# facebookresearch/AudioDec

Measured on NVIDIA H100. Metric: 48 kHz audio samples/s, encode+quantize+lookup+decode (% HBM roofline in `roofline`), higher is better.
Workload: dtype f32

## Files before the change

### audiodec_b200/_lib.py

```python
from __future__ import annotations

import ctypes
import os

_HERE = os.path.dirname(os.path.abspath(__file__))
LIB_PATH = os.environ.get("ADEC_LIB_PATH") or os.path.join(_HERE, "lib", "libaudiodec_b200.so")
MAX_STAGES = 8

c_int, c_float, c_void_p, c_char_p = ctypes.c_int, ctypes.c_float, ctypes.c_void_p, ctypes.c_char_p
c_int64 = ctypes.c_int64
_I8 = c_int * MAX_STAGES


class AdecConfig(ctypes.Structure):
    _fields_ = [
        ("model_type", c_int),
        ("input_channels", c_int), ("output_channels", c_int), ("encode_channels", c_int), ("decode_channels", c_int),
        ("code_dim", c_int), ("codebook_num", c_int), ("codebook_size", c_int),
        ("n_enc", c_int), ("enc_ratios", _I8), ("enc_strides", _I8),
        ("n_dec", c_int), ("dec_ratios", _I8), ("dec_strides", _I8),
        ("bias", c_int),
        ("in_channels", c_int), ("out_channels", c_int), ("channels", c_int), ("kernel_size", c_int),
        ("n_up", c_int), ("upsample_scales", _I8), ("upsample_kernel_sizes", _I8),
        ("resblock_kernel_size", c_int),
        ("n_dil", c_int), ("resblock_dilations", _I8),
        ("groups", c_int),
        ("negative_slope", c_float),
        ("use_weight_norm", c_int),
        ("has_stats", c_int),
        ("codec_activate", c_int),
        ("n_resblocks", c_int), ("resblock_kernel_sizes", _I8),
        ("compute_dtype", c_int),
    ]


MODEL_SYMAD, MODEL_HIFIGAN = 0, 1

SYMBOLS = {
    "adec_create": (c_int, [ctypes.POINTER(AdecConfig), c_int, ctypes.POINTER(c_void_p)]),
    "adec_destroy": (None, [c_void_p]),
    "adec_last_error": (c_char_p, [c_void_p]),
    "adec_set_tensor": (c_int, [c_void_p, c_char_p, c_void_p, ctypes.POINTER(c_int64), c_int]),
    "adec_finalize": (c_int, [c_void_p]),
    "adec_n_streams": (c_int, [c_void_p]),
    "adec_set_streams": (c_int, [c_void_p, c_int]),
    "adec_reset": (c_int, [c_void_p, c_void_p]),
    "adec_encode": (c_int, [c_void_p, c_void_p, c_int, c_int, c_void_p, c_void_p]),
    "adec_quantize": (c_int, [c_void_p, c_void_p, c_int, c_int, c_void_p, c_void_p]),
    "adec_quantize_ex": (c_int, [c_void_p, c_void_p, c_int, c_int, c_void_p, c_void_p, c_void_p, c_void_p]),
    "adec_lookup": (c_int, [c_void_p, c_void_p, c_int, c_int, c_void_p, c_void_p]),
    "adec_lookup_packed": (c_int, [c_void_p, c_void_p, c_int, c_int, c_void_p, c_void_p]),
    "adec_decode": (c_int, [c_void_p, c_void_p, c_int, c_int, c_void_p, c_void_p]),
    "adec_encode_offline": (c_int, [c_void_p, c_void_p, c_int, c_int, c_void_p, c_void_p]),
    "adec_decode_offline": (c_int, [c_void_p, c_void_p, c_int, c_int, c_void_p, c_void_p]),
    "adec_decode_bf16": (c_int, [c_void_p, c_void_p, c_int, c_int, c_void_p, c_void_p]),
    "adec_decode_offline_bf16": (c_int, [c_void_p, c_void_p, c_int, c_int, c_void_p, c_void_p]),
    "adec_encode_offline_varlen": (c_int, [c_void_p, c_void_p, ctypes.POINTER(c_int), c_int, c_void_p, c_void_p]),
    "adec_decode_offline_varlen": (c_int, [c_void_p, c_void_p, ctypes.POINTER(c_int), c_int, c_void_p, c_void_p]),
    "adec_decode_offline_varlen_bf16": (c_int, [c_void_p, c_void_p, ctypes.POINTER(c_int), c_int, c_void_p, c_void_p]),
    "adec_encode_streams": (c_int, [c_void_p, c_void_p, ctypes.POINTER(c_int), ctypes.POINTER(c_int), c_int, c_void_p, c_void_p]),
    "adec_decode_streams": (c_int, [c_void_p, c_void_p, ctypes.POINTER(c_int), ctypes.POINTER(c_int), c_int, c_void_p, c_void_p]),
    "adec_decode_streams_bf16": (c_int, [c_void_p, c_void_p, ctypes.POINTER(c_int), ctypes.POINTER(c_int), c_int, c_void_p, c_void_p]),
    "adec_copy_stream_state": (c_int, [c_void_p, c_int, ctypes.POINTER(c_int), c_int, c_void_p]),
    "adec_frames_for": (c_int, [c_void_p, c_int]),
    "adec_hop_length": (c_int, [c_void_p]),
    "adec_codec_host": (c_int, [c_void_p, c_void_p, c_void_p, c_int, c_int, c_void_p, c_void_p, c_void_p]),
    "adec_packed_frame_bytes": (c_int, [c_void_p]),
    "adec_pack_indices": (c_int, [c_void_p, c_void_p, c_int, c_int, c_void_p, c_void_p]),
    "adec_unpack_indices": (c_int, [c_void_p, c_void_p, c_int, c_int, c_void_p, c_void_p]),
    "adec_index_error": (c_int, [c_void_p, c_void_p]),
    "adec_range_error": (c_int, [c_void_p, c_void_p]),
    "adec_launch_count": (c_int64, [c_void_p]),
    "adec_ktrace": (c_int, [c_void_p, ctypes.POINTER(ctypes.c_ulonglong), c_int]),
    "adec_probe_mma": (c_int, [c_int, c_int, c_int, c_int, ctypes.POINTER(ctypes.c_double), ctypes.POINTER(ctypes.c_double)]),
    "adec_profile": (c_int, [c_void_p, c_int]),
    "adec_profile_report": (c_int, [c_void_p, c_char_p, c_int]),
    "adec_test_causal_conv": (c_int, [c_int, c_void_p, c_int, c_int, c_int, c_void_p, c_void_p, c_int, c_int, c_int,
                                      c_int, c_int, c_int, c_float, c_void_p, c_void_p]),
    "adec_test_residual_unit": (c_int, [c_int, c_void_p, c_int, c_int, c_int, c_void_p, c_void_p, c_int, c_int, c_void_p, c_void_p]),
    "adec_test_causal_convtr": (c_int, [c_int, c_void_p, c_int, c_int, c_int, c_void_p, c_void_p, c_int, c_int,
                                        c_void_p, c_void_p]),
    "adec_test_vocoder_layer": (c_int, [c_int, c_int, c_int, c_void_p, c_int, c_int, c_int, c_void_p, c_void_p, c_int, c_int, c_int,
                                        c_int, c_int, c_int, c_int, c_float, c_void_p, c_void_p, c_void_p, c_int, c_void_p, c_void_p]),
}

_lib = None


def load():
    global _lib
    if _lib is not None:
        return _lib
    if not os.path.exists(LIB_PATH):
        raise RuntimeError(
            f"{LIB_PATH} not found: build the CUDA extension first "
            "(python -c 'import __graft_entry__ as g; g.build()').  audiodec_b200 has no CPU fallback.")
    lib = ctypes.CDLL(LIB_PATH)
    for name, (res, args) in SYMBOLS.items():
        fn = getattr(lib, name)
        fn.restype = res
        fn.argtypes = args
    _lib = lib
    return lib


def last_error(handle=None) -> str:
    msg = load().adec_last_error(handle)
    return msg.decode() if msg else ""
```

### audiodec_b200/csrc/adec.cu

```cuda
#include <cuda_runtime.h>

#include <algorithm>
#include <cmath>
#include <cstdarg>
#include <cstdio>
#include <cstring>
#include <map>
#include <memory>
#include <set>
#include <string>
#include <vector>

#include "../../include/audiodec_b200.h"
#include "kernels.cuh"
#include "wg_conv.cuh"
#include <cuda_fp16.h>
#include <cuda_bf16.h>

using namespace adec;

namespace {
thread_local std::string g_create_error;

std::string fmt(const char* f, ...) {
    char buf[1024];
    va_list ap;
    va_start(ap, f);
    vsnprintf(buf, sizeof buf, f, ap);
    va_end(ap);
    return buf;
}

struct HostTensor {
    std::vector<int64_t> shape;
    std::vector<float> data;
    int64_t numel() const { int64_t n = 1; for (auto s : shape) n *= s; return n; }
};

int round_up(int v, int m) { return (v + m - 1) / m * m; }
bool is_pow2(int v) { return v > 0 && (v & (v - 1)) == 0; }
int ilog2(int v) { int l = 0; while ((1 << l) < v) ++l; return l; }

typedef cudaError_t (*ConvLaunchFn)(const ConvArgs&, dim3, int, cudaStream_t);

template <int CW, int CO, int TT, int KC, bool F>
cudaError_t launch_conv(const ConvArgs& a, dim3 grid, int window_rows, cudaStream_t s) {
    using Cfg = ConvCfg<CW, CO, TT, KC>;
    static bool configured[64] = {false};
    int dev = 0;
    cudaGetDevice(&dev);
    auto kern = conv_gemm_kernel<CW, CO, TT, KC, F>;
    if (dev < 64 && !configured[dev]) {
        cudaError_t e = cudaFuncSetAttribute(kern, cudaFuncAttributeMaxDynamicSharedMemorySize, 227 * 1024);
        if (e != cudaSuccess) return e;
        configured[dev] = true;
    }
    const size_t smem = Cfg::smem_bytes(window_rows);
    if (smem > 227 * 1024) return cudaErrorInvalidConfiguration;
    kern<<<grid, Cfg::NTHREADS, smem, s>>>(a);
    return cudaGetLastError();
}

struct ConvKernelCfg { int CW, CO, TT, KC; bool fuse; ConvLaunchFn fn; };

#define ADEC_PLAIN(CW) \
    {CW, 256, 64, 8, false, launch_conv<CW, 256, 64, 8, false>}, \
    {CW, 128, 64, 16, false, launch_conv<CW, 128, 64, 16, false>}, \
    {CW, 64, 128, 32, false, launch_conv<CW, 64, 128, 32, false>}, \
    {CW, 32, 256, 32, false, launch_conv<CW, 32, 256, 32, false>}

const ConvKernelCfg kConvKernels[] = {
    ADEC_PLAIN(32), ADEC_PLAIN(64), ADEC_PLAIN(96), ADEC_PLAIN(128), ADEC_PLAIN(256),
    {32, 32, 256, 32, true, launch_conv<32, 32, 256, 32, true>},
    {64, 64, 128, 32, true, launch_conv<64, 64, 128, 32, true>},
    {128, 128, 64, 16, true, launch_conv<128, 128, 64, 16, true>},
    {256, 256, 64, 8, true, launch_conv<256, 256, 64, 8, true>},
};

const ConvKernelCfg* find_conv_kernel(int CW, int CO, bool fuse) {
    for (const auto& k : kConvKernels)
        if (k.CW == CW && k.CO == CO && k.fuse == fuse) return &k;
    return nullptr;
}

typedef cudaError_t (*TcPersistFn)(const ConvArgs&, int, int, int, int, int, cudaStream_t);
template <int NT, bool F, int PRE, int PREC, bool BST, bool VL>
cudaError_t launch_wg(const ConvArgs& a, int n_xtiles, int n_ytiles, int n_tiles, int n_ctas, int smem_bytes, cudaStream_t s) {
    static bool configured[64] = {false};
    int dev = 0;
    cudaGetDevice(&dev);
    auto kern = wg_conv_kernel<NT, F, PRE, PREC, BST, VL>;
    constexpr int kMaxDyn = 227 * 1024;
    if (dev < 64 && !configured[dev]) {
        cudaError_t e = cudaFuncSetAttribute(kern, cudaFuncAttributeMaxDynamicSharedMemorySize, kMaxDyn);
        if (e != cudaSuccess) return e;
        configured[dev] = true;
    }
    if (smem_bytes > kMaxDyn) return cudaErrorInvalidConfiguration;
    static const bool pdl = [] { const char* e = getenv("ADEC_PDL"); return !e || atoi(e) != 0; }();
    cudaLaunchConfig_t cfg{};
    cfg.gridDim = dim3((unsigned)n_ctas);
    cfg.blockDim = dim3((unsigned)WgCfg<NT, PREC>::THREADS);
    cfg.dynamicSmemBytes = (size_t)smem_bytes;
    cfg.stream = s;
    cudaLaunchAttribute attr[1];
    attr[0].id = cudaLaunchAttributeProgrammaticStreamSerialization;
    attr[0].val.programmaticStreamSerializationAllowed = 1;
    cfg.attrs = attr;
    cfg.numAttrs = pdl ? 1 : 0;
    return cudaLaunchKernelEx(&cfg, kern, a, n_xtiles, n_ytiles, n_tiles);
}
typedef size_t (*TcSmemFn)(int, bool);
typedef int (*TcWbufFn)(int, bool);
struct TcKernelCfg { int NT; bool fuse; int pre, prec; bool bst; int tap_bytes; TcPersistFn pfn, pfn_vl; TcSmemFn smem; TcWbufFn n_wbuf; };
#define ADEC_TC1(NT, F, PRE, PREC, BST) \
    {NT, F, PRE, PREC, BST, WgCfg<NT, PREC>::TAP_BYTES, launch_wg<NT, F, PRE, PREC, BST, false>, launch_wg<NT, F, PRE, PREC, BST, true>, \
     WgCfg<NT, PREC>::smem_bytes, WgCfg<NT, PREC>::n_wbuf}
#define ADEC_TC_FP32(NT, PREC) \
    ADEC_TC1(NT, true, ACT_ELU, PREC, false), ADEC_TC1(NT, false, ACT_NONE, PREC, false), ADEC_TC1(NT, false, ACT_ELU, PREC, false), \
    ADEC_TC1(NT, false, ACT_LRELU, PREC, false), ADEC_TC1(NT, false, ACT_NORM, PREC, false)
#define ADEC_TC_BF16(NT, BST) \
    ADEC_TC1(NT, false, ACT_NONE, PREC_BF16, BST), ADEC_TC1(NT, false, ACT_LRELU, PREC_BF16, BST), ADEC_TC1(NT, false, ACT_NORM, PREC_BF16, BST)
#define ADEC_TC(NT) ADEC_TC_FP32(NT, PREC_F16), ADEC_TC_FP32(NT, PREC_TF32), ADEC_TC_BF16(NT, false), ADEC_TC_BF16(NT, true)
const TcKernelCfg kTcKernels[] = {ADEC_TC(128), ADEC_TC(64), ADEC_TC(32)};
int kTcMaxFuse = 128;

const TcKernelCfg* find_tc_kernel(int NT, bool fuse, int pre, int prec, bool bst) {
    for (const auto& k : kTcKernels)
        if (k.NT == NT && k.fuse == fuse && k.pre == pre && k.prec == prec && k.bst == bst) return &k;
    return nullptr;
}

uint16_t half_bits(float x) { const __half h = __float2half_rn(x); uint16_t u; memcpy(&u, &h, 2); return u; }
float half_value(uint16_t u) { __half h; memcpy(&h, &u, 2); return __half2float(h); }
uint16_t bf16_bits(float x) { const __nv_bfloat16 h = __float2bfloat16_rn(x); uint16_t u; memcpy(&u, &h, 2); return u; }

float tf32_round_host(float x) {
    uint32_t u;
    memcpy(&u, &x, 4);
    if ((u & 0x7F800000u) == 0x7F800000u) return x;
    u = (u + 0x1000u) & 0xFFFFE000u;
    float r;
    memcpy(&r, &u, 4);
    return r;
}

enum OpKind { OP_STEM, OP_CONV, OP_HEAD };
enum { BUF_EXT_IN = -10, BUF_EXT_OUT = -11, BUF_NONE = -1 };

struct Op {
    OpKind kind = OP_CONV;
    std::string name;
    int G = 1, Cin = 0, Cin_eff = 0, Cout = 0, Ktaps = 1, dil = 1, RG = 1;
    int P = 0;
    int down = 1;
    int up = 1;
    bool fuse = false, shared_in = false, out_nct = false, post_tanh = false;
    int pre_act = ACT_NONE, mid_act = ACT_NONE;
    float slope = 0.f;
    std::vector<float> weff;
    std::vector<float> weff2;
    std::vector<float> hbias;
    std::vector<float> hstate;
    const ConvKernelCfg* kc = nullptr;
    const TcKernelCfg* tc = nullptr;
    float w_scale = 1.f, w2_scale = 1.f;
    int n_pieces = 1, n_co_tiles = 1;
    float *w = nullptr, *w2 = nullptr, *bias = nullptr;
    const float *mean = nullptr, *scale = nullptr;
    float head_bias = 0.f;
    long long w_tile_floats = 0;
    int st_C = 0, st_groups = 1;
    float* st[2] = {nullptr, nullptr};
    int cur = 0;
    int in_buf = BUF_NONE, out_buf = BUF_NONE, res_buf = BUF_NONE;
    int ldx = 0, x_goff = 0, ldy = 0, y_goff = 0, ldr = 0, r_goff = 0;
};

struct DevBuf {
    float* p = nullptr;
    size_t cap = 0;
};

struct SlotBits {
    std::vector<uint8_t> bit;
    bool dirty = false;
};

}

struct adec_handle {
    adec_config cfg{};
    int device = 0;
    bool finalized = false;
    std::string err;
    std::map<std::string, HostTensor> tensors;
    std::set<std::string> consumed;
    std::vector<Op> enc_ops, dec_ops;
    int n_streams = 1;
    int st_cap = 1;
    int engine = 2;
    bool use_tc = true;
    bool bf16 = false;
    bool act_bf16 = false;
    int act_bytes() const { return act_bf16 ? 2 : 4; }
    bool stack_rows = true;
    unsigned long long* d_ktrace = nullptr;
    int ktrace_n = 0;
    int n_sms = 132;
    DevBuf ws[3];
    std::vector<void*> owned;
    float *d_embed = nullptr, *d_e2 = nullptr, *d_codebook = nullptr;
    float *d_mean = nullptr, *d_scale = nullptr;
    int* d_err = nullptr;
    int64_t launches = 0;
    bool profiling = false;
    std::vector<std::pair<cudaEvent_t, cudaEvent_t>> prof_events;
    std::vector<std::string> prof_names;
    std::vector<double> prof_bytes;
    DevBuf hx, hz, hzq, hy;
    DevBuf vl_tab;
    SlotBits enc_slots, dec_slots;
    DevBuf slot_tab;
    long long* hidx = nullptr;
    size_t hidx_cap = 0;

    int fail(const std::string& m) { err = m; return 1; }
};

namespace {

#define CK(h, call)                                                                        \
    do {                                                                                   \
        cudaError_t e_ = (call);                                                           \
        if (e_ != cudaSuccess) return (h)->fail(fmt("%s failed: %s", #call, cudaGetErrorString(e_))); \
    } while (0)

int dev_alloc(adec_handle* h, float** p, size_t n_floats) {
    CK(h, cudaMalloc((void**)p, std::max<size_t>(n_floats, 4) * sizeof(float)));
    h->owned.push_back(*p);
    return 0;
}

int dev_upload(adec_handle* h, float** p, const std::vector<float>& v) {
    if (dev_alloc(h, p, v.size())) return 1;
    if (!v.empty()) CK(h, cudaMemcpy(*p, v.data(), v.size() * sizeof(float), cudaMemcpyHostToDevice));
    return 0;
}

int ensure(adec_handle* h, DevBuf& b, size_t n_floats) {
    if (b.cap >= n_floats) return 0;
    if (b.p) CK(h, cudaFree(b.p));
    b.p = nullptr;
    b.cap = 0;
    CK(h, cudaMalloc((void**)&b.p, n_floats * sizeof(float)));
    b.cap = n_floats;
    return 0;
}

const HostTensor* find(adec_handle* h, const std::string& key) {
    auto it = h->tensors.find(key);
    if (it == h->tensors.end()) return nullptr;
    h->consumed.insert(key);
    return &it->second;
}

int get_weight(adec_handle* h, const std::string& prefix, HostTensor* out) {
    if (const HostTensor* w = find(h, prefix + ".weight")) { *out = *w; return 0; }
    const HostTensor* g = find(h, prefix + ".weight_g");
    const HostTensor* v = find(h, prefix + ".weight_v");
    if (!g || !v) return h->fail("missing key " + prefix + ".weight (or .weight_g/.weight_v)");
    const int64_t n0 = v->shape[0], inner = v->numel() / n0;
    if (g->numel() != n0) return h->fail("bad weight_g shape for " + prefix);
    *out = *v;
    for (int64_t i = 0; i < n0; ++i) {
        double ss = 0;
        for (int64_t j = 0; j < inner; ++j) ss += (double)v->data[i * inner + j] * v->data[i * inner + j];
        const float scale = g->data[i] / (float)std::sqrt(ss);
        for (int64_t j = 0; j < inner; ++j) out->data[i * inner + j] = v->data[i * inner + j] * scale;
    }
    return 0;
}

int make_conv_op(adec_handle* h, Op* op, const std::string& name, const HostTensor& W, const HostTensor* bias,
                 int stride, int dil, int groups, int pre_act, float slope, bool shared_in) {
    if (W.shape.size() != 3) return h->fail("conv weight must be 3-D: " + name);
    const int cout_t = (int)W.shape[0], cin_g = (int)W.shape[1], K = (int)W.shape[2];
    if (cout_t % groups) return h->fail("Cout not divisible by groups: " + name);
    const int cout_g = cout_t / groups;
    op->kind = OP_CONV;
    op->name = name;
    op->G = groups;
    op->pre_act = pre_act;
    op->slope = slope;
    op->shared_in = shared_in;
    op->Cout = round_up(cout_g, 32);
    if (stride == 1) {
        op->RG = 1; op->Ktaps = K; op->dil = dil; op->P = (K - 1) * dil; op->down = 1;
        op->Cin = round_up(cin_g, 32);
        op->Cin_eff = op->Cin;
    } else {
        if (K != 2 * stride || dil != 1) return h->fail(fmt("%s: strided conv needs kernel=2*stride, dilation 1", name.c_str()));
        if (!is_pow2(cin_g) || cin_g < 4) return h->fail(fmt("%s: strided conv needs power-of-two Cin>=4", name.c_str()));
        op->RG = stride; op->Ktaps = 2; op->dil = 1; op->P = K - 1; op->down = stride;
        op->Cin = cin_g;
        op->Cin_eff = round_up(stride * cin_g, 32);
    }
    op->weff.assign((size_t)groups * op->Ktaps * op->Cin_eff * op->Cout, 0.f);
    for (int g = 0; g < groups; ++g)
        for (int co = 0; co < cout_g; ++co)
            for (int ci = 0; ci < cin_g; ++ci)
                for (int k = 0; k < K; ++k) {
                    const float v = W.data[((size_t)(g * cout_g + co) * cin_g + ci) * K + k];
                    int tap, q;
                    if (stride == 1) { tap = k; q = ci; }
                    else { tap = k / stride; q = (k % stride) * cin_g + ci; }
                    op->weff[(((size_t)g * op->Ktaps + tap) * op->Cin_eff + q) * op->Cout + co] = v;
                }
    if (bias) {
        op->hbias.assign((size_t)groups * op->Cout, 0.f);
        for (int g = 0; g < groups; ++g)
            for (int co = 0; co < cout_g; ++co) op->hbias[(size_t)g * op->Cout + co] = bias->data[g * cout_g + co];
    }
    op->st_groups = shared_in ? 1 : groups;
    op->st_C = op->st_groups * op->Cin;
    return 0;
}

int make_convtr_op(adec_handle* h, Op* op, const std::string& name, const HostTensor& W, const HostTensor* bias,
                   int stride, int pre_act, float slope) {
    if (W.shape.size() != 3 || W.shape[2] != 2 * stride) return h->fail(name + ": transposed conv needs kernel = 2*stride");
    const int cin = (int)W.shape[0], cout = (int)W.shape[1], K = 2 * stride;
    op->kind = OP_CONV;
    op->name = name;
    op->G = 1; op->RG = 1; op->Ktaps = 2; op->dil = 1; op->P = 1; op->down = 1; op->up = stride;
    op->pre_act = pre_act; op->slope = slope;
    op->Cin = round_up(cin, 32);
    op->Cin_eff = op->Cin;
    op->Cout = round_up(stride * cout, 32);
    op->weff.assign((size_t)2 * op->Cin_eff * op->Cout, 0.f);
    for (int ci = 0; ci < cin; ++ci)
        for (int co = 0; co < cout; ++co)
            for (int r = 0; r < stride; ++r) {
                op->weff[((size_t)0 * op->Cin_eff + ci) * op->Cout + r * cout + co] = W.data[((size_t)ci * cout + co) * K + stride + r];
                op->weff[((size_t)1 * op->Cin_eff + ci) * op->Cout + r * cout + co] = W.data[((size_t)ci * cout + co) * K + r];
            }
    if (bias) {
        op->hbias.assign(op->Cout, 0.f);
        for (int r = 0; r < stride; ++r)
            for (int co = 0; co < cout; ++co) op->hbias[r * cout + co] = bias->data[co];
    }
    op->st_groups = 1;
    op->st_C = op->Cin;
    return 0;
}

int make_ru_op(adec_handle* h, Op* op, const std::string& name, const HostTensor& W1, const HostTensor& W2, int dil, int act) {
    if (make_conv_op(h, op, name, W1, nullptr, 1, dil, 1, act, 0.f, false)) return 1;
    const int c = (int)W1.shape[0];
    if (W1.shape[1] != c || W2.shape[0] != c || W2.shape[1] != c || W2.shape[2] != 1 || c != op->Cout)
        return h->fail(name + ": residual unit needs square weights with C % 32 == 0");
    op->fuse = true;
    op->mid_act = act;
    op->weff2.assign((size_t)c * c, 0.f);
    for (int co = 0; co < c; ++co)
        for (int ci = 0; ci < c; ++ci) op->weff2[(size_t)ci * c + co] = W2.data[(size_t)co * c + ci];
    return 0;
}

void split_ru_op(const Op& ru, Op* conv, Op* pw) {
    *conv = ru;
    conv->fuse = false;
    conv->weff2.clear();
    conv->mid_act = ACT_NONE;
    *pw = Op();
    pw->kind = OP_CONV;
    pw->name = ru.name + ".conv2";
    pw->G = 1; pw->Cin = ru.Cout; pw->Cin_eff = ru.Cout; pw->Cout = ru.Cout; pw->Ktaps = 1; pw->dil = 1; pw->RG = 1; pw->P = 0;
    pw->pre_act = ru.mid_act; pw->slope = ru.slope;
    pw->weff = ru.weff2;
    pw->st_groups = 1; pw->st_C = ru.Cout;
}

int pick_piece_width(const Op& op) {
    static const int cands[] = {256, 128, 96, 64, 32};
    for (int cw : cands) {
        if (op.Cin_eff % cw) continue;
        if (op.RG > 1 && !(cw % op.Cin == 0 || op.Cin % cw == 0)) continue;
        return cw;
    }
    return 0;
}

int finalize_op_tc(adec_handle* h, Op* op) {
    int NT = op->Cout % 128 == 0 ? 128 : op->Cout % 64 == 0 ? 64 : 32;
    const bool pad_tile = !op->fuse && NT == 32 && op->Cout > 64 && op->Cout < 128;
    if (pad_tile) NT = 128;
    op->tc = find_tc_kernel(NT, op->fuse, op->pre_act, PREC_TF32, false);
    if (!op->tc || (op->fuse && (NT != op->Cout || op->mid_act != op->pre_act))) return h->fail(op->name + ": no tensor-core kernel");
    const int KS = TC_CP, CP = TC_CP;
    op->n_pieces = op->Cin_eff / CP;
    op->n_co_tiles = pad_tile ? 1 : op->Cout / NT;
    op->w_tile_floats = (long long)op->Ktaps * op->Cin_eff * NT * 2;
    auto pack = [&](const float* weff, int G, int ntiles, int pieces, int taps, int cin_eff, int cout, std::vector<float>* out) {
        out->assign((size_t)G * ntiles * taps * cin_eff * NT * 2, 0.f);
        size_t o = 0;
        for (int g = 0; g < G; ++g)
            for (int nt = 0; nt < ntiles; ++nt)
                for (int pc = 0; pc < pieces; ++pc)
                    for (int tap = 0; tap < taps; ++tap)
                        for (int ks = 0; ks < CP / KS; ++ks) {
                            float* hi = out->data() + o;
                            float* lo = hi + (size_t)KS * NT;
                            for (int c4 = 0; c4 < KS / 4; ++c4)
                                for (int n = 0; n < NT; ++n)
                                    for (int e = 0; e < 4; ++e) {
                                        const int k = pc * CP + ks * KS + c4 * 4 + e;
                                        const float w = nt * NT + n < cout ? weff[(((size_t)g * taps + tap) * cin_eff + k) * cout + nt * NT + n] : 0.f;
                                        const float wh = tf32_round_host(w);
                                        hi[((size_t)c4 * NT + n) * 4 + e] = wh;
                                        lo[((size_t)c4 * NT + n) * 4 + e] = tf32_round_host(w - wh);
                                    }
                            o += (size_t)2 * KS * NT;
                        }
    };
    std::vector<float> packed;
    pack(op->weff.data(), op->G, op->n_co_tiles, op->n_pieces, op->Ktaps, op->Cin_eff, op->Cout, &packed);
    if (dev_upload(h, &op->w, packed)) return 1;
    if (op->fuse) {
        std::vector<float> p2;
        pack(op->weff2.data(), 1, 1, op->Cout / CP, 1, op->Cout, op->Cout, &p2);
        if (dev_upload(h, &op->w2, p2)) return 1;
    }
    if (!op->hbias.empty() && dev_upload(h, &op->bias, op->hbias)) return 1;
    std::vector<float>().swap(op->weff);
    std::vector<float>().swap(op->weff2);
    return 0;
}

int finalize_op_f16(adec_handle* h, Op* op) {
    int NT = op->Cout % 128 == 0 ? 128 : op->Cout % 64 == 0 ? 64 : 32;
    const bool pad_tile = !op->fuse && NT == 32 && op->Cout > 64 && op->Cout < 128;
    if (pad_tile) NT = 128;
    const int prec = (h->bf16 && !op->fuse) ? PREC_BF16 : PREC_F16;
    if (h->act_bf16 && op->RG > 1) return h->fail(op->name + ": bf16 activations are built for stride-1 and transposed convs only");
    op->tc = find_tc_kernel(NT, op->fuse, op->pre_act, prec, h->act_bf16);
    if (!op->tc || (op->fuse && (NT != op->Cout || op->mid_act != op->pre_act))) return h->fail(op->name + ": no tensor-core kernel");
    const int CP = TC_CP, KB = TC_CP / 8, npl = prec == PREC_F16 ? 3 : 1;
    op->n_pieces = op->Cin_eff / CP;
    op->n_co_tiles = pad_tile ? 1 : op->Cout / NT;
    const size_t tap_bytes = (size_t)op->tc->tap_bytes;
    op->w_tile_floats = (long long)((size_t)op->n_pieces * op->Ktaps * tap_bytes / 4);
    auto pow2_scale = [](const std::vector<float>& w, int* p_out) {
        float wmax = 0.f;
        for (float v : w) wmax = std::max(wmax, std::fabs(v));
        int p = 0;
        if (wmax > 0.f && std::isfinite(wmax)) {
            while (std::ldexp(wmax, p) < 4096.f) ++p;
            while (std::ldexp(wmax, p) >= 8192.f) --p;
        }
        *p_out = p;
    };
    auto pack = [&](const float* weff, int G, int ntiles, int pieces, int taps, int cin_eff, int cout, int p2, std::vector<float>* out) {
        std::vector<uint16_t> img((size_t)G * ntiles * pieces * taps * tap_bytes / 2, 0);
        size_t o = 0;
        for (int g = 0; g < G; ++g)
            for (int nt = 0; nt < ntiles; ++nt)
                for (int pc = 0; pc < pieces; ++pc)
                    for (int tap = 0; tap < taps; ++tap) {
                        for (int kb = 0; kb < KB; ++kb)
                            for (int n = 0; n < NT; ++n)
                                for (int e = 0; e < 8; ++e) {
                                    const int k = pc * CP + kb * 8 + e;
                                    const float w = nt * NT + n < cout ? weff[(((size_t)g * taps + tap) * cin_eff + k) * cout + nt * NT + n] : 0.f;
                                    const size_t at = o + ((size_t)kb * NT + n) * 8 + e, plane = (size_t)KB * NT * 8;
                                    if (prec == PREC_F16) {
                                        const float ws = std::ldexp(w, p2);
                                        const uint16_t hi = half_bits(ws);
                                        img[at] = hi;
                                        img[at + plane] = half_bits(ws - half_value(hi));
                                        img[at + 2 * plane] = half_bits(half_value(hi) * (1.0f / 2048.0f));
                                    } else {
                                        img[at] = bf16_bits(w);
                                    }
                                }
                        o += (size_t)npl * KB * NT * 8;
                    }
        out->assign((img.size() + 1) / 2, 0.f);
        memcpy(out->data(), img.data(), img.size() * 2);
    };
    int p1 = 0, p2 = 0;
    if (prec == PREC_F16) pow2_scale(op->weff, &p1);
    op->w_scale = std::ldexp(1.0f, -p1);
    std::vector<float> packed;
    pack(op->weff.data(), op->G, op->n_co_tiles, op->n_pieces, op->Ktaps, op->Cin_eff, op->Cout, p1, &packed);
    if (dev_upload(h, &op->w, packed)) return 1;
    if (op->fuse) {
        pow2_scale(op->weff2, &p2);
        op->w2_scale = std::ldexp(1.0f, -p2);
        std::vector<float> pk2;
        pack(op->weff2.data(), 1, 1, op->Cout / CP, 1, op->Cout, op->Cout, p2, &pk2);
        if (dev_upload(h, &op->w2, pk2)) return 1;
    }
    if (!op->hbias.empty() && dev_upload(h, &op->bias, op->hbias)) return 1;
    std::vector<float>().swap(op->weff);
    std::vector<float>().swap(op->weff2);
    return 0;
}

int finalize_op(adec_handle* h, Op* op) {
    if (op->kind != OP_CONV) return 0;
    if (h->engine == 2) return finalize_op_f16(h, op);
    if (h->use_tc) return finalize_op_tc(h, op);
    int CW, CO;
    if (op->fuse) {
        CW = CO = op->Cout;
    } else {
        CW = pick_piece_width(*op);
        CO = op->Cout % 256 == 0 ? 256 : op->Cout % 128 == 0 ? 128 : op->Cout % 64 == 0 ? 64 : 32;
    }
    op->kc = CW ? find_conv_kernel(CW, CO, op->fuse) : nullptr;
    if (!op->kc) return h->fail(fmt("%s: no kernel for Cin_eff=%d Cout=%d fuse=%d", op->name.c_str(), op->Cin_eff, op->Cout, (int)op->fuse));
    op->n_pieces = op->Cin_eff / CW;
    op->n_co_tiles = op->Cout / CO;
    const int KC = op->kc->KC, nkc = CW / KC;
    op->w_tile_floats = (long long)op->Ktaps * op->Cin_eff * CO;
    std::vector<float> packed((size_t)op->G * op->n_co_tiles * op->w_tile_floats);
    size_t o = 0;
    for (int g = 0; g < op->G; ++g)
        for (int ct = 0; ct < op->n_co_tiles; ++ct)
            for (int pc = 0; pc < op->n_pieces; ++pc)
                for (int tap = 0; tap < op->Ktaps; ++tap)
                    for (int kcc = 0; kcc < nkc; ++kcc)
                        for (int k = 0; k < KC; ++k) {
                            const int q = pc * CW + kcc * KC + k;
                            const float* src = &op->weff[(((size_t)g * op->Ktaps + tap) * op->Cin_eff + q) * op->Cout + ct * CO];
                            for (int co = 0; co < CO; ++co) packed[o++] = src[co];
                        }
    if (dev_upload(h, &op->w, packed)) return 1;
    if (op->fuse) {
        if (dev_upload(h, &op->w2, op->weff2)) return 1;
    }
    if (!op->hbias.empty() && dev_upload(h, &op->bias, op->hbias)) return 1;
    std::vector<float>().swap(op->weff);
    std::vector<float>().swap(op->weff2);
    return 0;
}

int alloc_state(adec_handle* h, Op* op, int n_streams) {
    const size_t per = (size_t)op->P * op->st_C, eb = h->act_bytes();
    if (per == 0) return 0;
    for (int i = 0; i < 2; ++i) {
        CK(h, cudaMalloc((void**)&op->st[i], per * n_streams * eb));
        CK(h, cudaMemset(op->st[i], 0, per * n_streams * eb));
    }
    op->cur = 0;
    if (!op->hstate.empty()) {
        std::vector<uint16_t> hb;
        if (h->act_bf16) for (float v : op->hstate) hb.push_back(bf16_bits(v));
        const void* src = h->act_bf16 ? (const void*)hb.data() : (const void*)op->hstate.data();
        for (int s = 0; s < n_streams; ++s)
            CK(h, cudaMemcpy((char*)op->st[0] + s * per * eb, src, per * eb, cudaMemcpyHostToDevice));
    }
    return 0;
}

void load_pad_buffer(adec_handle* h, Op* op, const std::string& key, int c_real) {
    const HostTensor* pb = find(h, key);
    if (!pb || pb->shape.size() != 3 || op->P == 0) return;
    const int C = (int)pb->shape[1], P = (int)pb->shape[2];
    if (P != op->P) return;
    bool any = false;
    for (float v : pb->data) any |= (v != 0.f);
    if (!any) return;
    op->hstate.assign((size_t)op->P * op->st_C, 0.f);
    const int groups = op->st_groups, cg = c_real;
    for (int g = 0; g < groups; ++g)
        for (int c = 0; c < cg && g * cg + c < C; ++c)
            for (int p = 0; p < P; ++p) op->hstate[(size_t)p * op->st_C + g * op->Cin + c] = pb->data[((size_t)(g * cg + c)) * P + p];
}

struct RunCtx {
    int B;
    const float* ext_in;
    float* ext_out;
    cudaStream_t stream;
    bool offline = false;
    const int* vl_len = nullptr;
    const char* what = "";
    const int* slots = nullptr;
};

SlotBits* slot_bits(adec_handle* h, const std::vector<Op>& ops) {
    return &ops == &h->enc_ops ? &h->enc_slots : &ops == &h->dec_ops ? &h->dec_slots : nullptr;
}

int slot_copy(adec_handle* h, std::vector<Op>& ops, const std::vector<int>& pairs, int src_sel, int dst_sel, cudaStream_t stream) {
    const int n = (int)pairs.size() / 2;
    if (n == 0) return 0;
    if (ensure(h, h->slot_tab, pairs.size())) return 1;
    CK(h, cudaMemcpyAsync(h->slot_tab.p, pairs.data(), pairs.size() * sizeof(int), cudaMemcpyHostToDevice, stream));
    for (Op& op : ops) {
        const long long per = (long long)op.P * op.st_C * h->act_bytes() / 4;
        if (!per) continue;
        const long long tot = per * n;
        slot_copy_kernel<<<(unsigned)((tot + 255) / 256), 256, 0, stream>>>(op.st[op.cur ^ dst_sel], op.st[op.cur ^ src_sel], per,
                                                                          reinterpret_cast<const int*>(h->slot_tab.p), n);
        CK(h, cudaGetLastError());
        ++h->launches;
    }
    return 0;
}

int slot_fixup(adec_handle* h, std::vector<Op>& ops, cudaStream_t stream) {
    SlotBits* sb = slot_bits(h, ops);
    if (!sb || !sb->dirty) return 0;
    std::vector<int> pairs;
    for (int s = 0; s < (int)sb->bit.size(); ++s)
        if (sb->bit[s]) { pairs.push_back(s); pairs.push_back(s); }
    if (slot_copy(h, ops, pairs, 1, 0, stream)) return 1;
    std::fill(sb->bit.begin(), sb->bit.end(), 0);
    sb->dirty = false;
    return 0;
}

constexpr long long kVlMaxRows = (1ll << 31) - 4096;

struct VlPlan {
    std::vector<int> tab;
    std::vector<long long> T, Tout;
};
int plan_varlen(adec_handle* h, const std::vector<Op>& ops, const RunCtx& rc, VlPlan* pl) {
    const int B = rc.B;
    std::vector<long long> len(rc.vl_len, rc.vl_len + B);
    pl->tab.assign(ops.size() * 2 * (B + 1), 0);
    for (size_t k = 0; k < ops.size(); ++k) {
        const Op& op = ops[k];
        const long long halo = op.kind == OP_CONV ? (long long)(op.Ktaps - 1) * op.dil : 0;
        int* in = pl->tab.data() + k * 2 * (B + 1);
        int* out = in + B + 1;
        long long si = 0, so = 0;
        for (int b = 0; b < B; ++b) {
            const long long tout = (len[b] - 1) / op.down + 1;
            si += len[b];
            so += tout;
            if (si > kVlMaxRows || so * op.up > kVlMaxRows || so + (b + 1) * halo > kVlMaxRows)
                return h->fail(fmt("%s: the batch needs more than %lld rows at %s, beyond the kernels' 32-bit row indexing; split it",
                                   rc.what, kVlMaxRows, op.name.c_str()));
            in[b + 1] = (int)si;
            out[b + 1] = (int)so;
            len[b] = tout * op.up;
        }
        pl->T.push_back(si);
        pl->Tout.push_back(so);
    }
    return 0;
}

int run_ops(adec_handle* h, std::vector<Op>& ops, const RunCtx& rc, int T_in, int* T_out_final) {
    const bool vl = rc.vl_len != nullptr;
    VlPlan pl;
    if (vl) {
        if (plan_varlen(h, ops, rc, &pl)) return 1;
        for (const Op& op : ops)
            if (op.kind == OP_CONV && !op.tc)
                return h->fail(fmt("%s: the FFMA engine (ADEC_CONV_PATH=ffma) has no varlen kernels; use the f16 or tf32 tensor-core engine",
                                   rc.what));
    }
    size_t need[3] = {0, 0, 0};
    {
        int T = T_in;
        for (size_t k = 0; k < ops.size(); ++k) {
            const Op& op = ops[k];
            const int Tout = (T - 1) / op.down + 1;
            const size_t rows = vl ? (size_t)pl.Tout[k] : (size_t)rc.B * Tout;
            if (op.out_buf >= 0) need[op.out_buf] = std::max(need[op.out_buf], rows * op.ldy);
            T = Tout * op.up;
        }
    }
    for (int i = 0; i < 3; ++i)
        if (need[i] && ensure(h, h->ws[i], (need[i] * h->act_bytes() + 3) / 4)) return 1;
    if (!vl && rc.B != h->n_streams) return h->fail(fmt("batch %d != n_streams %d (call adec_set_streams)", rc.B, h->n_streams));
    const int* vl_tab = nullptr;
    const int* vl_slot = nullptr;
    SlotBits* sb = slot_bits(h, ops);
    if (vl && rc.slots) {
        for (const Op& op : ops)
            if ((long long)h->n_streams * op.P * op.st_C >= (1ll << 31))
                return h->fail(fmt("%s: %d streams of %s state exceed 2^31 elements per buffer; use fewer streams per handle", rc.what,
                                   h->n_streams, op.name.c_str()));
        const size_t at = pl.tab.size();
        for (int b = 0; b < rc.B; ++b) pl.tab.push_back(2 * rc.slots[b] + sb->bit[rc.slots[b]]);
        if (ensure(h, h->vl_tab, pl.tab.size())) return 1;
        CK(h, cudaMemcpyAsync(h->vl_tab.p, pl.tab.data(), pl.tab.size() * sizeof(int), cudaMemcpyHostToDevice, rc.stream));
        vl_tab = reinterpret_cast<const int*>(h->vl_tab.p);
        vl_slot = vl_tab + at;
    } else if (vl) {
        if (adec_reset(h, (void*)rc.stream)) return 1;
        if (ensure(h, h->vl_tab, pl.tab.size())) return 1;
        CK(h, cudaMemcpyAsync(h->vl_tab.p, pl.tab.data(), pl.tab.size() * sizeof(int), cudaMemcpyHostToDevice, rc.stream));
        vl_tab = reinterpret_cast<const int*>(h->vl_tab.p);
    } else if (slot_fixup(h, ops, rc.stream)) {
        return 1;
    }

    int T = T_in;
    for (size_t k = 0; k < ops.size(); ++k) {
        Op& op = ops[k];
        int Tout = (T - 1) / op.down + 1;
        const int* vl_in = vl ? vl_tab + k * 2 * (rc.B + 1) : nullptr;
        const int* vl_out = vl ? vl_in + rc.B + 1 : nullptr;
        if (vl) { T = (int)pl.T[k]; Tout = (int)pl.Tout[k]; }
        const int nb = vl ? 1 : rc.B;
        const float* xin = op.in_buf == BUF_EXT_IN ? rc.ext_in : h->ws[op.in_buf].p;
        float* yout = op.out_buf == BUF_EXT_OUT ? rc.ext_out : h->ws[op.out_buf].p;
        const float* st_in = op.st[op.cur];
        float* st_out = op.st[op.cur ^ 1];
        cudaError_t e = cudaSuccess;
        cudaEvent_t ev0 = nullptr, ev1 = nullptr;
        if (h->profiling) {
            cudaEventCreate(&ev0); cudaEventCreate(&ev1);
            cudaEventRecord(ev0, rc.stream);
        }
        if (op.kind == OP_STEM) {
            StemArgs a{};
            a.x = xin; a.x_bs = T; a.st_in = st_in; a.st_out = st_out; a.T = T;
            a.w = op.w; a.bias = op.bias; a.y = yout; a.y_bs = (long long)T * op.ldy;
            a.vl_off = vl_in; a.vl_B = rc.B; a.vl_slot = vl_slot;
            dim3 grid((T + 1023) / 1024, nb);
            if (vl) stem_kernel<32, 7, true><<<grid, 256, 0, rc.stream>>>(a);
            else stem_kernel<32, 7><<<grid, 256, 0, rc.stream>>>(a);
            e = cudaGetLastError();
        } else if (op.kind == OP_HEAD) {
            HeadArgs a{};
            a.x = xin; a.x_bs = (long long)T * op.ldx; a.ldx = op.ldx; a.st_in = st_in; a.st_out = st_out; a.T = T;
            a.w = op.w; a.bias = op.head_bias; a.pre_act = op.pre_act; a.slope = op.slope; a.post_tanh = op.post_tanh;
            a.y = yout; a.y_bs = T;
            a.vl_off = vl_in; a.vl_B = rc.B; a.vl_slot = vl_slot;
            dim3 grid((T + 255) / 256, nb);
            if (vl && h->act_bf16) head_kernel<32, 7, true, true><<<grid, 256, 0, rc.stream>>>(a);
            else if (vl) head_kernel<32, 7, false, true><<<grid, 256, 0, rc.stream>>>(a);
            else if (h->act_bf16) head_kernel<32, 7, true><<<grid, 256, 0, rc.stream>>>(a);
            else head_kernel<32, 7, false><<<grid, 256, 0, rc.stream>>>(a);
            e = cudaGetLastError();
        } else {
            ConvArgs a{};
            a.x = xin; a.x_bs = (long long)T * op.ldx; a.ldx = op.ldx; a.x_goff = op.x_goff;
            a.st_in = st_in; a.st_out = st_out; a.st_ld = op.st_C; a.st_goff = op.shared_in ? 0 : op.Cin; a.st_groups = op.st_groups;
            a.P = op.P; a.T = T; a.Tout = Tout;
            a.Ktaps = op.Ktaps; a.dil = op.dil; a.RG = op.RG; a.lgCin = ilog2(op.Cin); a.Cin = op.Cin;
            a.n_pieces = op.n_pieces; a.pre_act = op.pre_act; a.slope = op.slope; a.mean = op.mean; a.scale = op.scale;
            a.w = op.w; a.w2 = op.w2; a.bias = op.bias; a.n_co_tiles = op.n_co_tiles; a.Cout_g = op.Cout;
            a.w_tile_floats = op.w_tile_floats;
            if (op.fuse) { a.res = xin; a.res_bs = a.x_bs; a.ldr = op.ldx; a.r_goff = 0; }
            else if (op.res_buf >= 0) { a.res = h->ws[op.res_buf].p; a.res_bs = (long long)Tout * op.ldr; a.ldr = op.ldr; a.r_goff = op.r_goff; }
            a.y = yout; a.ldy = op.ldy; a.y_goff = op.y_goff; a.out_nct = op.out_nct;
            a.y_bs = op.out_nct ? (long long)op.G * op.Cout * Tout : (long long)Tout * op.ldy;
            a.mid_act = op.mid_act;
            a.hist_rep = (rc.offline && op.up > 1) ? 1 : 0;
            a.w_scale = op.w_scale; a.w2_scale = op.w2_scale; a.err = h->d_err;
            if (h->d_ktrace && h->ktrace_n < 4096) a.dbg = h->d_ktrace + 3 * (size_t)(h->ktrace_n++);
            if (op.tc) {
                const int wrows = TC_TT + (op.Ktaps - 1) * op.dil;
                dim3 grid((Tout + TC_TT - 1) / TC_TT, op.G * op.n_co_tiles, rc.B);
                a.n_streams = rc.B;
                if (vl) {
                    const long long rows = (long long)Tout + (long long)rc.B * (op.Ktaps - 1) * op.dil;
                    grid = dim3((unsigned)((rows + TC_TT - 1) / TC_TT), grid.y, 1);
                    a.n_streams = 1;
                    a.vl_in = vl_in; a.vl_out = vl_out; a.vl_B = rc.B; a.vl_slot = vl_slot;
                } else if (h->stack_rows) {
                    const long long L = (long long)Tout + (long long)(op.Ktaps - 1) * op.dil;
                    const long long stacked = (rc.B * L + TC_TT - 1) / TC_TT;
                    if (stacked * 4 <= (long long)grid.x * rc.B * 3 && rc.B * L < (1ll << 30)) {
                        a.stack_L = (int)L;
                        grid = dim3((unsigned)stacked, grid.y, 1);
                    }
                }
                const long long n_tiles = (long long)grid.x * grid.y * grid.z;
                const int n_ctas = (int)std::min<long long>(n_tiles, h->n_sms);
                const size_t psmem = op.tc->smem(wrows, op.fuse);
                a.n_wbuf = op.tc->n_wbuf(wrows, op.fuse);
                if (a.n_wbuf < 1) return h->fail(fmt("%s: window of %d rows does not fit in shared memory", op.name.c_str(), wrows));
                e = (vl ? op.tc->pfn_vl : op.tc->pfn)(a, (int)grid.x, (int)grid.y, (int)n_tiles, n_ctas, (int)psmem, rc.stream);
            } else {
                const int TT = op.kc->TT;
                dim3 grid((Tout + TT - 1) / TT, op.G * op.n_co_tiles, rc.B);
                e = op.kc->fn(a, grid, TT + (op.Ktaps - 1) * op.dil, rc.stream);
            }
        }
        if (e != cudaSuccess) return h->fail(fmt("launch of %s failed: %s", op.name.c_str(), cudaGetErrorString(e)));
        ++h->launches;
        if (h->profiling) {
            cudaEventRecord(ev1, rc.stream);
            h->prof_events.emplace_back(ev0, ev1);
            h->prof_names.push_back(op.name);
            const double cin = op.kind == OP_STEM ? 1 : (double)op.G * op.Cin_eff / std::max(1, op.RG) * (op.shared_in ? 1.0 / op.G : 1.0);
            const double cout = op.kind == OP_HEAD ? 1 : (double)op.G * op.Cout;
            const double eb = h->act_bytes();
            double bytes = eb * nb * (cin * T + cout * Tout);
            if (op.fuse) bytes += eb * nb * (3.0 * cout * Tout);
            else if (op.res_buf >= 0) bytes += eb * nb * cout * Tout;
            h->prof_bytes.push_back(bytes);
        }
        if (op.P > 0 && !vl) op.cur ^= 1;
        T = Tout * op.up;
    }
    if (vl_slot) {
        for (int b = 0; b < rc.B; ++b) sb->bit[rc.slots[b]] ^= 1;
        sb->dirty = true;
    }
    if (T_out_final) *T_out_final = T;
    return 0;
}

int need_tensor(adec_handle* h, const std::string& key, const HostTensor** out) {
    *out = find(h, key);
    if (!*out) return h->fail("missing key " + key);
    return 0;
}

int build_stem(adec_handle* h, Op* op, const std::string& prefix, int cout) {
    HostTensor Wt;
    if (get_weight(h, prefix + ".conv", &Wt)) return 1;
    const HostTensor* W = &Wt;
    if (W->shape[0] != 32 || W->shape[1] != 1 || W->shape[2] != 7 || cout != 32)
        return h->fail("stem conv: only input_channels=1, encode_channels=32, kernel 7 is built");
    op->kind = OP_STEM; op->name = prefix; op->P = 6; op->st_C = 1; op->Cin = 1; op->Cout = 32;
    std::vector<float> w(7 * 32);
    for (int co = 0; co < 32; ++co)
        for (int k = 0; k < 7; ++k) w[k * 32 + co] = W->data[co * 7 + k];
    if (dev_upload(h, &op->w, w)) return 1;
    if (const HostTensor* b = find(h, prefix + ".conv.bias")) { if (dev_upload(h, &op->bias, b->data)) return 1; }
    if (const HostTensor* pb = find(h, prefix + ".pad_buffer")) {
        bool any = false; for (float v : pb->data) any |= v != 0.f;
        if (any && pb->numel() == 6) op->hstate = pb->data;
    }
    return 0;
}

int build_head(adec_handle* h, Op* op, const std::string& prefix, int pre_act, float slope, bool tanh_out) {
    HostTensor W;
    if (get_weight(h, prefix + ".conv", &W)) return 1;
    if (W.shape[0] != 1 || W.shape[1] != 32 || W.shape[2] != 7)
        return h->fail("head conv: only 32 -> 1 channels, kernel 7 is built");
    op->kind = OP_HEAD; op->name = prefix; op->P = 6; op->st_C = 32; op->Cin = 32; op->Cout = 1;
    op->pre_act = pre_act; op->slope = slope; op->post_tanh = tanh_out;
    std::vector<float> w(7 * 32);
    for (int ci = 0; ci < 32; ++ci)
        for (int k = 0; k < 7; ++k) w[k * 32 + ci] = W.data[ci * 7 + k];
    if (dev_upload(h, &op->w, w)) return 1;
    if (const HostTensor* b = find(h, prefix + ".conv.bias")) op->head_bias = b->data[0];
    op->st_groups = 1;
    load_pad_buffer(h, op, prefix + ".pad_buffer", 32);
    return 0;
}

struct Wire {
    int cur = BUF_EXT_IN;
    int cur_ld = 0;
    int pick(int avoid1 = -99, int avoid2 = -99) const {
        for (int i = 0; i < 3; ++i)
            if (i != cur && i != avoid1 && i != avoid2) return i;
        return 0;
    }
};

void chain(Op* op, Wire* w, int out_ld) {
    op->in_buf = w->cur; op->ldx = w->cur_ld; op->x_goff = op->shared_in ? 0 : op->Cin;
    op->out_buf = w->pick(); op->ldy = out_ld; op->y_goff = op->Cout;
    w->cur = op->out_buf; w->cur_ld = out_ld;
}

int push_ru(adec_handle* h, std::vector<Op>* ops, Wire* w, const std::string& ru, int dil, int ch) {
    HostTensor W1, W2;
    if (get_weight(h, ru + ".conv1.conv", &W1) || get_weight(h, ru + ".conv2", &W2)) return 1;
    Op op;
    if (make_ru_op(h, &op, ru, W1, W2, dil, ACT_ELU)) return 1;
    load_pad_buffer(h, &op, ru + ".conv1.pad_buffer", ch);
    if (h->use_tc && op.Cout > kTcMaxFuse) {
        Op conv, pw;
        split_ru_op(op, &conv, &pw);
        const int x_buf = w->cur;
        chain(&conv, w, ch);
        pw.in_buf = w->cur; pw.ldx = ch; pw.x_goff = pw.Cin;
        pw.res_buf = x_buf; pw.ldr = ch; pw.r_goff = 0;
        pw.out_buf = w->pick(x_buf); pw.ldy = ch; pw.y_goff = pw.Cout;
        w->cur = pw.out_buf; w->cur_ld = ch;
        ops->push_back(std::move(conv));
        ops->push_back(std::move(pw));
    } else {
        chain(&op, w, ch);
        ops->push_back(std::move(op));
    }
    return 0;
}

int build_symad(adec_handle* h) {
    const adec_config& c = h->cfg;
    if (c.input_channels != 1 || c.output_channels != 1) return h->fail("symAD: only mono (input/output_channels=1) is built");
    if (c.code_dim != 64) return h->fail("symAD: only code_dim=64 is built");
    Wire w; w.cur = BUF_EXT_IN; w.cur_ld = 1;
    {
        Op op;
        if (build_stem(h, &op, "encoder.conv", c.encode_channels)) return 1;
        op.in_buf = BUF_EXT_IN; op.ldx = 1; op.out_buf = 0; op.ldy = 32;
        w.cur = 0; w.cur_ld = 32;
        h->enc_ops.push_back(std::move(op));
    }
    int ch = c.encode_channels;
    static const int dils[3] = {1, 3, 9};
    for (int i = 0; i < c.n_enc; ++i) {
        const std::string pre = fmt("encoder.conv_blocks.%d", i);
        for (int j = 0; j < 3; ++j)
            if (push_ru(h, &h->enc_ops, &w, pre + fmt(".res_units.%d", j), dils[j], ch)) return 1;
        HostTensor W;
        if (get_weight(h, pre + ".conv.conv", &W)) return 1;
        const HostTensor* b = find(h, pre + ".conv.conv.bias");
        Op op;
        if (make_conv_op(h, &op, pre + ".conv", W, b, c.enc_strides[i], 1, 1, ACT_NONE, 0.f, false)) return 1;
        load_pad_buffer(h, &op, pre + ".conv.pad_buffer", ch);
        ch = c.encode_channels * c.enc_ratios[i];
        chain(&op, &w, ch);
        h->enc_ops.push_back(std::move(op));
    }
    {
        HostTensor W;
        if (get_weight(h, "projector.project.conv", &W)) return 1;
        Op op;
        if (make_conv_op(h, &op, "projector.project", W, find(h, "projector.project.conv.bias"), 1, 1, 1,
                         c.codec_activate ? ACT_ELU : ACT_NONE, 0.f, false)) return 1;
        load_pad_buffer(h, &op, "projector.project.pad_buffer", ch);
        op.in_buf = w.cur; op.ldx = w.cur_ld; op.x_goff = op.Cin;
        op.out_buf = BUF_EXT_OUT; op.out_nct = true; op.ldy = op.Cout; op.y_goff = op.Cout;
        if (op.Cout != c.code_dim) return h->fail("projector: code_dim must be a multiple of 32");
        h->enc_ops.push_back(std::move(op));
    }
    Wire d; d.cur = BUF_EXT_IN; d.cur_ld = c.code_dim;
    {
        HostTensor W;
        if (get_weight(h, "decoder.conv1.conv", &W)) return 1;
        Op op;
        if (make_conv_op(h, &op, "decoder.conv1", W, find(h, "decoder.conv1.conv.bias"), 1, 1, 1, ACT_NONE, 0.f, false)) return 1;
        load_pad_buffer(h, &op, "decoder.conv1.pad_buffer", c.code_dim);
        chain(&op, &d, op.Cout);
        h->dec_ops.push_back(std::move(op));
    }
    for (int i = 0; i < c.n_dec; ++i) {
        const std::string pre = fmt(c.codec_activate ? "decoder.conv_blocks.%d.1" : "decoder.conv_blocks.%d", i);
        const int cin = c.decode_channels * c.dec_ratios[i];
        const int cout = i < c.n_dec - 1 ? c.decode_channels * c.dec_ratios[i + 1] : c.decode_channels;
        HostTensor W;
        if (get_weight(h, pre + ".conv.deconv", &W)) return 1;
        Op op;
        if (make_convtr_op(h, &op, pre + ".conv", W, find(h, pre + ".conv.deconv.bias"), c.dec_strides[i],
                           c.codec_activate ? ACT_ELU : ACT_NONE, 0.f)) return 1;
        if (op.Cout != c.dec_strides[i] * cout) return h->fail(pre + ": stride*Cout must be a multiple of 32");
        load_pad_buffer(h, &op, pre + ".conv.pad_buffer", cin);
        chain(&op, &d, op.Cout);
        d.cur_ld = cout;
        h->dec_ops.push_back(std::move(op));
        for (int j = 0; j < 3; ++j)
            if (push_ru(h, &h->dec_ops, &d, pre + fmt(".res_units.%d", j), dils[j], cout)) return 1;
    }
    {
        Op op;
        if (build_head(h, &op, "decoder.conv2", c.codec_activate ? ACT_ELU : ACT_NONE, 0.f, c.codec_activate != 0)) return 1;
        op.in_buf = d.cur; op.ldx = d.cur_ld; op.out_buf = BUF_EXT_OUT; op.ldy = 1;
        h->dec_ops.push_back(std::move(op));
    }
    const int nq = c.codebook_num, D = c.code_dim, N = c.codebook_size;
    if (N != 1024) return h->fail("RVQ: only codebook_size=1024 is built");
    std::vector<float> embed((size_t)nq * D * N), e2((size_t)nq * N), cb((size_t)nq * N * D);
    for (int i = 0; i < nq; ++i) {
        const HostTensor* E;
        if (need_tensor(h, fmt("quantizer.codebook.layers.%d.embed", i), &E)) return 1;
        if (E->shape.size() != 2 || E->shape[0] != D || E->shape[1] != N) return h->fail("bad embed shape");
        std::copy(E->data.begin(), E->data.end(), embed.begin() + (size_t)i * D * N);
        for (int cdx = 0; cdx < N; ++cdx) {
            float total = 0.f;
            for (int bk = 0; bk < D; bk += 16) {
                float part = 0.f;
                for (int k = bk; k < bk + 16 && k < D; ++k) {
                    volatile float sq = E->data[(size_t)k * N + cdx] * E->data[(size_t)k * N + cdx];
                    part = part + sq;
                }
                total = bk == 0 ? part : total + part;
            }
            e2[(size_t)i * N + cdx] = total;
            for (int k = 0; k < D; ++k) cb[((size_t)i * N + cdx) * D + k] = E->data[(size_t)k * N + cdx];
        }
        find(h, fmt("quantizer.codebook.layers.%d.cluster_size", i));
        find(h, fmt("quantizer.codebook.layers.%d.embed_avg", i));
    }
    if (dev_upload(h, &h->d_embed, embed) || dev_upload(h, &h->d_e2, e2) || dev_upload(h, &h->d_codebook, cb)) return 1;
    return 0;
}

int synthesize_mrf_as_groups(adec_handle* h, int stage, int C, HostTensor W1[], HostTensor B1[], HostTensor W2[], HostTensor B2[],
                             HostTensor* Wout) {
    const adec_config& c = h->cfg;
    const int nb = c.n_resblocks;
    int K = 0;
    for (int b = 0; b < nb; ++b) K = std::max(K, c.resblock_kernel_sizes[b]);
    for (int j = 0; j < c.n_dil; ++j)
        for (int which = 0; which < 2; ++which) {
            HostTensor& W = which ? W2[j] : W1[j];
            HostTensor& Bt = which ? B2[j] : B1[j];
            W.shape = {nb * C, C, K};
            W.data.assign((size_t)nb * C * C * K, 0.f);
            Bt.shape = {nb * C};
            Bt.data.assign((size_t)nb * C, 0.f);
            for (int b = 0; b < nb; ++b) {
                const int kb = c.resblock_kernel_sizes[b];
                const std::string pre = fmt("blocks.%d.blocks.%d.convs%d.%d", stage, b, which + 1, j);
                HostTensor w;
                if (get_weight(h, pre + ".conv", &w)) return 1;
                if (w.shape.size() != 3 || w.shape[0] != C || w.shape[1] != C || w.shape[2] != kb) return h->fail("bad shape: " + pre);
                for (int co = 0; co < C; ++co)
                    for (int ci = 0; ci < C; ++ci)
                        for (int k = 0; k < kb; ++k)
                            W.data[((size_t)(b * C + co) * C + ci) * K + (K - kb) + k] = w.data[((size_t)co * C + ci) * kb + k];
                if (const HostTensor* bb = find(h, pre + ".conv.bias"))
                    for (int co = 0; co < C; ++co) Bt.data[b * C + co] = bb->data[co];
                find(h, pre + ".pad_buffer");
            }
        }
    Wout->shape = {C, nb * C, 1};
    Wout->data.assign((size_t)C * nb * C, 0.f);
    for (int co = 0; co < C; ++co)
        for (int b = 0; b < nb; ++b) Wout->data[(size_t)co * nb * C + b * C + co] = 1.0f / nb;
    return 0;
}

int build_hifigan(adec_handle* h) {
    const adec_config& c = h->cfg;
    if (c.out_channels != 1) return h->fail("HiFi-GAN: only out_channels=1 is built");
    const bool mrf = c.n_resblocks > 0;
    if (!mrf && c.groups < 2) return h->fail("HiFi-GAN: groups must be > 1 for the MultiGroupConv1d variant");
    if (mrf && c.groups != 1) return h->fail("HiFi-GAN: MultiReceptiveField needs groups = 1");
    const float slope = c.negative_slope;
    if (c.has_stats) {
        const HostTensor *m, *s;
        if (need_tensor(h, "mean", &m) || need_tensor(h, "scale", &s)) return 1;
        std::vector<float> mp(round_up(c.in_channels, 32), 0.f), sp(round_up(c.in_channels, 32), 1.f);
        std::copy(m->data.begin(), m->data.end(), mp.begin());
        std::copy(s->data.begin(), s->data.end(), sp.begin());
        if (dev_upload(h, &h->d_mean, mp) || dev_upload(h, &h->d_scale, sp)) return 1;
    }
    Wire w; w.cur = BUF_EXT_IN; w.cur_ld = c.in_channels;
    {
        HostTensor W;
        if (get_weight(h, "input_conv.conv", &W)) return 1;
        Op op;
        if (make_conv_op(h, &op, "input_conv", W, find(h, "input_conv.conv.bias"), 1, 1, 1, c.has_stats ? ACT_NORM : ACT_NONE, 0.f, false)) return 1;
        op.mean = h->d_mean; op.scale = h->d_scale;
        load_pad_buffer(h, &op, "input_conv.pad_buffer", c.in_channels);
        chain(&op, &w, op.Cout);
        h->dec_ops.push_back(std::move(op));
    }
    for (int i = 0; i < c.n_up; ++i) {
        const int cin = c.channels >> i, cout = c.channels >> (i + 1), s = c.upsample_scales[i];
        if (c.upsample_kernel_sizes[i] != 2 * s) return h->fail("HiFi-GAN: upsample kernel must be 2*scale (HiFiGAN.py:95)");
        {
            HostTensor W;
            const std::string pre = fmt("upsamples.%d", i);
            if (get_weight(h, pre + ".deconv", &W)) return 1;
            Op op;
            if (make_convtr_op(h, &op, pre, W, find(h, pre + ".deconv.bias"), s, ACT_LRELU, slope)) return 1;
            if (op.Cout != s * cout) return h->fail(pre + ": scale*Cout must be a multiple of 32");
            load_pad_buffer(h, &op, pre + ".pad_buffer", cin);
            chain(&op, &w, op.Cout);
            w.cur_ld = cout;
            h->dec_ops.push_back(std::move(op));
        }
        const int G = mrf ? c.n_resblocks : c.groups, C3 = G * cout;
        HostTensor mW1[ADEC_MAX_STAGES], mB1[ADEC_MAX_STAGES], mW2[ADEC_MAX_STAGES], mB2[ADEC_MAX_STAGES], mWout;
        if (mrf && synthesize_mrf_as_groups(h, i, cout, mW1, mB1, mW2, mB2, &mWout)) return 1;
        const int A = w.cur;
        const int Bb = w.pick();
        const int Cc = w.pick(Bb);
        for (int j = 0; j < c.n_dil; ++j) {
            const std::string p1 = fmt("blocks.%d.convs1.%d", i, j), p2 = fmt("blocks.%d.convs2.%d", i, j);
            HostTensor W1, W2;
            const HostTensor *b1 = nullptr, *b2 = nullptr;
            if (mrf) {
                W1 = mW1[j]; W2 = mW2[j]; b1 = &mB1[j]; b2 = &mB2[j];
            } else {
                if (get_weight(h, p1 + ".conv", &W1) || get_weight(h, p2 + ".conv", &W2)) return 1;
                b1 = find(h, p1 + ".conv.bias"); b2 = find(h, p2 + ".conv.bias");
            }
            Op o1, o2;
            if (make_conv_op(h, &o1, p1, W1, b1, 1, c.resblock_dilations[j], G, ACT_LRELU, slope, j == 0)) return 1;
            if (make_conv_op(h, &o2, p2, W2, b2, 1, 1, G, ACT_LRELU, slope, false)) return 1;
            if (o1.Cout != cout || o1.Cin != cout) return h->fail(p1 + ": channels must be a multiple of 32");
            if (!mrf) {
                load_pad_buffer(h, &o1, p1 + ".pad_buffer", cout);
                load_pad_buffer(h, &o2, p2 + ".pad_buffer", cout);
            }
            o1.in_buf = j == 0 ? A : Cc; o1.ldx = j == 0 ? cout : C3; o1.x_goff = j == 0 ? 0 : cout;
            o1.out_buf = Bb; o1.ldy = C3; o1.y_goff = cout;
            o2.in_buf = Bb; o2.ldx = C3; o2.x_goff = cout;
            o2.res_buf = j == 0 ? A : Cc; o2.ldr = j == 0 ? cout : C3; o2.r_goff = j == 0 ? 0 : cout;
            o2.out_buf = Cc; o2.ldy = C3; o2.y_goff = cout;
            h->dec_ops.push_back(std::move(o1));
            h->dec_ops.push_back(std::move(o2));
        }
        {
            HostTensor W;
            const std::string po = fmt("blocks.%d.conv_out", i);
            if (mrf) W = mWout;
            else if (get_weight(h, po, &W)) return 1;
            Op op;
            if (make_conv_op(h, &op, po, W, find(h, po + ".bias"), 1, 1, 1, ACT_NONE, 0.f, false)) return 1;
            op.in_buf = Cc; op.ldx = C3; op.x_goff = op.Cin;
            op.out_buf = A; op.ldy = cout; op.y_goff = op.Cout;
            w.cur = A; w.cur_ld = cout;
            h->dec_ops.push_back(std::move(op));
        }
    }
    {
        Op op;
        if (build_head(h, &op, "output_conv", ACT_LRELU, 0.01f, true)) return 1;
        op.in_buf = w.cur; op.ldx = w.cur_ld; op.out_buf = BUF_EXT_OUT; op.ldy = 1;
        h->dec_ops.push_back(std::move(op));
    }
    return 0;
}

int hop_of(const adec_handle* h) {
    int hop = 1;
    if (h->cfg.model_type == ADEC_MODEL_SYMAD) for (int i = 0; i < h->cfg.n_enc; ++i) hop *= h->cfg.enc_strides[i];
    else for (int i = 0; i < h->cfg.n_up; ++i) hop *= h->cfg.upsample_scales[i];
    return hop;
}

struct DeviceGuard {
    int prev = -1;
    explicit DeviceGuard(int dev) { cudaGetDevice(&prev); if (prev != dev) cudaSetDevice(dev); else prev = -1; }
    ~DeviceGuard() { if (prev >= 0) cudaSetDevice(prev); }
};

}

extern "C" {

int adec_create(const adec_config* cfg, int device, adec_handle** out) {
    if (!cfg || !out) { g_create_error = "null argument"; return 1; }
    int ndev = 0;
    cudaError_t e = cudaGetDeviceCount(&ndev);
    if (e != cudaSuccess || device < 0 || device >= ndev) {
        g_create_error = fmt("no usable CUDA device %d (%s); audiodec_b200 has no CPU fallback", device,
                             e == cudaSuccess ? "out of range" : cudaGetErrorString(e));
        return 1;
    }
    if (cfg->n_enc > ADEC_MAX_STAGES || cfg->n_dec > ADEC_MAX_STAGES || cfg->n_up > ADEC_MAX_STAGES || cfg->n_dil > ADEC_MAX_STAGES) {
        g_create_error = "too many stages";
        return 1;
    }
    auto* h = new adec_handle();
    h->cfg = *cfg;
    h->device = device;
    if (const char* pth = getenv("ADEC_CONV_PATH")) {
        if (!strcmp(pth, "ffma")) h->engine = 0;
        else if (!strcmp(pth, "tf32")) h->engine = 1;
        else if (!strcmp(pth, "f16") || !strcmp(pth, "tc") || !*pth) h->engine = 2;
        else { g_create_error = std::string("ADEC_CONV_PATH must be f16, tf32 or ffma, not ") + pth; delete h; return 1; }
    }
    h->use_tc = h->engine != 0;
    if (const char* sr = getenv("ADEC_STACK_ROWS")) h->stack_rows = atoi(sr) != 0;
    if (const char* kt = getenv("ADEC_KTRACE")) {
        if (atoi(kt)) { DeviceGuard dgk(device); cudaMalloc((void**)&h->d_ktrace, 4096 * 3 * sizeof(unsigned long long)); }
    }
    h->bf16 = cfg->compute_dtype == 1 || cfg->compute_dtype == 2;
    h->act_bf16 = cfg->compute_dtype == 2;
    if (cfg->compute_dtype < 0 || cfg->compute_dtype > 2) {
        g_create_error = "compute_dtype must be 0 (fp32), 1 (bf16 operands) or 2 (bf16 operands and activations)";
        delete h;
        return 1;
    }
    if (h->bf16 && (cfg->model_type != ADEC_MODEL_HIFIGAN || h->engine != 2)) {
        g_create_error = "compute_dtype = bf16 is built for the HiFi-GAN vocoder on the f16 tensor-core engine only (the encoder, projector and RVQ "
                         "must stay fp32-grade for bit-identical indices)";
        delete h;
        return 1;
    }
    if (h->act_bf16 && cfg->in_channels % 8) {
        g_create_error = "compute_dtype = 2 needs in_channels to be a multiple of 8";
        delete h;
        return 1;
    }
    if (const char* mf = getenv("ADEC_TC_MAXFUSE")) kTcMaxFuse = atoi(mf);
    cudaDeviceGetAttribute(&h->n_sms, cudaDevAttrMultiProcessorCount, device);
    DeviceGuard dg(device);
    if (cudaMalloc((void**)&h->d_err, sizeof(int)) != cudaSuccess || cudaMemset(h->d_err, 0, sizeof(int)) != cudaSuccess) {
        g_create_error = "cudaMalloc failed";
        delete h;
        return 1;
    }
    *out = h;
    return 0;
}

void adec_destroy(adec_handle* h) {
    if (!h) return;
    DeviceGuard dg(h->device);
    for (void* p : h->owned) cudaFree(p);
    for (auto* ops : {&h->enc_ops, &h->dec_ops})
        for (Op& op : *ops)
            for (int i = 0; i < 2; ++i) if (op.st[i]) cudaFree(op.st[i]);
    for (auto& b : h->ws) if (b.p) cudaFree(b.p);
    for (DevBuf* b : {&h->hx, &h->hz, &h->hzq, &h->hy, &h->vl_tab, &h->slot_tab}) if (b->p) cudaFree(b->p);
    if (h->hidx) cudaFree(h->hidx);
    if (h->d_err) cudaFree(h->d_err);
    if (h->d_ktrace) cudaFree(h->d_ktrace);
    delete h;
}

const char* adec_last_error(const adec_handle* h) { return h ? h->err.c_str() : g_create_error.c_str(); }

int adec_set_tensor(adec_handle* h, const char* key, const float* data, const int64_t* shape, int ndim) {
    if (!h || !key || !data || ndim < 0 || ndim > 4) return h ? h->fail("bad argument to adec_set_tensor") : 1;
    if (h->finalized) return h->fail("adec_set_tensor after adec_finalize");
    HostTensor t;
    t.shape.assign(shape, shape + ndim);
    t.data.assign(data, data + t.numel());
    h->tensors[key] = std::move(t);
    return 0;
}

int adec_finalize(adec_handle* h) {
    if (!h) return 1;
    if (h->finalized) return h->fail("already finalized");
    DeviceGuard dg(h->device);
    int rc = h->cfg.model_type == ADEC_MODEL_SYMAD ? build_symad(h)
           : h->cfg.model_type == ADEC_MODEL_HIFIGAN ? build_hifigan(h)
           : h->fail("unknown model_type");
    if (rc) return rc;
    for (const auto& kv : h->tensors)
        if (!h->consumed.count(kv.first)) return h->fail("unexpected key in state dict: " + kv.first);
    for (auto* ops : {&h->enc_ops, &h->dec_ops})
        for (Op& op : *ops) {
            if (finalize_op(h, &op)) return 1;
            if (alloc_state(h, &op, 1)) return 1;
        }
    h->n_streams = 1;
    h->enc_slots.bit.assign(1, 0);
    h->dec_slots.bit.assign(1, 0);
    h->tensors.clear();
    h->finalized = true;
    return 0;
}

int adec_n_streams(const adec_handle* h) { return h ? h->n_streams : 0; }

static int resize_state(adec_handle* h, int n, bool replicate) {
    const int keep = std::min(n, h->n_streams);
    CK(h, cudaDeviceSynchronize());
    if (slot_fixup(h, h->enc_ops, 0) || slot_fixup(h, h->dec_ops, 0)) return 1;
    CK(h, cudaDeviceSynchronize());
    for (auto* ops : {&h->enc_ops, &h->dec_ops})
        for (Op& op : *ops) {
            const size_t per = (size_t)op.P * op.st_C * h->act_bytes() / 4;
            if (!per) continue;
            if (n > h->st_cap) {
                float* nb[2] = {nullptr, nullptr};
                for (int i = 0; i < 2; ++i) CK(h, cudaMalloc((void**)&nb[i], per * n * sizeof(float)));
                CK(h, cudaMemcpy(nb[0], op.st[op.cur], per * keep * sizeof(float), cudaMemcpyDeviceToDevice));
                for (int i = 0; i < 2; ++i) cudaFree(op.st[i]);
                op.st[0] = nb[0]; op.st[1] = nb[1]; op.cur = 0;
            }
            if (n > keep) {
                float* tail = op.st[op.cur] + per * keep;
                const long long tot = (long long)per * (n - keep);
                if (replicate) {
                    replicate_kernel<<<(unsigned)((tot + 255) / 256), 256>>>(tail, op.st[op.cur], (long long)per, n - keep);
                    CK(h, cudaGetLastError());
                } else {
                    CK(h, cudaMemset(tail, 0, tot * sizeof(float)));
                }
            }
        }
    CK(h, cudaDeviceSynchronize());
    h->st_cap = std::max(h->st_cap, n);
    h->n_streams = n;
    h->enc_slots.bit.assign(n, 0);
    h->dec_slots.bit.assign(n, 0);
    return 0;
}

int adec_set_streams(adec_handle* h, int n) {
    if (!h || !h->finalized) return h ? h->fail("not finalized") : 1;
    if (n == h->n_streams) return 0;
    if (n < 1) return h->fail("n_streams must be >= 1");
    DeviceGuard dg(h->device);
    return resize_state(h, n, h->n_streams == 1);
}

static int offline_state(adec_handle* h, int B, cudaStream_t s) {
    if (B != h->n_streams && resize_state(h, B, false)) return 1;
    return adec_reset(h, (void*)s);
}

int adec_reset(adec_handle* h, void* stream) {
    if (!h || !h->finalized) return h ? h->fail("not finalized") : 1;
    DeviceGuard dg(h->device);
    for (auto* ops : {&h->enc_ops, &h->dec_ops})
        for (Op& op : *ops) {
            const size_t per = (size_t)op.P * op.st_C;
            if (!per) continue;
            for (int i = 0; i < 2; ++i) CK(h, cudaMemsetAsync(op.st[i], 0, per * h->n_streams * h->act_bytes(), (cudaStream_t)stream));
        }
    for (SlotBits* sb : {&h->enc_slots, &h->dec_slots}) {
        std::fill(sb->bit.begin(), sb->bit.end(), 0);
        sb->dirty = false;
    }
    return 0;
}

int adec_frames_for(const adec_handle* h, int T) {
    if (!h || h->cfg.model_type != ADEC_MODEL_SYMAD) return -1;
    int t = T;
    for (int i = 0; i < h->cfg.n_enc; ++i) t = (t - 1) / h->cfg.enc_strides[i] + 1;
    return t;
}

int adec_hop_length(const adec_handle* h) { return h ? hop_of(h) : -1; }

int adec_encode(adec_handle* h, const float* x, int B, int T, float* z, void* stream) {
    if (!h || !h->finalized) return h ? h->fail("not finalized") : 1;
    if (h->cfg.model_type != ADEC_MODEL_SYMAD) return h->fail("encode: not a symAD handle");
    if (B < 1 || T < 1) return h->fail("encode: empty input");
    DeviceGuard dg(h->device);
    RunCtx rc{B, x, z, (cudaStream_t)stream};
    return run_ops(h, h->enc_ops, rc, T, nullptr);
}

static int varlen_args(adec_handle* h, const char* name, const int* lengths, int B) {
    if (B < 1) return h->fail(fmt("%s: B must be >= 1, got %d", name, B));
    if (!lengths) return h->fail(fmt("%s: lengths is NULL", name));
    for (int b = 0; b < B; ++b)
        if (lengths[b] < 1) return h->fail(fmt("%s: utterance %d has length %d; every length must be >= 1", name, b, lengths[b]));
    return 0;
}

static int stream_args(adec_handle* h, const char* name, const int* streams, int B) {
    if (!streams) return h->fail(fmt("%s: streams is NULL", name));
    std::vector<char> seen(h->n_streams, 0);
    for (int b = 0; b < B; ++b) {
        const int s = streams[b];
        if (s < 0 || s >= h->n_streams)
            return h->fail(fmt("%s: stream %d (entry %d) is out of range [0, %d) (call adec_set_streams)", name, s, b, h->n_streams));
        if (seen[s]) return h->fail(fmt("%s: stream %d is listed twice; each stream advances by one chunk per call", name, s));
        seen[s] = 1;
    }
    return 0;
}

static int decode_common(adec_handle* h, const void* zq, int B, int F, void* y, void* stream, bool offline, bool bf16_io,
                         bool vl = false, const int* vl_frames = nullptr, const int* slots = nullptr, bool slot_call = false) {
    if (!h || !h->finalized) return h ? h->fail("not finalized") : 1;
    const char* base = slot_call ? "decode_streams" : vl ? "decode_offline_varlen" : offline ? "decode_offline" : "decode";
    const std::string name = std::string(base) + (bf16_io ? "_bf16" : "");
    if (h->act_bf16 && !bf16_io)
        return h->fail(fmt("%s: this handle has bf16 activations (compute_dtype 2); call adec_%s_bf16 with bf16 zq / y", name.c_str(), base));
    if (!h->act_bf16 && bf16_io)
        return h->fail(fmt("%s: this handle has fp32 activations (compute_dtype %d); call adec_%s with fp32 zq / y", name.c_str(),
                           h->cfg.compute_dtype, base));
    if (bf16_io && (((uintptr_t)zq | (uintptr_t)y) & 15)) return h->fail(fmt("%s: zq and y must be 16-byte aligned", name.c_str()));
    if (vl) {
        if (varlen_args(h, name.c_str(), vl_frames, B)) return 1;
        if (slot_call && stream_args(h, name.c_str(), slots, B)) return 1;
    } else if (B < 1 || F < 1) {
        return h->fail(fmt("%s: empty input", name.c_str()));
    }
    DeviceGuard dg(h->device);
    if (offline && !vl && offline_state(h, B, (cudaStream_t)stream)) return 1;
    RunCtx rc{B, (const float*)zq, (float*)y, (cudaStream_t)stream, offline, vl ? vl_frames : nullptr, name.c_str(), slots};
    return run_ops(h, h->dec_ops, rc, vl ? 1 : F, nullptr);
}

int adec_decode(adec_handle* h, const float* zq, int B, int F, float* y, void* stream) {
    return decode_common(h, zq, B, F, y, stream, false, false);
}

int adec_decode_bf16(adec_handle* h, const uint16_t* zq, int B, int F, uint16_t* y, void* stream) {
    return decode_common(h, zq, B, F, y, stream, false, true);
}

int adec_encode_offline(adec_handle* h, const float* x, int B, int T, float* z, void* stream) {
    if (!h || !h->finalized) return h ? h->fail("not finalized") : 1;
    if (h->cfg.model_type != ADEC_MODEL_SYMAD) return h->fail("encode_offline: not a symAD handle");
    if (B < 1 || T < 1) return h->fail("encode_offline: empty input");
    DeviceGuard dg(h->device);
    if (offline_state(h, B, (cudaStream_t)stream)) return 1;
    RunCtx rc{B, x, z, (cudaStream_t)stream, true};
    return run_ops(h, h->enc_ops, rc, T, nullptr);
}

int adec_decode_offline(adec_handle* h, const float* zq, int B, int F, float* y, void* stream) {
    return decode_common(h, zq, B, F, y, stream, true, false);
}

int adec_decode_offline_bf16(adec_handle* h, const uint16_t* zq, int B, int F, uint16_t* y, void* stream) {
    return decode_common(h, zq, B, F, y, stream, true, true);
}

int adec_encode_offline_varlen(adec_handle* h, const float* x, const int* lengths, int B, float* z, void* stream) {
    if (!h || !h->finalized) return h ? h->fail("not finalized") : 1;
    if (h->cfg.model_type != ADEC_MODEL_SYMAD) return h->fail("encode_offline_varlen: not a symAD handle");
    if (varlen_args(h, "encode_offline_varlen", lengths, B)) return 1;
    DeviceGuard dg(h->device);
    RunCtx rc{B, x, z, (cudaStream_t)stream, true, lengths, "encode_offline_varlen"};
    return run_ops(h, h->enc_ops, rc, 1, nullptr);
}

int adec_decode_offline_varlen(adec_handle* h, const float* zq, const int* frames, int B, float* y, void* stream) {
    return decode_common(h, zq, B, 0, y, stream, true, false, true, frames);
}

int adec_decode_offline_varlen_bf16(adec_handle* h, const uint16_t* zq, const int* frames, int B, uint16_t* y, void* stream) {
    return decode_common(h, zq, B, 0, y, stream, true, true, true, frames);
}

int adec_encode_streams(adec_handle* h, const float* x, const int* lengths, const int* streams, int B, float* z, void* stream) {
    if (!h || !h->finalized) return h ? h->fail("not finalized") : 1;
    if (h->cfg.model_type != ADEC_MODEL_SYMAD) return h->fail("encode_streams: not a symAD handle");
    if (varlen_args(h, "encode_streams", lengths, B) || stream_args(h, "encode_streams", streams, B)) return 1;
    DeviceGuard dg(h->device);
    RunCtx rc{B, x, z, (cudaStream_t)stream, false, lengths, "encode_streams", streams};
    return run_ops(h, h->enc_ops, rc, 1, nullptr);
}

int adec_decode_streams(adec_handle* h, const float* zq, const int* frames, const int* streams, int B, float* y, void* stream) {
    return decode_common(h, zq, B, 0, y, stream, false, false, true, frames, streams, true);
}

int adec_decode_streams_bf16(adec_handle* h, const uint16_t* zq, const int* frames, const int* streams, int B, uint16_t* y, void* stream) {
    return decode_common(h, zq, B, 0, y, stream, false, true, true, frames, streams, true);
}

int adec_copy_stream_state(adec_handle* h, int src, const int* dst, int n, void* stream) {
    if (!h || !h->finalized) return h ? h->fail("not finalized") : 1;
    if (src < 0 || src >= h->n_streams) return h->fail(fmt("copy_stream_state: src %d is out of range [0, %d)", src, h->n_streams));
    if (n < 0 || (n > 0 && !dst)) return h->fail("copy_stream_state: bad dst list");
    for (int i = 0; i < n; ++i)
        if (dst[i] < 0 || dst[i] >= h->n_streams)
            return h->fail(fmt("copy_stream_state: dst %d (entry %d) is out of range [0, %d)", dst[i], i, h->n_streams));
    DeviceGuard dg(h->device);
    for (auto* ops : {&h->enc_ops, &h->dec_ops}) {
        SlotBits* sb = slot_bits(h, *ops);
        const int sel = sb->bit[src];
        std::vector<int> pairs;
        for (int i = 0; i < n; ++i)
            if (dst[i] != src) { pairs.push_back(src); pairs.push_back(dst[i]); }
        if (slot_copy(h, *ops, pairs, sel, sel, (cudaStream_t)stream)) return 1;
        for (int i = 0; i < n; ++i) sb->bit[dst[i]] = (uint8_t)sel;
        if (sel) sb->dirty = true;
    }
    return 0;
}

static int index_bits(int n) { int b = 1; while ((1 << b) < n) ++b; return b; }

int adec_packed_frame_bytes(const adec_handle* h) {
    if (!h || h->cfg.model_type != ADEC_MODEL_SYMAD) return -1;
    return (h->cfg.codebook_num * index_bits(h->cfg.codebook_size) + 7) / 8;
}

extern "C++" template <int FP>
cudaError_t launch_rvq(const adec_handle* h, RvqArgs a, cudaStream_t s, int* cost) {
    static int per_sm[64] = {0};
    auto kern = rvq_kernel<64, 4, FP>;
    const int dev = h->device;
    const auto smem_of = [&](int n_pass) { const int FR = n_pass * FP; return (size_t)FR * (3 * 64 + 1 + 2 * (RVQ_THREADS / 32) + a.nq) * 4; };
    if (dev < 64 && !per_sm[dev]) {
        cudaFuncSetAttribute(kern, cudaFuncAttributeMaxDynamicSharedMemorySize, 100 * 1024);
        int nb = 0;
        cudaOccupancyMaxActiveBlocksPerMultiprocessor(&nb, kern, RVQ_THREADS, smem_of(2));
        per_sm[dev] = std::max(1, nb);
    }
    const long long nfr = (long long)a.B * a.F, slots = (long long)h->n_sms * per_sm[dev < 64 ? dev : 0];
    int n_pass = (int)((nfr + slots * FP - 1) / (slots * FP));
    n_pass = std::max(1, std::min(n_pass, 96 / FP));
    if (cost) { *cost = n_pass * (FP + 2) * (int)((nfr + slots * n_pass * FP - 1) / (slots * n_pass * FP)); return cudaSuccess; }
    a.n_pass = n_pass;
    const long long FR = (long long)n_pass * FP;
    kern<<<(unsigned)((nfr + FR - 1) / FR), RVQ_THREADS, smem_of(n_pass), s>>>(a);
    return cudaGetLastError();
}

int adec_quantize_ex(adec_handle* h, const float* z, int B, int F, int64_t* idx, uint8_t* packed, float* zq, void* stream) {
    if (!h || !h->finalized) return h ? h->fail("not finalized") : 1;
    if (h->cfg.model_type != ADEC_MODEL_SYMAD) return h->fail("quantize: not a symAD handle");
    if (B < 1 || F < 1) return h->fail("quantize: empty input");
    if (!idx && !packed && !zq) return h->fail("quantize: no output requested");
    DeviceGuard dg(h->device);
    RvqArgs a{};
    a.z = z; a.B = B; a.F = F; a.nq = h->cfg.codebook_num; a.embed = h->d_embed; a.e2 = h->d_e2; a.idx = (long long*)idx;
    a.packed = packed; a.zq = zq; a.bits = index_bits(h->cfg.codebook_size); a.bpf = adec_packed_frame_bytes(h);
    int c16 = 0, c12 = 0, c8 = 0;
    launch_rvq<16>(h, a, nullptr, &c16); launch_rvq<12>(h, a, nullptr, &c12); launch_rvq<8>(h, a, nullptr, &c8);
    cudaError_t e = (c12 <= c16 && c12 <= c8) ? launch_rvq<12>(h, a, (cudaStream_t)stream, nullptr)
                  : (c16 <= c8)               ? launch_rvq<16>(h, a, (cudaStream_t)stream, nullptr)
                                              : launch_rvq<8>(h, a, (cudaStream_t)stream, nullptr);
    if (e != cudaSuccess) return h->fail(fmt("launch of rvq_kernel failed: %s", cudaGetErrorString(e)));
    ++h->launches;
    return 0;
}

int adec_quantize(adec_handle* h, const float* z, int B, int F, int64_t* idx, void* stream) {
    return adec_quantize_ex(h, z, B, F, idx, nullptr, nullptr, stream);
}

static int lookup_common(adec_handle* h, const int64_t* idx, const uint8_t* packed, int B, int F, float* zq, void* stream) {
    if (!h || !h->finalized) return h ? h->fail("not finalized") : 1;
    if (h->cfg.model_type != ADEC_MODEL_SYMAD) return h->fail("lookup: not a symAD handle");
    if (B < 1 || F < 1) return h->fail("lookup: empty input");
    DeviceGuard dg(h->device);
    LookupArgs a{};
    a.idx = (const long long*)idx; a.packed = packed; a.nfr = (long long)B * F; a.nq = h->cfg.codebook_num; a.D = h->cfg.code_dim;
    a.N = h->cfg.codebook_size; a.bits = index_bits(a.N); a.bpf = adec_packed_frame_bytes(h);
    a.codebook = h->d_codebook; a.n_rows = (long long)h->cfg.codebook_num * h->cfg.codebook_size; a.zq = zq; a.err = h->d_err;
    const long long nth = a.nfr * (a.D / 4);
    lookup_kernel<<<(unsigned)((nth + 255) / 256), 256, 0, (cudaStream_t)stream>>>(a);
    CK(h, cudaGetLastError());
    ++h->launches;
    return 0;
}

int adec_lookup(adec_handle* h, const int64_t* idx, int B, int F, float* zq, void* stream) {
    return lookup_common(h, idx, nullptr, B, F, zq, stream);
}

int adec_lookup_packed(adec_handle* h, const uint8_t* packed, int B, int F, float* zq, void* stream) {
    return lookup_common(h, nullptr, packed, B, F, zq, stream);
}

int adec_codec_host(adec_handle* enc, adec_handle* dec, const float* x_host, int B, int T, int64_t* idx_host,
                    float* y_host, void* stream) {
    if (!enc || !dec) return 1;
    if (enc->device != dec->device) return enc->fail("codec_host: handles on different devices");
    if (dec->act_bf16) return enc->fail("codec_host: the decoder has bf16 activations (compute_dtype 2), which the host path does not carry; "
                                        "use compute_dtype 0 or 1, or adec_decode_bf16 on device buffers");
    DeviceGuard dg(enc->device);
    cudaStream_t s = (cudaStream_t)stream;
    const int F = adec_frames_for(enc, T);
    if (F < 1) return enc->fail("codec_host: bad T or not a symAD encoder");
    const int D = enc->cfg.code_dim, nq = enc->cfg.codebook_num, hop = hop_of(dec);
    if (ensure(enc, enc->hx, (size_t)B * T) || ensure(enc, enc->hz, (size_t)B * D * F) || ensure(enc, enc->hzq, (size_t)B * F * D) ||
        ensure(enc, enc->hy, (size_t)B * F * hop))
        return 1;
    const size_t nidx = (size_t)nq * B * F;
    if (enc->hidx_cap < nidx) {
        if (enc->hidx) CK(enc, cudaFree(enc->hidx));
        CK(enc, cudaMalloc((void**)&enc->hidx, nidx * sizeof(long long)));
        enc->hidx_cap = nidx;
    }
    CK(enc, cudaMemcpyAsync(enc->hx.p, x_host, (size_t)B * T * sizeof(float), cudaMemcpyHostToDevice, s));
    if (adec_encode(enc, enc->hx.p, B, T, enc->hz.p, stream)) return 1;
    if (adec_quantize_ex(enc, enc->hz.p, B, F, (int64_t*)enc->hidx, nullptr, enc->hzq.p, stream)) return 1;
    if (adec_decode(dec, enc->hzq.p, B, F, enc->hy.p, stream)) { enc->err = dec->err; return 1; }
    if (idx_host) CK(enc, cudaMemcpyAsync(idx_host, enc->hidx, nidx * sizeof(long long), cudaMemcpyDeviceToHost, s));
    CK(enc, cudaMemcpyAsync(y_host, enc->hy.p, (size_t)B * F * hop * sizeof(float), cudaMemcpyDeviceToHost, s));
    CK(enc, cudaStreamSynchronize(s));
    for (adec_handle* hh : {enc, dec}) {
        int herr = 0;
        CK(enc, cudaMemcpy(&herr, hh->d_err, sizeof(int), cudaMemcpyDeviceToHost));
        if (herr) CK(enc, cudaMemset(hh->d_err, 0, sizeof(int)));
        if (herr & 1) return enc->fail("lookup: index out of range");
        if (herr & 2) return enc->fail("an activation left the range of the fp16-split tensor-core engine (|a| >= 6e4); use ADEC_CONV_PATH=tf32");
        if (hh == dec) break;
    }
    return 0;
}

static int pack_common(adec_handle* h, const char* what, int64_t* idx, int B, int F, uint8_t* packed, void* stream, bool pack) {
    if (!h || !h->finalized) return h ? h->fail("not finalized") : 1;
    if (h->cfg.model_type != ADEC_MODEL_SYMAD) return h->fail(std::string(what) + ": not a symAD handle");
    if (B < 1 || F < 1) return h->fail(std::string(what) + ": empty input");
    if (h->cfg.codebook_size < 2 || h->cfg.codebook_size > 65536) return h->fail(std::string(what) + ": codebook_size must be in [2, 65536]");
    DeviceGuard dg(h->device);
    PackArgs a{};
    a.idx = (long long*)idx; a.packed = packed; a.nfr = (long long)B * F; a.nq = h->cfg.codebook_num; a.N = h->cfg.codebook_size;
    a.bits = index_bits(a.N); a.bpf = adec_packed_frame_bytes(h); a.err = h->d_err;
    const unsigned grid = (unsigned)((a.nfr + 255) / 256);
    if (pack) pack_kernel<<<grid, 256, 0, (cudaStream_t)stream>>>(a);
    else unpack_kernel<<<grid, 256, 0, (cudaStream_t)stream>>>(a);
    CK(h, cudaGetLastError());
    ++h->launches;
    return 0;
}

int adec_pack_indices(adec_handle* h, const int64_t* idx, int B, int F, uint8_t* packed, void* stream) {
    return pack_common(h, "pack_indices", const_cast<int64_t*>(idx), B, F, packed, stream, true);
}

int adec_unpack_indices(adec_handle* h, const uint8_t* packed, int B, int F, int64_t* idx, void* stream) {
    return pack_common(h, "unpack_indices", idx, B, F, const_cast<uint8_t*>(packed), stream, false);
}

static int read_flag(adec_handle* h, void* stream, int bit) {
    if (!h || !h->d_err) return -1;
    DeviceGuard dg(h->device);
    int herr = 0;
    if (cudaStreamSynchronize((cudaStream_t)stream) != cudaSuccess ||
        cudaMemcpy(&herr, h->d_err, sizeof(int), cudaMemcpyDeviceToHost) != cudaSuccess) {
        h->fail("CUDA error while reading the device flag word");
        return -1;
    }
    if (herr & bit) {
        const int rest = herr & ~bit;
        if (cudaMemcpy(h->d_err, &rest, sizeof(int), cudaMemcpyHostToDevice) != cudaSuccess) { h->fail("CUDA error while clearing the device flag word"); return -1; }
    }
    return (herr & bit) ? 1 : 0;
}

int adec_index_error(adec_handle* h, void* stream) { return read_flag(h, stream, 1); }
int adec_range_error(adec_handle* h, void* stream) { return read_flag(h, stream, 2); }

int64_t adec_launch_count(const adec_handle* h) { return h ? h->launches : 0; }

int adec_ktrace(adec_handle* h, unsigned long long* out, int max_records) {
    if (!h || !h->d_ktrace || !out) return -1;
    DeviceGuard dg(h->device);
    const int n = std::min(h->ktrace_n, max_records);
    if (cudaDeviceSynchronize() != cudaSuccess || cudaMemcpy(out, h->d_ktrace, (size_t)n * 3 * sizeof(unsigned long long), cudaMemcpyDeviceToHost) != cudaSuccess) return -1;
    h->ktrace_n = 0;
    return n;
}

int adec_probe_mma(int device, int kind, int NT, int n_groups, double* tflops, double* ms) {
    if (!tflops || (kind != 0 && kind != 1) || (NT != 32 && NT != 64 && NT != 128 && NT != 256) || n_groups < 1) { g_create_error = "probe_mma: bad argument"; return 1; }
    int ndev = 0;
    if (cudaGetDeviceCount(&ndev) != cudaSuccess || device < 0 || device >= ndev) { g_create_error = "probe_mma: no usable CUDA device"; return 1; }
    DeviceGuard dg(device);
    int n_sms = 0;
    cudaDeviceGetAttribute(&n_sms, cudaDevAttrMultiProcessorCount, device);
    constexpr int a_pitch_rows = 136;
    const int smem = 8 * 2 * a_pitch_rows * 16 + 8 * 2 * NT * 16;
    auto launch = [&](cudaStream_t s) {
        auto go = [&](auto kern) {
            cudaFuncSetAttribute(kern, cudaFuncAttributeMaxDynamicSharedMemorySize, smem);
            kern<<<n_sms, 256, smem, s>>>(n_groups, a_pitch_rows);
        };
        if (kind == 0) {
            if (NT == 32) go(mma_probe_kernel<32, PREC_TF32>); else if (NT == 64) go(mma_probe_kernel<64, PREC_TF32>);
            else if (NT == 128) go(mma_probe_kernel<128, PREC_TF32>); else go(mma_probe_kernel<256, PREC_TF32>);
        } else {
            if (NT == 32) go(mma_probe_kernel<32, PREC_F16>); else if (NT == 64) go(mma_probe_kernel<64, PREC_F16>);
            else if (NT == 128) go(mma_probe_kernel<128, PREC_F16>); else go(mma_probe_kernel<256, PREC_F16>);
        }
    };
    cudaEvent_t e0, e1;
    cudaEventCreate(&e0); cudaEventCreate(&e1);
    launch(0);
    cudaEventRecord(e0, 0);
    launch(0);
    cudaEventRecord(e1, 0);
    cudaError_t e = cudaEventSynchronize(e1);
    float t = 0.f;
    if (e == cudaSuccess) e = cudaEventElapsedTime(&t, e0, e1);
    cudaEventDestroy(e0); cudaEventDestroy(e1);
    if (e != cudaSuccess || cudaGetLastError() != cudaSuccess) { g_create_error = fmt("probe_mma: %s", cudaGetErrorString(e)); return 1; }
    const double flops = (double)n_sms * n_groups * 12.0 * 2.0 * 128.0 * NT * (kind == 0 ? 8.0 : 16.0);
    *tflops = flops / (t * 1e-3) / 1e12;
    if (ms) *ms = t;
    return 0;
}

int adec_profile(adec_handle* h, int enable) {
    if (!h) return 1;
    for (auto& ev : h->prof_events) { cudaEventDestroy(ev.first); cudaEventDestroy(ev.second); }
    h->prof_events.clear(); h->prof_names.clear(); h->prof_bytes.clear();
    h->profiling = enable != 0;
    return 0;
}

int adec_profile_report(adec_handle* h, char* buf, int buf_len) {
    if (!h || !buf || buf_len < 2) return 1;
    DeviceGuard dg(h->device);
    std::string out;
    for (size_t i = 0; i < h->prof_events.size(); ++i) {
        if (cudaEventSynchronize(h->prof_events[i].second) != cudaSuccess) return h->fail("profile: event sync failed");
        float ms = 0.f;
        cudaEventElapsedTime(&ms, h->prof_events[i].first, h->prof_events[i].second);
        out += fmt("%s\t%.6f\t%.0f\n", h->prof_names[i].c_str(), ms, h->prof_bytes[i]);
    }
    if ((int)out.size() + 1 > buf_len) return h->fail("profile: buffer too small");
    memcpy(buf, out.c_str(), out.size() + 1);
    return 0;
}

static int run_single(adec_handle* h, Op& op, const void* x, int B, int Cin_real, int T, int Cout_real_total, void* state, int P_real,
                      void* y, bool convtr, int stride, const void* res = nullptr, bool offline = false) {
    const size_t eb = h->act_bytes();
    auto put = [eb](void* dst, size_t i, const void* src, size_t j) { memcpy((char*)dst + i * eb, (const char*)src + j * eb, eb); };
    const int G = op.shared_in ? 1 : op.G;
    const int cin_g = Cin_real / G, ldx = G * op.Cin;
    std::vector<char> xl((size_t)B * T * ldx * eb, 0);
    for (int b = 0; b < B; ++b)
        for (int g = 0; g < G; ++g)
            for (int c = 0; c < cin_g; ++c)
                for (int t = 0; t < T; ++t) put(xl.data(), ((size_t)b * T + t) * ldx + g * op.Cin + c, x, ((size_t)b * Cin_real + g * cin_g + c) * T + t);
    const size_t per = (size_t)op.P * op.st_C;
    std::vector<char> hs(per * B * eb, 0);
    if (!offline)
        for (int b = 0; b < B; ++b)
            for (int g = 0; g < G; ++g)
                for (int c = 0; c < cin_g; ++c)
                    for (int p = 0; p < P_real; ++p)
                        put(hs.data(), ((size_t)b * op.P + p) * op.st_C + g * op.Cin + c, state, ((size_t)b * Cin_real + g * cin_g + c) * P_real + p);
    op.in_buf = BUF_EXT_IN; op.ldx = ldx; op.x_goff = op.shared_in ? 0 : op.Cin;
    op.out_buf = BUF_EXT_OUT; op.ldy = op.G * op.Cout; op.y_goff = op.Cout;
    if (finalize_op(h, &op)) return 1;
    for (int i = 0; i < 2; ++i) if (dev_alloc(h, &op.st[i], (per * B * eb + 3) / 4)) return 1;
    CK(h, cudaMemcpy(op.st[0], hs.data(), hs.size(), cudaMemcpyHostToDevice));
    h->n_streams = B;
    const int Tout = (T - 1) / op.down + 1;
    const int cout_g = Cout_real_total / op.G;
    if (res) {
        std::vector<char> rl((size_t)B * Tout * op.ldy * eb, 0);
        for (int b = 0; b < B; ++b)
            for (int g = 0; g < op.G; ++g)
                for (int c = 0; c < cout_g; ++c)
                    for (int t = 0; t < Tout; ++t)
                        put(rl.data(), ((size_t)b * Tout + t) * op.ldy + g * op.Cout + c, res, ((size_t)b * Cout_real_total + g * cout_g + c) * Tout + t);
        if (ensure(h, h->ws[0], (rl.size() + 3) / 4)) return 1;
        CK(h, cudaMemcpy(h->ws[0].p, rl.data(), rl.size(), cudaMemcpyHostToDevice));
        op.res_buf = 0; op.ldr = op.ldy; op.r_goff = op.Cout;
    }
    float *dx, *dy;
    const size_t ybytes = (size_t)B * Tout * op.ldy * eb;
    if (dev_alloc(h, &dx, (xl.size() + 3) / 4) || dev_alloc(h, &dy, (ybytes + 3) / 4)) return 1;
    CK(h, cudaMemcpy(dx, xl.data(), xl.size(), cudaMemcpyHostToDevice));
    std::vector<Op> ops;
    ops.push_back(op);
    RunCtx rc{B, dx, dy, 0, offline};
    if (run_ops(h, ops, rc, T, nullptr)) return 1;
    CK(h, cudaDeviceSynchronize());
    std::vector<char> yl(ybytes), sl(per * B * eb);
    CK(h, cudaMemcpy(yl.data(), dy, yl.size(), cudaMemcpyDeviceToHost));
    CK(h, cudaMemcpy(sl.data(), ops[0].st[ops[0].cur], sl.size(), cudaMemcpyDeviceToHost));
    if (!convtr) {
        for (int b = 0; b < B; ++b)
            for (int g = 0; g < op.G; ++g)
                for (int c = 0; c < cout_g; ++c)
                    for (int t = 0; t < Tout; ++t)
                        put(y, ((size_t)b * Cout_real_total + g * cout_g + c) * Tout + t, yl.data(), ((size_t)b * Tout + t) * op.ldy + g * op.Cout + c);
    } else {
        for (int b = 0; b < B; ++b)
            for (int c = 0; c < Cout_real_total; ++c)
                for (int j = 0; j < Tout; ++j)
                    for (int r = 0; r < stride; ++r)
                        put(y, ((size_t)b * Cout_real_total + c) * Tout * stride + j * stride + r, yl.data(), ((size_t)b * Tout + j) * op.ldy + r * Cout_real_total + c);
    }
    if (!offline)
        for (int b = 0; b < B; ++b)
            for (int g = 0; g < G; ++g)
                for (int c = 0; c < cin_g; ++c)
                    for (int p = 0; p < P_real; ++p)
                        put(state, ((size_t)b * Cin_real + g * cin_g + c) * P_real + p, sl.data(), ((size_t)b * op.P + p) * op.st_C + g * op.Cin + c);
    return 0;
}

int adec_test_causal_conv(int device, const float* x, int B, int Cin, int T, const float* w, const float* bias, int Cout,
                          int K, int stride, int dil, int groups, int pre_act, float slope, float* state, float* y) {
    adec_config cfg{};
    adec_handle* h = nullptr;
    if (adec_create(&cfg, device, &h)) return 1;
    DeviceGuard dg(device);
    HostTensor W, Bt;
    W.shape = {Cout, Cin / groups, K};
    W.data.assign(w, w + (size_t)Cout * (Cin / groups) * K);
    if (bias) { Bt.shape = {Cout}; Bt.data.assign(bias, bias + Cout); }
    Op op;
    int rc = make_conv_op(h, &op, "test_conv", W, bias ? &Bt : nullptr, stride, dil, groups, pre_act, slope, false);
    if (!rc) rc = run_single(h, op, x, B, Cin, T, Cout, state, (K - 1) * dil, y, false, 1);
    if (rc) g_create_error = h->err;
    adec_destroy(h);
    return rc;
}

int adec_test_residual_unit(int device, const float* x, int B, int C, int T, const float* w1, const float* w2, int K, int dil,
                            float* state, float* y) {
    adec_config cfg{};
    adec_handle* h = nullptr;
    if (adec_create(&cfg, device, &h)) return 1;
    DeviceGuard dg(device);
    HostTensor W1, W2;
    W1.shape = {C, C, K};
    W1.data.assign(w1, w1 + (size_t)C * C * K);
    W2.shape = {C, C, 1};
    W2.data.assign(w2, w2 + (size_t)C * C);
    Op op;
    int rc = make_ru_op(h, &op, "test_ru", W1, W2, dil, ACT_ELU);
    if (!rc && h->use_tc && op.Cout > kTcMaxFuse) rc = h->fail("test_ru: C > 128 runs as two ops on the tensor-core path; test those separately");
    if (!rc) rc = run_single(h, op, x, B, C, T, C, state, (K - 1) * dil, y, false, 1);
    if (rc) g_create_error = h->err;
    adec_destroy(h);
    return rc;
}

int adec_test_causal_convtr(int device, const float* x, int B, int Cin, int T, const float* w, const float* bias, int Cout,
                            int stride, float* state, float* y) {
    adec_config cfg{};
    adec_handle* h = nullptr;
    if (adec_create(&cfg, device, &h)) return 1;
    DeviceGuard dg(device);
    HostTensor W, Bt;
    W.shape = {Cin, Cout, 2 * stride};
    W.data.assign(w, w + (size_t)Cin * Cout * 2 * stride);
    if (bias) { Bt.shape = {Cout}; Bt.data.assign(bias, bias + Cout); }
    Op op;
    int rc = make_convtr_op(h, &op, "test_convtr", W, bias ? &Bt : nullptr, stride, ACT_NONE, 0.f);
    if (!rc) rc = run_single(h, op, x, B, Cin, T, Cout, state, 1, y, true, stride);
    if (rc) g_create_error = h->err;
    adec_destroy(h);
    return rc;
}

int adec_test_vocoder_layer(int device, int compute_dtype, int kind, const void* x, int B, int Cin, int T, const float* w,
                            const float* bias, int Cout, int K, int dil, int up, int groups, int shared_in, int pre_act, float slope,
                            const float* mean, const float* scale, const void* res, int offline, void* state, void* y) {
    if (compute_dtype != 1 && compute_dtype != 2) {
        g_create_error = "adec_test_vocoder_layer: compute_dtype must be 1 or 2 (the fp32-grade engines: adec_test_causal_conv / _convtr)";
        return 1;
    }
    adec_config cfg{};
    cfg.model_type = ADEC_MODEL_HIFIGAN;
    cfg.compute_dtype = compute_dtype;
    cfg.in_channels = Cin;
    adec_handle* h = nullptr;
    if (adec_create(&cfg, device, &h)) return 1;
    DeviceGuard dg(device);
    int rc = 0;
    Op op;
    if (!x || !w || !y || B < 1 || T < 1 || (!offline && !state)) {
        rc = h->fail("adec_test_vocoder_layer: NULL x, w, y or (streaming) state, or B / T < 1");
    } else if (kind == 0 && (groups < 1 || Cin % groups || Cout % groups)) {
        rc = h->fail("adec_test_vocoder_layer: Cin and Cout must divide into groups");
    } else if (kind == 0 && pre_act == ACT_NORM && (groups != 1 || !mean || !scale)) {
        rc = h->fail("adec_test_vocoder_layer: norm needs groups = 1, mean and scale");
    } else if (kind == 0) {
        HostTensor W, Bt;
        W.shape = {Cout, Cin / groups, K};
        W.data.assign(w, w + (size_t)Cout * (Cin / groups) * K);
        if (bias) { Bt.shape = {Cout}; Bt.data.assign(bias, bias + Cout); }
        rc = make_conv_op(h, &op, "test_conv", W, bias ? &Bt : nullptr, 1, dil, groups, pre_act, slope, shared_in != 0);
        if (!rc && pre_act == ACT_NORM) {
            std::vector<float> mp(op.Cin, 0.f), sp(op.Cin, 1.f);
            std::copy(mean, mean + Cin, mp.begin());
            std::copy(scale, scale + Cin, sp.begin());
            if (dev_upload(h, &h->d_mean, mp) || dev_upload(h, &h->d_scale, sp)) rc = 1;
            op.mean = h->d_mean; op.scale = h->d_scale;
        }
        if (!rc) rc = run_single(h, op, x, B, shared_in ? Cin / groups : Cin, T, Cout, state, (K - 1) * dil, y, false, 1, res, offline != 0);
    } else if (res) {
        rc = h->fail("adec_test_vocoder_layer: a residual is built for kind 0 only");
    } else if (kind == 1) {
        HostTensor W, Bt;
        W.shape = {Cin, Cout, 2 * up};
        W.data.assign(w, w + (size_t)Cin * Cout * 2 * up);
        if (bias) { Bt.shape = {Cout}; Bt.data.assign(bias, bias + Cout); }
        rc = make_convtr_op(h, &op, "test_convtr", W, bias ? &Bt : nullptr, up, ACT_LRELU, slope);
        if (!rc) rc = run_single(h, op, x, B, Cin, T, Cout, state, 1, y, true, up, nullptr, offline != 0);
    } else if (kind == 2) {
        HostTensor W, Bt;
        W.shape = {Cout, Cin, K};
        W.data.assign(w, w + (size_t)Cout * Cin * K);
        h->tensors["test_head.conv.weight"] = W;
        if (bias) { Bt.shape = {1}; Bt.data.assign(bias, bias + 1); h->tensors["test_head.conv.bias"] = Bt; }
        rc = build_head(h, &op, "test_head", ACT_LRELU, slope, true);
        if (!rc) rc = run_single(h, op, x, B, Cin, T, 1, state, op.P, y, false, 1, nullptr, offline != 0);
    } else {
        rc = h->fail("adec_test_vocoder_layer: kind must be 0 (conv), 1 (transposed conv) or 2 (head)");
    }
    if (rc) g_create_error = h->err;
    adec_destroy(h);
    return rc;
}

}
```

### audiodec_b200/csrc/wg_conv.cuh

```cuda
#pragma once
#include <cuda_bf16.h>
#include <cuda_fp16.h>

#include "kernels.cuh"

namespace adec {

constexpr int TC_TT = 128;
constexpr int TC_CP = 32;
constexpr int TC_MIDP = 128;
constexpr float F16_LO_SCALE = 2048.f;
enum { PREC_BF16 = 1, PREC_TF32 = 2, PREC_F16 = 3 };

__device__ __forceinline__ void fence_async_smem() { asm volatile("fence.proxy.async.shared::cta;" ::: "memory"); }
__device__ __forceinline__ float tf32_rna(float x) {
    uint32_t r;
    asm("cvt.rna.tf32.f32 %0, %1;" : "=r"(r) : "f"(x));
    return __uint_as_float(r);
}

__device__ __forceinline__ uint64_t wg_desc(uint32_t saddr, uint32_t lbo_bytes) {
    return (uint64_t)((saddr & 0x3FFFF) >> 4) | ((uint64_t)((lbo_bytes >> 4) & 0x3FFF) << 16) | ((uint64_t)(128 >> 4) << 32);
}
__device__ __forceinline__ void wg_fence() { asm volatile("wgmma.fence.sync.aligned;" ::: "memory"); }
__device__ __forceinline__ void wg_commit() { asm volatile("wgmma.commit_group.sync.aligned;" ::: "memory"); }
__device__ __forceinline__ void wg_wait0() { asm volatile("wgmma.wait_group.sync.aligned 0;" ::: "memory"); }
template <int N>
__device__ __forceinline__ void wg_fence_regs(float (&d)[N]) {
#pragma unroll
    for (int i = 0; i < N; ++i) asm volatile("" : "+f"(d[i])::"memory");
}

template <int N, int PREC> struct Wgmma;
#define ADEC_WG_N32(PREC, TYPE, TAIL)                                                                                              \
    template <> struct Wgmma<32, PREC> {                                                                                           \
        __device__ __forceinline__ static void mma(float (&d)[16], uint64_t da, uint64_t db, uint32_t acc) {                     \
            asm volatile("{\n .reg .pred p;\n setp.ne.b32 p, %18, 0;\n wgmma.mma_async.sync.aligned.m64n32" TYPE                \
                         " {%0,%1,%2,%3,%4,%5,%6,%7,%8,%9,%10,%11,%12,%13,%14,%15}, %16, %17, p, 1, 1" TAIL ";\n}"                  \
                         : "+f"(d[0]), "+f"(d[1]), "+f"(d[2]), "+f"(d[3]), "+f"(d[4]), "+f"(d[5]), "+f"(d[6]), "+f"(d[7]),          \
                           "+f"(d[8]), "+f"(d[9]), "+f"(d[10]), "+f"(d[11]), "+f"(d[12]), "+f"(d[13]), "+f"(d[14]), "+f"(d[15])     \
                         : "l"(da), "l"(db), "r"(acc));                                                                            \
        }                                                                                                                          \
    };
#define ADEC_WG_N64(PREC, TYPE, TAIL)                                                                                              \
    template <> struct Wgmma<64, PREC> {                                                                                           \
        __device__ __forceinline__ static void mma(float (&d)[32], uint64_t da, uint64_t db, uint32_t acc) {                     \
            asm volatile("{\n .reg .pred p;\n setp.ne.b32 p, %34, 0;\n wgmma.mma_async.sync.aligned.m64n64" TYPE                \
                         " {%0,%1,%2,%3,%4,%5,%6,%7,%8,%9,%10,%11,%12,%13,%14,%15,%16,%17,%18,%19,%20,%21,%22,%23,%24,%25,%26,%27," \
                         "%28,%29,%30,%31}, %32, %33, p, 1, 1" TAIL ";\n}"                                                          \
                         : "+f"(d[0]), "+f"(d[1]), "+f"(d[2]), "+f"(d[3]), "+f"(d[4]), "+f"(d[5]), "+f"(d[6]), "+f"(d[7]),          \
                           "+f"(d[8]), "+f"(d[9]), "+f"(d[10]), "+f"(d[11]), "+f"(d[12]), "+f"(d[13]), "+f"(d[14]), "+f"(d[15]),    \
                           "+f"(d[16]), "+f"(d[17]), "+f"(d[18]), "+f"(d[19]), "+f"(d[20]), "+f"(d[21]), "+f"(d[22]), "+f"(d[23]),  \
                           "+f"(d[24]), "+f"(d[25]), "+f"(d[26]), "+f"(d[27]), "+f"(d[28]), "+f"(d[29]), "+f"(d[30]), "+f"(d[31])   \
                         : "l"(da), "l"(db), "r"(acc));                                                                            \
        }                                                                                                                          \
    };
ADEC_WG_N32(PREC_F16, "k16.f32.f16.f16", ", 0, 0")
ADEC_WG_N32(PREC_BF16, "k16.f32.bf16.bf16", ", 0, 0")
ADEC_WG_N32(PREC_TF32, "k8.f32.tf32.tf32", "")
ADEC_WG_N64(PREC_F16, "k16.f32.f16.f16", ", 0, 0")
ADEC_WG_N64(PREC_BF16, "k16.f32.bf16.bf16", ", 0, 0")
ADEC_WG_N64(PREC_TF32, "k8.f32.tf32.tf32", "")
#undef ADEC_WG_N32
#undef ADEC_WG_N64

template <int NT, int PREC> struct WgCfg {
    static constexpr int EB = PREC == PREC_TF32 ? 4 : 2;
    static constexpr int KBB = TC_CP * EB / 16;
    static constexpr int NPR = PREC == PREC_F16 ? 3 : PREC == PREC_TF32 ? 2 : 1;
    static constexpr int NPL = PREC == PREC_BF16 ? 1 : 2;
    static constexpr int TPG = PREC == PREC_TF32 ? 1 : 2;
    static constexpr int TAP_BYTES = NPR * KBB * NT * 16;
    static constexpr int STAGE_BYTES = TPG * TAP_BYTES;
    static constexpr int MID_BYTES = NPL * (NT * EB / 16) * TC_MIDP * 16;
    __host__ __device__ static constexpr int stages(bool fuse) { return PREC == PREC_TF32 && NT == 128 && fuse ? 1 : NT == 128 ? 2 : 3; }
    static constexpr int PW = NT < 64 ? NT : 64;
    static constexpr int NPROD = 96;
    static constexpr int THREADS = 256 + NPROD + 32;
    __host__ __device__ static constexpr int win_pitch(int wrows) { return ((wrows + 1) & ~3) + 2; }
    __host__ __device__ static constexpr int win_bytes(int wrows) { return NPL * KBB * win_pitch(wrows) * 16; }
    static int n_wbuf(int wrows, bool fuse) {
        const long long avail = 227 * 1024 - 512 - (long long)stages(fuse) * STAGE_BYTES - (fuse ? (long long)MID_BYTES : 0);
        const long long n = avail / win_bytes(wrows);
        return (int)(n > 4 ? 4 : n);
    }
    static size_t smem_bytes(int wrows, bool fuse) {
        return 512 + (size_t)stages(fuse) * STAGE_BYTES + (size_t)n_wbuf(wrows, fuse) * win_bytes(wrows) + (fuse ? (size_t)MID_BYTES : 0);
    }
};

template <int ACT>
__device__ __forceinline__ float4 apply_act_t(float4 v, float slope) {
    if (ACT == ACT_ELU) { v.x = act_elu(v.x); v.y = act_elu(v.y); v.z = act_elu(v.z); v.w = act_elu(v.w); }
    if (ACT == ACT_LRELU) { v.x = act_lrelu(v.x, slope); v.y = act_lrelu(v.y, slope); v.z = act_lrelu(v.z, slope); v.w = act_lrelu(v.w, slope); }
    return v;
}

__device__ __forceinline__ uint32_t h2_bits(__half2 h) { return *reinterpret_cast<const uint32_t*>(&h); }
__device__ __forceinline__ uint32_t b2_bits(__nv_bfloat162 h) { return *reinterpret_cast<const uint32_t*>(&h); }
template <int PREC>
__device__ __forceinline__ void split2(float x, float y, uint2& hi, uint2& lo) {
    if (PREC == PREC_F16) {
        const __half2 h = __floats2half2_rn(x, y);
        const float2 f = __half22float2(h);
        hi.x = h2_bits(h);
        lo.x = h2_bits(__floats2half2_rn((x - f.x) * F16_LO_SCALE, (y - f.y) * F16_LO_SCALE));
    } else if (PREC == PREC_TF32) {
        const float hx = tf32_rna(x), hy = tf32_rna(y);
        hi = make_uint2(__float_as_uint(hx), __float_as_uint(hy));
        lo = make_uint2(__float_as_uint(x - hx), __float_as_uint(y - hy));
    } else {
        hi.x = b2_bits(__floats2bfloat162_rn(x, y));
    }
}
template <int PREC>
__device__ __forceinline__ void split_store(unsigned char* hi, unsigned char* lo, size_t bstride, const float4 u, const float4 v) {
    uint2 h0, l0, h1, l1, h2, l2, h3, l3;
    split2<PREC>(u.x, u.y, h0, l0); split2<PREC>(u.z, u.w, h1, l1);
    split2<PREC>(v.x, v.y, h2, l2); split2<PREC>(v.z, v.w, h3, l3);
    if (PREC == PREC_TF32) {
        *reinterpret_cast<uint4*>(hi) = make_uint4(h0.x, h0.y, h1.x, h1.y);
        *reinterpret_cast<uint4*>(hi + bstride) = make_uint4(h2.x, h2.y, h3.x, h3.y);
        *reinterpret_cast<uint4*>(lo) = make_uint4(l0.x, l0.y, l1.x, l1.y);
        *reinterpret_cast<uint4*>(lo + bstride) = make_uint4(l2.x, l2.y, l3.x, l3.y);
    } else {
        *reinterpret_cast<uint4*>(hi) = make_uint4(h0.x, h1.x, h2.x, h3.x);
        if (PREC == PREC_F16) *reinterpret_cast<uint4*>(lo) = make_uint4(l0.x, l1.x, l2.x, l3.x);
    }
}

struct TileIter {
    int tile, xt, y, b, sx, sy, sb, nx, ny;
    __device__ __forceinline__ TileIter(int first, int step, int n_x, int n_y) {
        nx = n_x; ny = n_y; tile = first;
        xt = first % n_x;
        const int q = first / n_x;
        y = q % n_y; b = q / n_y;
        sx = step % n_x;
        const int sq = step / n_x;
        sy = sq % n_y; sb = sq / n_y;
    }
    __device__ __forceinline__ void next(int step) {
        tile += step;
        xt += sx;
        const int cx = xt >= nx ? 1 : 0;
        xt -= cx ? nx : 0;
        y += sy + cx;
        const int cy = y >= ny ? 1 : 0;
        y -= cy ? ny : 0;
        b += sb + cy;
    }
};

__device__ __forceinline__ float4 norm4(float4 x, const float* mean, const float* scale) {
    const float4 mu = *reinterpret_cast<const float4*>(mean);
    const float4 sc = *reinterpret_cast<const float4*>(scale);
    x.x = __fdiv_rn(x.x - mu.x, sc.x); x.y = __fdiv_rn(x.y - mu.y, sc.y);
    x.z = __fdiv_rn(x.z - mu.z, sc.z); x.w = __fdiv_rn(x.w - mu.w, sc.w);
    return x;
}

template <int NT, int PREC>
__device__ __forceinline__ void wg_group(float (&d)[WgCfg<NT, PREC>::PW / 2], uint32_t a_hi, uint32_t a_lo, uint32_t lbo, uint32_t tap_step,
                                         int ntaps, uint32_t bw) {
    using Cfg = WgCfg<NT, PREC>;
    constexpr int NKS = Cfg::KBB / 2, TPG = Cfg::TPG;
    constexpr uint32_t B_LBO = NT * 16u, B_KS = 2u * NT * 16u, B_T = Cfg::TAP_BYTES, B_PL = Cfg::KBB * NT * 16u;
    constexpr uint32_t PL_SMALL = PREC == PREC_F16 ? 2u : 0u;
    uint32_t acc = 0u;
    wg_fence_regs(d);
    wg_fence();
    if (PREC != PREC_BF16) {
#pragma unroll
        for (int t = 0; t < TPG; ++t)
#pragma unroll
            for (int ks = 0; ks < NKS; ++ks)
                if (t < ntaps) {
                    Wgmma<Cfg::PW, PREC>::mma(d, wg_desc(a_lo + t * tap_step + ks * 2u * lbo, lbo), wg_desc(bw + t * B_T + PL_SMALL * B_PL + ks * B_KS, B_LBO), acc);
                    acc = 1u;
                }
#pragma unroll
        for (int t = 0; t < TPG; ++t)
#pragma unroll
            for (int ks = 0; ks < NKS; ++ks)
                if (t < ntaps) Wgmma<Cfg::PW, PREC>::mma(d, wg_desc(a_hi + t * tap_step + ks * 2u * lbo, lbo), wg_desc(bw + t * B_T + B_PL + ks * B_KS, B_LBO), 1u);
    }
#pragma unroll
    for (int t = 0; t < TPG; ++t)
#pragma unroll
        for (int ks = 0; ks < NKS; ++ks)
            if (t < ntaps) {
                Wgmma<Cfg::PW, PREC>::mma(d, wg_desc(a_hi + t * tap_step + ks * 2u * lbo, lbo), wg_desc(bw + t * B_T + ks * B_KS, B_LBO), acc);
                acc = 1u;
            }
    wg_commit();
    wg_wait0();
    wg_fence_regs(d);
}

template <typename XT>
__device__ __forceinline__ const XT* slot_hist(const ConvArgs& a, int u, int i, int c) {
    const int e = __ldg(a.vl_slot + u);
    const XT* base = reinterpret_cast<const XT*>((e & 1) ? (const void*)a.st_out : (const void*)a.st_in);
    return base + (((e >> 1) * a.P + i) * a.st_ld + c);
}

template <int NT, bool FUSE, int PRE, int PREC, bool BST, bool VL = false>
__global__ void __launch_bounds__(WgCfg<NT, PREC>::THREADS, 1) wg_conv_kernel(const ConvArgs a, int n_xtiles, int n_ytiles, int n_tiles) {
    static_assert(!BST || (PREC == PREC_BF16 && !FUSE), "bf16 storage is built for the non-fused bf16-operand kernels");
    using Cfg = WgCfg<NT, PREC>;
    using XT = typename std::conditional<BST, __nv_bfloat16, float>::type;
    constexpr int S = Cfg::stages(FUSE), CP = TC_CP, TT = TC_TT, KBB = Cfg::KBB, EB = Cfg::EB, TPG = Cfg::TPG, PW = Cfg::PW;
    constexpr int NPROD = Cfg::NPROD, WWARP = (256 + NPROD) / 32;
    constexpr int STAGE_BYTES = Cfg::STAGE_BYTES, TAP_BYTES = Cfg::TAP_BYTES;
    constexpr int NH = NT / PW;
    constexpr int NACC = NT / 2;
    constexpr int MBLK = NT * EB / 16;

    extern __shared__ __align__(128) unsigned char smem_raw[];
    uint64_t* b_full = reinterpret_cast<uint64_t*>(smem_raw);
    uint64_t* b_empty = b_full + S;
    uint64_t* w_full = b_empty + S;
    uint64_t* w_empty = w_full + 4;
    unsigned char* bst = smem_raw + 512;
    const int wrows = TT + (a.Ktaps - 1) * a.dil;
    const int wrp = Cfg::win_pitch(wrows);
    const int win_b = Cfg::win_bytes(wrows);
    unsigned char* wbuf0 = bst + S * STAGE_BYTES;
    unsigned char* mbuf = wbuf0 + (size_t)a.n_wbuf * win_b;

    const int tid = threadIdx.x, lane = tid & 31;
    const int warp = __shfl_sync(0xffffffffu, tid >> 5, 0);
    unsigned long long kt0 = 0;
    long long kc0 = 0;
    if (a.dbg && blockIdx.x == 0 && tid == 0) { asm volatile("mov.u64 %0, %%globaltimer;" : "=l"(kt0)); kc0 = clock64(); }
    if (tid == 0) {
        for (int s = 0; s < S; ++s) { mbar_init(&b_full[s], 1); mbar_init(&b_empty[s], 2); }
        for (int i = 0; i < 4; ++i) { mbar_init(&w_full[i], NPROD); mbar_init(&w_empty[i], 2); }
        mbar_fence_init();
    }
    __syncthreads();
    asm volatile("griddepcontrol.launch_dependents;" ::: "memory");
    if (warp != WWARP) asm volatile("griddepcontrol.wait;" ::: "memory");

    if (warp == WWARP) {
        if (lane == 0) {
            int c = 0;
            auto stream = [&](const unsigned char* base, int pieces, int taps) {
                for (int p = 0; p < pieces; ++p)
                    for (int t0 = 0; t0 < taps; t0 += TPG, ++c) {
                        const int s = c % S, it = c / S;
                        const uint32_t bytes = (uint32_t)(taps - t0 >= TPG ? TPG : taps - t0) * TAP_BYTES;
                        if (it > 0) mbar_wait(&b_empty[s], (it - 1) & 1, 100);
                        mbar_arrive_expect_tx(&b_full[s], bytes);
                        bulk_g2s(bst + s * STAGE_BYTES, base + ((long long)p * taps + t0) * TAP_BYTES, bytes, &b_full[s]);
                    }
            };
            const unsigned char* w1 = reinterpret_cast<const unsigned char*>(a.w);
            const unsigned char* w2 = reinterpret_cast<const unsigned char*>(a.w2);
            for (TileIter it(blockIdx.x, gridDim.x, n_xtiles, n_ytiles); it.tile < n_tiles; it.next(gridDim.x)) {
                stream(w1 + (long long)it.y * a.w_tile_floats * 4, a.n_pieces, a.Ktaps);
                if (FUSE) stream(w2, NT / CP, 1);
            }
        }
    } else if (warp >= 8) {
        const int pt = tid - 256;
        int wb = 0, wround = 0;
        constexpr int RPP = NPROD / 4;
        constexpr int UNR = 6;
        constexpr int UNR_E = VL ? 5 : 6;
        const int c8 = pt & 3, m0 = pt >> 2;
        const size_t bstride = (size_t)wrp * 16;
        const bool halves = a.RG > 1 && a.Cin < 8;
        for (TileIter it(blockIdx.x, gridDim.x, n_xtiles, n_ytiles); it.tile < n_tiles; it.next(gridDim.x)) {
            const int xt = it.xt, y = it.y, b = it.b;
            int g = 0, co_tile = y;
            if (a.n_co_tiles != n_ytiles) { g = y / a.n_co_tiles; co_tile = y - g * a.n_co_tiles; }
            const int j0 = xt * TT;
            const XT* xg = reinterpret_cast<const XT*>(a.x) + (long long)b * a.x_bs + g * a.x_goff;
            const XT* sg = reinterpret_cast<const XT*>(a.st_in) + (long long)b * a.P * a.st_ld + g * a.st_goff;
            const int halo = (a.Ktaps - 1) * a.dil;
            int u0 = 0, u0_start = 0, u0_next = 0, u0_T = 0;
            const XT* xu0 = xg;
            if constexpr (VL) {
                u0 = vl_find(a.vl_out, halo, a.vl_B, j0);
                u0_start = vl_row(a.vl_out, halo, u0);
                u0_next = vl_row(a.vl_out, halo, u0 + 1);
                const int i0 = __ldg(a.vl_in + u0);
                u0_T = __ldg(a.vl_in + u0 + 1) - i0;
                xu0 = xg + (long long)i0 * a.ldx;
            }
            for (int p = 0; p < a.n_pieces; ++p) {
                const int buf = wb;
                const uint32_t wpar = (uint32_t)(wround - 1) & 1u;
                bool waited = wround == 0;
                if (++wb == a.n_wbuf) { wb = 0; ++wround; }
                unsigned char* hi = wbuf0 + (size_t)buf * win_b + (size_t)c8 * (KBB / 4) * bstride;
                unsigned char* lo = hi + (size_t)KBB * bstride;
                const int q = p * CP + c8 * 8;
                int r = 0, ci = q;
                if (a.RG > 1) { r = q >> a.lgCin; ci = q & (a.Cin - 1); }
                long long i_first = (long long)j0 * a.RG + r;
                long long i_last = (long long)(j0 + wrows - 1) * a.RG + r;
                const XT* xb = xg;
                int Tb = a.T;
                bool one_utt = true;
                if constexpr (VL) {
                    i_first = (long long)(j0 - u0_start) * a.RG + r;
                    i_last = (long long)(j0 - u0_start + wrows - 1) * a.RG + r;
                    xb = xu0;
                    Tb = u0_T;
                    one_utt = j0 + wrows <= u0_next;
                }
                if (i_first >= a.P && i_last - a.P < Tb && one_utt && PRE != ACT_NORM && !halves && !a.stack_L) {
                    const XT* xp = xb + ci + (i_first - a.P + (long long)m0 * a.RG) * a.ldx;
                    const long long xstep = (long long)RPP * a.RG * a.ldx;
                    for (int mb = m0; mb < wrows; mb += RPP * UNR, xp += xstep * UNR) {
                        float4 u[UNR], v[UNR];
#pragma unroll
                        for (int k = 0; k < UNR; ++k)
                            if (mb + k * RPP < wrows) ldg8(xp + k * xstep, u[k], v[k]);
                        if (!waited) { mbar_wait(&w_empty[buf], wpar, 500); waited = true; }
#pragma unroll
                        for (int k = 0; k < UNR; ++k) {
                            const int m = mb + k * RPP;
                            if (m < wrows) split_store<PREC>(hi + m * 16, lo + m * 16, bstride, apply_act_t<PRE>(u[k], a.slope), apply_act_t<PRE>(v[k], a.slope));
                        }
                    }
                } else {
                    int ci2 = ci + 4;
                    int vu = u0, vu_start = u0_start, vu_next = u0_next, vu_T = u0_T;
                    const XT* xvu = xu0;
                    for (int mb = m0; mb < wrows; mb += RPP * UNR_E) {
                        float4 u[UNR_E], v[UNR_E];
                        unsigned act = 0u;
#pragma unroll
                        for (int k = 0; k < UNR_E; ++k) {
                            const int m = mb + k * RPP;
                            u[k] = v[k] = make_float4(0.f, 0.f, 0.f, 0.f);
                            if (m < wrows) {
                                int ml = j0 + m;
                                const XT* xs = xg;
                                const XT* ss = sg;
                                bool live = true;
                                if constexpr (VL) {
                                    while (vu + 1 < a.vl_B && ml >= vu_next) {
                                        ++vu;
                                        vu_start = vu_next;
                                        vu_next = vl_row(a.vl_out, halo, vu + 1);
                                        const int i0 = __ldg(a.vl_in + vu);
                                        vu_T = __ldg(a.vl_in + vu + 1) - i0;
                                        xvu = xg + (long long)i0 * a.ldx;
                                    }
                                    ml -= vu_start;
                                    xs = xvu;
                                } else if (a.stack_L) {
                                    const int sm = ml / a.stack_L;
                                    ml -= sm * a.stack_L;
                                    live = sm < a.n_streams;
                                    xs = xg + (long long)sm * a.x_bs;
                                    ss = sg + (long long)sm * a.P * a.st_ld;
                                }
                                if constexpr (BST) {
                                    const long long i = (long long)ml * a.RG + r;
                                    long long ti = i - a.P;
                                    if (a.hist_rep && ti < 0) ti = 0;
                                    if (live) {
                                        if (ti < 0) {
                                            if (!VL) ldg8(ss + i * a.st_ld + ci, u[k], v[k]);
                                            else if (a.vl_slot) ldg8(slot_hist<XT>(a, vu, (int)i, g * a.st_goff + ci), u[k], v[k]);
                                        }
                                        else if (ti < (VL ? vu_T : a.T)) { ldg8(xs + ti * a.ldx + ci, u[k], v[k]); act |= 3u << (2 * k); }
                                    }
                                } else {
#pragma unroll
                                    for (int hf = 0; hf < 2; ++hf) {
                                        int rr = r, cc = ci + 4 * hf;
                                        if (halves) { rr = (q + 4 * hf) >> a.lgCin; cc = (q + 4 * hf) & (a.Cin - 1); if (hf) ci2 = cc; }
                                        const long long i = (long long)ml * a.RG + rr;
                                        long long ti = i - a.P;
                                        if (a.hist_rep && ti < 0) ti = 0;
                                        float4 w4 = make_float4(0.f, 0.f, 0.f, 0.f);
                                        if (live) {
                                            if (ti < 0) {
                                                if (!VL) w4 = __ldg(reinterpret_cast<const float4*>(ss + i * a.st_ld + cc));
                                                else if (a.vl_slot) w4 = ldg4(slot_hist<XT>(a, vu, (int)i, g * a.st_goff + cc));
                                            }
                                            else if (ti < (VL ? vu_T : a.T)) { w4 = __ldg(reinterpret_cast<const float4*>(xs + ti * a.ldx + cc)); act |= 1u << (2 * k + hf); }
                                        }
                                        if (hf) v[k] = w4; else u[k] = w4;
                                    }
                                }
                            }
                        }
                        if (!waited) { mbar_wait(&w_empty[buf], wpar, 500); waited = true; }
#pragma unroll
                        for (int k = 0; k < UNR_E; ++k) {
                            const int m = mb + k * RPP;
                            if (m < wrows) {
                                float4 x0 = u[k], x1 = v[k];
                                if ((act >> (2 * k)) & 1u) x0 = PRE == ACT_NORM ? norm4(x0, a.mean + ci, a.scale + ci) : apply_act_t<PRE>(x0, a.slope);
                                if ((act >> (2 * k)) & 2u) x1 = PRE == ACT_NORM ? norm4(x1, a.mean + ci2, a.scale + ci2) : apply_act_t<PRE>(x1, a.slope);
                                split_store<PREC>(hi + m * 16, lo + m * 16, bstride, x0, x1);
                            }
                        }
                    }
                }
                fence_async_smem();
                mbar_arrive(&w_full[buf]);
            }
            if (!VL && co_tile == 0 && g < a.st_groups && a.P > 0) {
                int s_lo = b, s_hi = b - 1;
                if (a.stack_L) {
                    s_lo = (j0 - (a.Tout - 1) + a.stack_L - 1) / a.stack_L;
                    if (j0 < a.Tout - 1) s_lo = 0;
                    s_hi = (j0 + TT - 1 - (a.Tout - 1)) / a.stack_L;
                    if (j0 + TT - 1 < a.Tout - 1) s_hi = -1;
                    if (s_hi > a.n_streams - 1) s_hi = a.n_streams - 1;
                } else if (xt == (a.Tout - 1) / TT) {
                    s_hi = b;
                }
                for (int sm = s_lo; sm <= s_hi; ++sm) {
                    const XT* xs = reinterpret_cast<const XT*>(a.x) + (long long)sm * a.x_bs + g * a.x_goff;
                    const XT* ss = reinterpret_cast<const XT*>(a.st_in) + (long long)sm * a.P * a.st_ld + g * a.st_goff;
                    XT* so = reinterpret_cast<XT*>(a.st_out) + (long long)sm * a.P * a.st_ld + g * a.st_goff;
                    const int nvec = a.P * (a.Cin / 4);
                    for (int idx = pt; idx < nvec; idx += NPROD) {
                        const int r = idx / (a.Cin / 4);
                        const int cc = (idx - r * (a.Cin / 4)) * 4;
                        const long long i = (long long)a.T + r;
                        float4 w4;
                        if (i < a.P) {
                            w4 = ld4(ss + i * a.st_ld + cc);
                        } else {
                            w4 = ldg4(xs + (i - a.P) * a.ldx + cc);
                            if (PRE == ACT_NORM) w4 = norm4(w4, a.mean + cc, a.scale + cc);
                            else w4 = apply_act_t<PRE>(w4, a.slope);
                        }
                        st4(so + (long long)r * a.st_ld + cc, w4);
                    }
                }
            }
        }
        if (VL && a.vl_slot && a.P > 0) {
            const long long per = (long long)a.P * a.st_ld;
            const int nvec = a.P * (a.Cin / 4);
            for (int w = blockIdx.x; w < a.vl_B * a.st_groups; w += gridDim.x) {
                const int g = w / a.vl_B, u = w - g * a.vl_B;
                const int i0 = __ldg(a.vl_in + u), Tu = __ldg(a.vl_in + u + 1) - i0;
                const XT* xs = reinterpret_cast<const XT*>(a.x) + (long long)i0 * a.ldx + g * a.x_goff;
                const XT* ss = slot_rows(a.vl_slot, u, reinterpret_cast<const XT*>(a.st_in) + g * a.st_goff,
                                         reinterpret_cast<XT*>(a.st_out) + g * a.st_goff, per, true);
                XT* so = slot_rows(a.vl_slot, u, reinterpret_cast<const XT*>(a.st_in) + g * a.st_goff,
                                   reinterpret_cast<XT*>(a.st_out) + g * a.st_goff, per, false);
                for (int idx = pt; idx < nvec; idx += NPROD) {
                    const int r = idx / (a.Cin / 4);
                    const int cc = (idx - r * (a.Cin / 4)) * 4;
                    const long long i = (long long)Tu + r;
                    float4 w4;
                    if (i < a.P) {
                        w4 = ldg4(ss + i * a.st_ld + cc);
                    } else {
                        w4 = ldg4(xs + (i - a.P) * a.ldx + cc);
                        if (PRE == ACT_NORM) w4 = norm4(w4, a.mean + cc, a.scale + cc);
                        else w4 = apply_act_t<PRE>(w4, a.slope);
                    }
                    st4(so + (long long)r * a.st_ld + cc, w4);
                }
            }
        }
    } else {
        const int wg = warp >> 2;
        const int wrow = 64 * wg + 16 * (warp & 3) + (lane >> 2), col2 = 2 * (lane & 3);
        const uint32_t row0_off = (uint32_t)(64 * wg) * 16u;
        const uint32_t wbuf0_u = smem_u32(wbuf0), mbuf_u = smem_u32(mbuf), bst_u = smem_u32(bst);
        const uint32_t lbo1 = (uint32_t)wrp * 16u, lbo2 = (uint32_t)TC_MIDP * 16u;
        const uint32_t tap_step = (uint32_t)a.dil * 16u;
        float racc[NACC];
        float part[PW / 2];
#pragma unroll
        for (int i = 0; i < PW / 2; ++i) part[i] = 0.f;
        int c = 0, wb = 0, wround = 0;
        float vmax = 0.f;
        auto group = [&](uint32_t a_hi, uint32_t a_lo, uint32_t lbo, uint32_t row_off, int ntaps) {
            const int s = c % S;
            mbar_wait(&b_full[s], (c / S) & 1, 300);
            const uint32_t bw = bst_u + (uint32_t)s * STAGE_BYTES;
#pragma unroll
            for (int h = 0; h < NH; ++h) {
                wg_group<NT, PREC>(part, a_hi + row_off, a_lo + row_off, lbo, tap_step, ntaps, bw + (uint32_t)h * PW * 16u);
#pragma unroll
                for (int i = 0; i < PW / 2; ++i) racc[h * (PW / 2) + i] = __fadd_rn(racc[h * (PW / 2) + i], part[i]);
            }
            if (threadIdx.x % 128 == 0) mbar_arrive(&b_empty[s]);
            ++c;
        };
        for (TileIter it(blockIdx.x, gridDim.x, n_xtiles, n_ytiles); it.tile < n_tiles; it.next(gridDim.x)) {
            const int xt = it.xt, y = it.y, b = it.b;
            int g = 0, co_tile = y;
            if (a.n_co_tiles != n_ytiles) { g = y / a.n_co_tiles; co_tile = y - g * a.n_co_tiles; }
            const int j0 = xt * TT;
#pragma unroll
            for (int i = 0; i < NACC; ++i) racc[i] = 0.f;
            for (int p = 0; p < a.n_pieces; ++p) {
                const int buf = wb;
                mbar_wait(&w_full[buf], wround & 1, 200);
                if (++wb == a.n_wbuf) { wb = 0; ++wround; }
                const uint32_t a_hi = wbuf0_u + (uint32_t)buf * (uint32_t)win_b;
                for (int t0 = 0; t0 < a.Ktaps; t0 += TPG)
                    group(a_hi, a_hi + (uint32_t)KBB * lbo1, lbo1, row0_off + (uint32_t)t0 * tap_step, a.Ktaps - t0 >= TPG ? TPG : a.Ktaps - t0);
                if (threadIdx.x % 128 == 0) mbar_arrive(&w_empty[buf]);
            }
            if (FUSE) {
#pragma unroll
                for (int i = 0; i < NACC; i += 4) {
                    const float4 m4 = apply_act_t<PRE>(make_float4(racc[i] * a.w_scale, racc[i + 1] * a.w_scale, racc[i + 2] * a.w_scale, racc[i + 3] * a.w_scale), a.slope);
                    racc[i] = m4.x; racc[i + 1] = m4.y; racc[i + 2] = m4.z; racc[i + 3] = m4.w;
                    vmax = fmaxf(vmax, fmaxf(fmaxf(fabsf(m4.x), fabsf(m4.y)), fmaxf(fabsf(m4.z), fabsf(m4.w))));
                }
#pragma unroll
                for (int i = 0; i < NACC; i += 2) {
                    const int h = i / (PW / 2), fi = i % (PW / 2);
                    const int co = h * PW + 8 * (fi >> 2) + col2, row = wrow + 8 * ((fi >> 1) & 1);
                    const int blk = co * EB / 16, off = (co * EB) & 15;
                    unsigned char* hp = mbuf + ((size_t)blk * TC_MIDP + row) * 16 + off;
                    uint2 hi, lo;
                    split2<PREC>(racc[i], racc[i + 1], hi, lo);
                    if (PREC == PREC_TF32) {
                        *reinterpret_cast<uint2*>(hp) = hi;
                        *reinterpret_cast<uint2*>(hp + (size_t)MBLK * TC_MIDP * 16) = lo;
                    } else {
                        *reinterpret_cast<uint32_t*>(hp) = hi.x;
                        if (PREC == PREC_F16) *reinterpret_cast<uint32_t*>(hp + (size_t)MBLK * TC_MIDP * 16) = lo.x;
                    }
                }
                fence_async_smem();
                named_bar_sync(1 + wg, 128);
#pragma unroll
                for (int i = 0; i < NACC; ++i) racc[i] = 0.f;
                for (int p = 0; p < NT / CP; ++p) {
                    const uint32_t m_hi = mbuf_u + (uint32_t)(p * KBB) * lbo2;
                    group(m_hi, m_hi + (uint32_t)MBLK * lbo2, lbo2, row0_off, 1);
                }
            }
            const float oscale = FUSE ? a.w2_scale : a.w_scale;
            int vu = 0, vu_start = 0, vu_next = 0;
            const int halo = (a.Ktaps - 1) * a.dil;
            if constexpr (VL) {
                vu = vl_find(a.vl_out, halo, a.vl_B, j0 + wrow);
                vu_start = vl_row(a.vl_out, halo, vu);
                vu_next = vl_row(a.vl_out, halo, vu + 1);
            }
#pragma unroll
            for (int hr = 0; hr < 2; ++hr) {
                int bo = b, t = j0 + wrow + 8 * hr;
                if constexpr (VL) {
                    while (vu + 1 < a.vl_B && t >= vu_next) { ++vu; vu_start = vu_next; vu_next = vl_row(a.vl_out, halo, vu + 1); }
                    const int o0 = __ldg(a.vl_out + vu), ml = t - vu_start;
                    if (ml >= __ldg(a.vl_out + vu + 1) - o0) continue;
                    t = o0 + ml;
                } else {
                    if (a.stack_L) { bo = t / a.stack_L; t -= bo * a.stack_L; }
                    if (!(t < a.Tout && bo < a.n_streams)) continue;
                }
#pragma unroll
                for (int i = 2 * hr; i < NACC; i += 4) {
                    const int h = i / (PW / 2), fi = i % (PW / 2);
                    const int co_l = co_tile * NT + h * PW + 8 * (fi >> 2) + col2;
                    if (co_l >= a.Cout_g) continue;
                    float v0 = racc[i] * oscale, v1 = racc[i + 1] * oscale;
                    if (a.bias) {
                        const float2 b2 = __ldg(reinterpret_cast<const float2*>(a.bias + g * a.Cout_g + co_l));
                        v0 += b2.x; v1 += b2.y;
                    }
                    if (a.res) {
                        const float2 r2 = ldg2(reinterpret_cast<const XT*>(a.res) + (long long)bo * a.res_bs + (long long)t * a.ldr + g * a.r_goff + co_l);
                        v0 = r2.x + v0; v1 = r2.y + v1;
                    }
                    vmax = fmaxf(vmax, fmaxf(fabsf(v0), fabsf(v1)));
                    if (a.out_nct) {
                        XT* yp = reinterpret_cast<XT*>(a.y) + (long long)bo * a.y_bs + (long long)(g * a.y_goff + co_l) * a.Tout + t;
                        st1(yp, v0);
                        st1(yp + a.Tout, v1);
                    } else {
                        st2(reinterpret_cast<XT*>(a.y) + (long long)bo * a.y_bs + (long long)t * a.ldy + g * a.y_goff + co_l, v0, v1);
                    }
                }
            }
        }
        if (PREC == PREC_F16 && a.err && !(vmax < 60000.f)) atomicOr(a.err, 2);
    }
    if (a.dbg && blockIdx.x == 0 && tid == 0) {
        unsigned long long kt1;
        asm volatile("mov.u64 %0, %%globaltimer;" : "=l"(kt1));
        a.dbg[0] = kt0; a.dbg[1] = kt1; a.dbg[2] = (unsigned long long)(clock64() - kc0);
    }
}

__device__ float g_probe_sink;
template <int NT, int PREC>
__global__ void __launch_bounds__(256) mma_probe_kernel(int n_groups, int a_pitch_rows) {
    using Cfg = WgCfg<NT, PREC>;
    constexpr int PW = Cfg::PW, KSTEPS = 8;
    extern __shared__ __align__(128) unsigned char smem[];
    const int a_bytes = KSTEPS * 2 * a_pitch_rows * 16;
    for (int i = threadIdx.x; i < a_bytes / 16 + KSTEPS * 2 * NT; i += 256) reinterpret_cast<uint4*>(smem)[i] = make_uint4(0u, 0u, 0u, 0u);
    fence_async_smem();
    __syncthreads();
    const int wg = threadIdx.x >> 7;
    const uint32_t a_u = smem_u32(smem) + (uint32_t)(64 * wg) * 16u, b_u = smem_u32(smem + a_bytes);
    const uint32_t a_lbo = (uint32_t)a_pitch_rows * 16u, b_lbo = (uint32_t)NT * 16u;
    float d[PW / 2];
#pragma unroll
    for (int i = 0; i < PW / 2; ++i) d[i] = 0.f;
    float sink = 0.f;
    for (int g = 0; g < n_groups; ++g) {
#pragma unroll 1
        for (int h = 0; h < NT / PW; ++h) {
            wg_fence_regs(d);
            wg_fence();
#pragma unroll
            for (int k = 0; k < 12; ++k) {
                const uint32_t ks = (uint32_t)((g * 12 + k) % KSTEPS);
                Wgmma<PW, PREC>::mma(d, wg_desc(a_u + ks * 2u * a_lbo, a_lbo), wg_desc(b_u + ks * 2u * b_lbo + (uint32_t)h * PW * 16u, b_lbo), k ? 1u : 0u);
            }
            wg_commit();
            wg_wait0();
            wg_fence_regs(d);
            sink += d[0];
        }
    }
    if (sink != 0.f) g_probe_sink = sink;
}

}
```

### include/audiodec_b200.h

```cpp
#ifndef AUDIODEC_B200_H
#define AUDIODEC_B200_H

#include <stdint.h>

#ifdef __cplusplus
extern "C" {
#endif

#define ADEC_MAX_STAGES 8

typedef struct adec_handle adec_handle;

enum adec_model_type {
    ADEC_MODEL_SYMAD = 0,
    ADEC_MODEL_HIFIGAN = 1
};

typedef struct adec_config {
    int model_type;
    int input_channels, output_channels, encode_channels, decode_channels;
    int code_dim, codebook_num, codebook_size;
    int n_enc;  int enc_ratios[ADEC_MAX_STAGES];  int enc_strides[ADEC_MAX_STAGES];
    int n_dec;  int dec_ratios[ADEC_MAX_STAGES];  int dec_strides[ADEC_MAX_STAGES];
    int bias;
    int in_channels, out_channels, channels, kernel_size;
    int n_up;   int upsample_scales[ADEC_MAX_STAGES];  int upsample_kernel_sizes[ADEC_MAX_STAGES];
    int resblock_kernel_size;
    int n_dil;  int resblock_dilations[ADEC_MAX_STAGES];
    int groups;
    float negative_slope;
    int use_weight_norm;
    int has_stats;
    int codec_activate;
    int n_resblocks;  int resblock_kernel_sizes[ADEC_MAX_STAGES];
    int compute_dtype;
} adec_config;

int adec_create(const adec_config *cfg, int device, adec_handle **out);
void adec_destroy(adec_handle *h);
const char *adec_last_error(const adec_handle *h);

int adec_set_tensor(adec_handle *h, const char *key, const float *data, const int64_t *shape, int ndim);
int adec_finalize(adec_handle *h);

int adec_n_streams(const adec_handle *h);
int adec_set_streams(adec_handle *h, int n_streams);
int adec_reset(adec_handle *h, void *stream);

int adec_encode(adec_handle *h, const float *x, int B, int T, float *z, void *stream);
int adec_quantize(adec_handle *h, const float *z, int B, int F, int64_t *idx, void *stream);
int adec_quantize_ex(adec_handle *h, const float *z, int B, int F, int64_t *idx, uint8_t *packed, float *zq, void *stream);
int adec_lookup(adec_handle *h, const int64_t *idx, int B, int F, float *zq, void *stream);
int adec_decode(adec_handle *h, const float *zq, int B, int F, float *y, void *stream);

int adec_decode_bf16(adec_handle *h, const uint16_t *zq, int B, int F, uint16_t *y, void *stream);

int adec_encode_offline(adec_handle *h, const float *x, int B, int T, float *z, void *stream);
int adec_decode_offline(adec_handle *h, const float *zq, int B, int F, float *y, void *stream);
int adec_decode_offline_bf16(adec_handle *h, const uint16_t *zq, int B, int F, uint16_t *y, void *stream);

int adec_encode_offline_varlen(adec_handle *h, const float *x, const int *lengths, int B, float *z, void *stream);
int adec_decode_offline_varlen(adec_handle *h, const float *zq, const int *frames, int B, float *y, void *stream);
int adec_decode_offline_varlen_bf16(adec_handle *h, const uint16_t *zq, const int *frames, int B, uint16_t *y, void *stream);

int adec_encode_streams(adec_handle *h, const float *x, const int *lengths, const int *streams, int B, float *z, void *stream);
int adec_decode_streams(adec_handle *h, const float *zq, const int *frames, const int *streams, int B, float *y, void *stream);
int adec_decode_streams_bf16(adec_handle *h, const uint16_t *zq, const int *frames, const int *streams, int B, uint16_t *y, void *stream);
int adec_copy_stream_state(adec_handle *h, int src, const int *dst, int n, void *stream);

int adec_frames_for(const adec_handle *h, int T);
int adec_hop_length(const adec_handle *h);

int adec_codec_host(adec_handle *enc, adec_handle *dec, const float *x_host, int B, int T,
                    int64_t *idx_host, float *y_host, void *stream);

int adec_packed_frame_bytes(const adec_handle *h);
int adec_pack_indices(adec_handle *h, const int64_t *idx, int B, int F, uint8_t *packed, void *stream);
int adec_unpack_indices(adec_handle *h, const uint8_t *packed, int B, int F, int64_t *idx, void *stream);
int adec_lookup_packed(adec_handle *h, const uint8_t *packed, int B, int F, float *zq, void *stream);
int adec_index_error(adec_handle *h, void *stream);
int adec_range_error(adec_handle *h, void *stream);

int64_t adec_launch_count(const adec_handle *h);

int adec_ktrace(adec_handle *h, unsigned long long *out, int max_records);

int adec_probe_mma(int device, int kind, int NT, int n_groups, double *tflops, double *ms);

int adec_profile(adec_handle *h, int enable);
int adec_profile_report(adec_handle *h, char *buf, int buf_len);

int adec_test_causal_conv(int device, const float *x, int B, int Cin, int T, const float *w, const float *bias,
                          int Cout, int K, int stride, int dil, int groups, int pre_act, float slope,
                          float *state, float *y);
int adec_test_causal_convtr(int device, const float *x, int B, int Cin, int T, const float *w, const float *bias,
                            int Cout, int stride, float *state, float *y);

int adec_test_residual_unit(int device, const float *x, int B, int C, int T, const float *w1, const float *w2,
                            int K, int dil, float *state, float *y);

int adec_test_vocoder_layer(int device, int compute_dtype, int kind, const void *x, int B, int Cin, int T,
                            const float *w, const float *bias, int Cout, int K, int dil, int up, int groups, int shared_in,
                            int pre_act, float slope, const float *mean, const float *scale, const void *res, int offline,
                            void *state, void *y);

#ifdef __cplusplus
}
#endif
#endif
```

Before: 147.7 million.

## Add paired-tap wgmma kernel for fused fp16 RU(32) residual units

Adds a PAIR variant of the fused NT=32 fp16-split residual-unit kernel. Weights for adjacent taps are repacked into a doubled output width (2*Cout), so one wgmma of N=64 computes two time-shifted outputs at once, and the time window is reorganised into dilation blocks. The aim is to use wider MMA instructions and fewer tap iterations for small-channel convs, which are poorly served by N=32 wgmma. The cost is extra weight memory, a more complex window indexing, more pipeline stages and a new epilogue path. A wgmma column test helper is also added.

```diff
diff --git a/audiodec_b200/_lib.py b/audiodec_b200/_lib.py
--- a/audiodec_b200/_lib.py
+++ b/audiodec_b200/_lib.py
@@ -78,6 +78,7 @@
     "adec_test_causal_conv": (c_int, [c_int, c_void_p, c_int, c_int, c_int, c_void_p, c_void_p, c_int, c_int, c_int,
                                       c_int, c_int, c_int, c_float, c_void_p, c_void_p]),
     "adec_test_residual_unit": (c_int, [c_int, c_void_p, c_int, c_int, c_int, c_void_p, c_void_p, c_int, c_int, c_void_p, c_void_p]),
+    "adec_test_wgmma_columns": (c_int, [c_int, c_void_p, c_void_p, c_void_p, c_void_p]),
     "adec_test_causal_convtr": (c_int, [c_int, c_void_p, c_int, c_int, c_int, c_void_p, c_void_p, c_int, c_int,
                                         c_void_p, c_void_p]),
     "adec_test_vocoder_layer": (c_int, [c_int, c_int, c_int, c_void_p, c_int, c_int, c_int, c_void_p, c_void_p, c_int, c_int, c_int,
diff --git a/audiodec_b200/csrc/adec.cu b/audiodec_b200/csrc/adec.cu
--- a/audiodec_b200/csrc/adec.cu
+++ b/audiodec_b200/csrc/adec.cu
@@ -84,12 +84,12 @@
 }
 
 typedef cudaError_t (*TcPersistFn)(const ConvArgs&, int, int, int, int, int, cudaStream_t);
-template <int NT, bool F, int PRE, int PREC, bool BST, bool VL>
+template <int NT, bool F, int PRE, int PREC, bool BST, bool VL, bool PAIR = false>
 cudaError_t launch_wg(const ConvArgs& a, int n_xtiles, int n_ytiles, int n_tiles, int n_ctas, int smem_bytes, cudaStream_t s) {
     static bool configured[64] = {false};
     int dev = 0;
     cudaGetDevice(&dev);
-    auto kern = wg_conv_kernel<NT, F, PRE, PREC, BST, VL>;
+    auto kern = wg_conv_kernel<NT, F, PRE, PREC, BST, VL, PAIR>;
     constexpr int kMaxDyn = 227 * 1024;
     if (dev < 64 && !configured[dev]) {
         cudaError_t e = cudaFuncSetAttribute(kern, cudaFuncAttributeMaxDynamicSharedMemorySize, kMaxDyn);
@@ -110,12 +110,17 @@
     cfg.numAttrs = pdl ? 1 : 0;
     return cudaLaunchKernelEx(&cfg, kern, a, n_xtiles, n_ytiles, n_tiles);
 }
-typedef size_t (*TcSmemFn)(int, bool);
-typedef int (*TcWbufFn)(int, bool);
-struct TcKernelCfg { int NT; bool fuse; int pre, prec; bool bst; int tap_bytes; TcPersistFn pfn, pfn_vl; TcSmemFn smem; TcWbufFn n_wbuf; };
+typedef size_t (*TcSmemFn)(int, bool, bool);
+typedef int (*TcWbufFn)(int, bool, bool);
+template <int NT, bool F, int PRE, int PREC, bool BST>
+constexpr TcPersistFn pair_fn() {
+    if constexpr (NT == 32 && F && PREC == PREC_F16 && !BST) return launch_wg<NT, F, PRE, PREC, BST, false, true>;
+    else return nullptr;
+}
+struct TcKernelCfg { int NT; bool fuse; int pre, prec; bool bst; int tap_bytes; TcPersistFn pfn, pfn_vl, pfn_pair; TcSmemFn smem; TcWbufFn n_wbuf; };
 #define ADEC_TC1(NT, F, PRE, PREC, BST) \
     {NT, F, PRE, PREC, BST, WgCfg<NT, PREC>::TAP_BYTES, launch_wg<NT, F, PRE, PREC, BST, false>, launch_wg<NT, F, PRE, PREC, BST, true>, \
-     WgCfg<NT, PREC>::smem_bytes, WgCfg<NT, PREC>::n_wbuf}
+     pair_fn<NT, F, PRE, PREC, BST>(), WgCfg<NT, PREC>::smem_bytes, WgCfg<NT, PREC>::n_wbuf}
 #define ADEC_TC_FP32(NT, PREC) \
     ADEC_TC1(NT, true, ACT_ELU, PREC, false), ADEC_TC1(NT, false, ACT_NONE, PREC, false), ADEC_TC1(NT, false, ACT_ELU, PREC, false), \
     ADEC_TC1(NT, false, ACT_LRELU, PREC, false), ADEC_TC1(NT, false, ACT_NORM, PREC, false)
@@ -167,6 +172,7 @@
     float w_scale = 1.f, w2_scale = 1.f;
     int n_pieces = 1, n_co_tiles = 1;
     float *w = nullptr, *w2 = nullptr, *bias = nullptr;
+    float* w_pair = nullptr;
     const float *mean = nullptr, *scale = nullptr;
     float head_bias = 0.f;
     long long w_tile_floats = 0;
@@ -461,19 +467,19 @@
         }
         *p_out = p;
     };
-    auto pack = [&](const float* weff, int G, int ntiles, int pieces, int taps, int cin_eff, int cout, int p2, std::vector<float>* out) {
-        std::vector<uint16_t> img((size_t)G * ntiles * pieces * taps * tap_bytes / 2, 0);
+    auto pack = [&](const float* weff, int G, int ntiles, int pieces, int taps, int cin_eff, int cout, int p2, int ntw, std::vector<float>* out) {
+        std::vector<uint16_t> img((size_t)G * ntiles * pieces * taps * npl * KB * ntw * 8, 0);
         size_t o = 0;
         for (int g = 0; g < G; ++g)
             for (int nt = 0; nt < ntiles; ++nt)
                 for (int pc = 0; pc < pieces; ++pc)
                     for (int tap = 0; tap < taps; ++tap) {
                         for (int kb = 0; kb < KB; ++kb)
-                            for (int n = 0; n < NT; ++n)
+                            for (int n = 0; n < ntw; ++n)
                                 for (int e = 0; e < 8; ++e) {
                                     const int k = pc * CP + kb * 8 + e;
-                                    const float w = nt * NT + n < cout ? weff[(((size_t)g * taps + tap) * cin_eff + k) * cout + nt * NT + n] : 0.f;
-                                    const size_t at = o + ((size_t)kb * NT + n) * 8 + e, plane = (size_t)KB * NT * 8;
+                                    const float w = nt * ntw + n < cout ? weff[(((size_t)g * taps + tap) * cin_eff + k) * cout + nt * ntw + n] : 0.f;
+                                    const size_t at = o + ((size_t)kb * ntw + n) * 8 + e, plane = (size_t)KB * ntw * 8;
                                     if (prec == PREC_F16) {
                                         const float ws = std::ldexp(w, p2);
                                         const uint16_t hi = half_bits(ws);
@@ -484,7 +490,7 @@
                                         img[at] = bf16_bits(w);
                                     }
                                 }
-                        o += (size_t)npl * KB * NT * 8;
+                        o += (size_t)npl * KB * ntw * 8;
                     }
         out->assign((img.size() + 1) / 2, 0.f);
         memcpy(out->data(), img.data(), img.size() * 2);
@@ -493,13 +499,27 @@
     if (prec == PREC_F16) pow2_scale(op->weff, &p1);
     op->w_scale = std::ldexp(1.0f, -p1);
     std::vector<float> packed;
-    pack(op->weff.data(), op->G, op->n_co_tiles, op->n_pieces, op->Ktaps, op->Cin_eff, op->Cout, p1, &packed);
+    pack(op->weff.data(), op->G, op->n_co_tiles, op->n_pieces, op->Ktaps, op->Cin_eff, op->Cout, p1, NT, &packed);
     if (dev_upload(h, &op->w, packed)) return 1;
+    if (op->tc->pfn_pair && op->Ktaps % 2 == 1) {
+        const int C = op->Cout, Ci = op->Cin_eff, K = op->Ktaps;
+        std::vector<float> wp((size_t)(K + 1) * Ci * 2 * C, 0.f);
+        for (int j = 0; j <= K; ++j)
+            for (int ci = 0; ci < Ci; ++ci)
+                for (int co = 0; co < C; ++co) {
+                    float* row = wp.data() + ((size_t)j * Ci + ci) * 2 * C;
+                    if (j < K) row[co] = op->weff[((size_t)j * Ci + ci) * C + co];
+                    if (j > 0) row[C + co] = op->weff[((size_t)(j - 1) * Ci + ci) * C + co];
+                }
+        std::vector<float> pkp;
+        pack(wp.data(), 1, 1, op->n_pieces, K + 1, Ci, 2 * C, p1, 2 * NT, &pkp);
+        if (dev_upload(h, &op->w_pair, pkp)) return 1;
+    }
     if (op->fuse) {
         pow2_scale(op->weff2, &p2);
         op->w2_scale = std::ldexp(1.0f, -p2);
         std::vector<float> pk2;
-        pack(op->weff2.data(), 1, 1, op->Cout / CP, 1, op->Cout, op->Cout, p2, &pk2);
+        pack(op->weff2.data(), 1, 1, op->Cout / CP, 1, op->Cout, op->Cout, p2, NT, &pk2);
         if (dev_upload(h, &op->w2, pk2)) return 1;
     }
     if (!op->hbias.empty() && dev_upload(h, &op->bias, op->hbias)) return 1;
@@ -761,7 +781,7 @@
             a.w_scale = op.w_scale; a.w2_scale = op.w2_scale; a.err = h->d_err;
             if (h->d_ktrace && h->ktrace_n < 4096) a.dbg = h->d_ktrace + 3 * (size_t)(h->ktrace_n++);
             if (op.tc) {
-                const int wrows = TC_TT + (op.Ktaps - 1) * op.dil;
+                int wrows = TC_TT + (op.Ktaps - 1) * op.dil;
                 dim3 grid((Tout + TC_TT - 1) / TC_TT, op.G * op.n_co_tiles, rc.B);
                 a.n_streams = rc.B;
                 if (vl) {
@@ -777,12 +797,18 @@
                         grid = dim3((unsigned)stacked, grid.y, 1);
                     }
                 }
+                const bool pair = op.w_pair && !vl && !a.stack_L;
+                if (pair) {
+                    a.w = op.w_pair;
+                    wrows = 2 * pair_rows(op.Ktaps, op.dil);
+                    grid.x = (unsigned)((Tout + pair_tt(op.dil) - 1) / pair_tt(op.dil));
+                }
                 const long long n_tiles = (long long)grid.x * grid.y * grid.z;
                 const int n_ctas = (int)std::min<long long>(n_tiles, h->n_sms);
-                const size_t psmem = op.tc->smem(wrows, op.fuse);
-                a.n_wbuf = op.tc->n_wbuf(wrows, op.fuse);
+                const size_t psmem = op.tc->smem(wrows, op.fuse, pair);
+                a.n_wbuf = op.tc->n_wbuf(wrows, op.fuse, pair);
                 if (a.n_wbuf < 1) return h->fail(fmt("%s: window of %d rows does not fit in shared memory", op.name.c_str(), wrows));
-                e = (vl ? op.tc->pfn_vl : op.tc->pfn)(a, (int)grid.x, (int)grid.y, (int)n_tiles, n_ctas, (int)psmem, rc.stream);
+                e = (vl ? op.tc->pfn_vl : pair ? op.tc->pfn_pair : op.tc->pfn)(a, (int)grid.x, (int)grid.y, (int)n_tiles, n_ctas, (int)psmem, rc.stream);
             } else {
                 const int TT = op.kc->TT;
                 dim3 grid((Tout + TT - 1) / TT, op.G * op.n_co_tiles, rc.B);
@@ -1669,6 +1695,31 @@
     return 0;
 }
 
+int adec_test_wgmma_columns(int device, const void* a, const void* b, float* d64, float* d32) {
+    if (!a || !b || !d64 || !d32) { g_create_error = "test_wgmma_columns: NULL argument"; return 1; }
+    int ndev = 0;
+    if (cudaGetDeviceCount(&ndev) != cudaSuccess || device < 0 || device >= ndev) { g_create_error = "test_wgmma_columns: no usable CUDA device"; return 1; }
+    DeviceGuard dg(device);
+    const size_t na = 2 * 4 * 64 * 16, nb = 3 * 4 * 64 * 16, nd = 64 * 64 * sizeof(float);
+    void* buf = nullptr;
+    cudaError_t e = cudaMalloc(&buf, na + nb + 2 * nd);
+    if (e == cudaSuccess) {
+        char* p = static_cast<char*>(buf);
+        e = cudaMemcpy(p, a, na, cudaMemcpyHostToDevice);
+        if (e == cudaSuccess) e = cudaMemcpy(p + na, b, nb, cudaMemcpyHostToDevice);
+        if (e == cudaSuccess) {
+            wgmma_cols_kernel<<<1, 128>>>(reinterpret_cast<const uint4*>(p), reinterpret_cast<const uint4*>(p + na),
+                                          reinterpret_cast<float*>(p + na + nb), reinterpret_cast<float*>(p + na + nb + nd));
+            e = cudaGetLastError();
+        }
+        if (e == cudaSuccess) e = cudaMemcpy(d64, p + na + nb, nd, cudaMemcpyDeviceToHost);
+        if (e == cudaSuccess) e = cudaMemcpy(d32, p + na + nb + nd, nd, cudaMemcpyDeviceToHost);
+        cudaFree(buf);
+    }
+    if (e != cudaSuccess) { g_create_error = fmt("test_wgmma_columns: %s", cudaGetErrorString(e)); return 1; }
+    return 0;
+}
+
 int adec_profile(adec_handle* h, int enable) {
     if (!h) return 1;
     for (auto& ev : h->prof_events) { cudaEventDestroy(ev.first); cudaEventDestroy(ev.second); }
diff --git a/audiodec_b200/csrc/wg_conv.cuh b/audiodec_b200/csrc/wg_conv.cuh
--- a/audiodec_b200/csrc/wg_conv.cuh
+++ b/audiodec_b200/csrc/wg_conv.cuh
@@ -69,25 +69,30 @@
     static constexpr int KBB = TC_CP * EB / 16;
     static constexpr int NPR = PREC == PREC_F16 ? 3 : PREC == PREC_TF32 ? 2 : 1;
     static constexpr int NPL = PREC == PREC_BF16 ? 1 : 2;
-    static constexpr int TPG = PREC == PREC_TF32 ? 1 : 2;
+    __host__ __device__ static constexpr int tpg(bool fuse) { return PREC == PREC_TF32 || (PREC == PREC_F16 && NT == 32 && fuse) ? 1 : 2; }
     static constexpr int TAP_BYTES = NPR * KBB * NT * 16;
-    static constexpr int STAGE_BYTES = TPG * TAP_BYTES;
-    static constexpr int MID_BYTES = NPL * (NT * EB / 16) * TC_MIDP * 16;
-    __host__ __device__ static constexpr int stages(bool fuse) { return PREC == PREC_TF32 && NT == 128 && fuse ? 1 : NT == 128 ? 2 : 3; }
+    __host__ __device__ static constexpr int stage_bytes(bool fuse) { return tpg(fuse) * TAP_BYTES; }
+    __host__ __device__ static constexpr int mid_bytes(bool pair) { return NPL * (NT * EB / 16) * TC_MIDP * (pair ? 2 : 1) * 16; }
+    __host__ __device__ static constexpr int stages(bool fuse, bool pair) { return pair ? 9 : PREC == PREC_TF32 && NT == 128 && fuse ? 1 : NT == 128 ? 2 : 3; }
+    __host__ __device__ static constexpr int stage_alloc(bool fuse, bool pair) { return pair ? 2 * TAP_BYTES : stage_bytes(fuse); }
     static constexpr int PW = NT < 64 ? NT : 64;
     static constexpr int NPROD = 96;
     static constexpr int THREADS = 256 + NPROD + 32;
     __host__ __device__ static constexpr int win_pitch(int wrows) { return ((wrows + 1) & ~3) + 2; }
     __host__ __device__ static constexpr int win_bytes(int wrows) { return NPL * KBB * win_pitch(wrows) * 16; }
-    static int n_wbuf(int wrows, bool fuse) {
-        const long long avail = 227 * 1024 - 512 - (long long)stages(fuse) * STAGE_BYTES - (fuse ? (long long)MID_BYTES : 0);
+    static int n_wbuf(int wrows, bool fuse, bool pair) {
+        const long long avail = 227 * 1024 - 512 - (long long)stages(fuse, pair) * stage_alloc(fuse, pair) - (fuse ? (long long)mid_bytes(pair) : 0);
         const long long n = avail / win_bytes(wrows);
         return (int)(n > 4 ? 4 : n);
     }
-    static size_t smem_bytes(int wrows, bool fuse) {
-        return 512 + (size_t)stages(fuse) * STAGE_BYTES + (size_t)n_wbuf(wrows, fuse) * win_bytes(wrows) + (fuse ? (size_t)MID_BYTES : 0);
+    static size_t smem_bytes(int wrows, bool fuse, bool pair) {
+        return 512 + (size_t)stages(fuse, pair) * stage_alloc(fuse, pair) + (size_t)n_wbuf(wrows, fuse, pair) * win_bytes(wrows) +
+               (fuse ? (size_t)mid_bytes(pair) : 0);
     }
 };
+
+__host__ __device__ constexpr int pair_tt(int dil) { return 2 * dil * (TC_TT / dil); }
+__host__ __device__ constexpr int pair_rows(int K, int dil) { return TC_TT + (K - 1) / 2 * dil; }
 
 template <int ACT>
 __device__ __forceinline__ float4 apply_act_t(float4 v, float slope) {
@@ -160,11 +165,11 @@
     return x;
 }
 
-template <int NT, int PREC>
+template <int NT, int PREC, int TPG>
 __device__ __forceinline__ void wg_group(float (&d)[WgCfg<NT, PREC>::PW / 2], uint32_t a_hi, uint32_t a_lo, uint32_t lbo, uint32_t tap_step,
                                          int ntaps, uint32_t bw) {
     using Cfg = WgCfg<NT, PREC>;
-    constexpr int NKS = Cfg::KBB / 2, TPG = Cfg::TPG;
+    constexpr int NKS = Cfg::KBB / 2;
     constexpr uint32_t B_LBO = NT * 16u, B_KS = 2u * NT * 16u, B_T = Cfg::TAP_BYTES, B_PL = Cfg::KBB * NT * 16u;
     constexpr uint32_t PL_SMALL = PREC == PREC_F16 ? 2u : 0u;
     uint32_t acc = 0u;
@@ -205,17 +210,19 @@
     return base + (((e >> 1) * a.P + i) * a.st_ld + c);
 }
 
-template <int NT, bool FUSE, int PRE, int PREC, bool BST, bool VL = false>
+template <int NT, bool FUSE, int PRE, int PREC, bool BST, bool VL = false, bool PAIR = false>
 __global__ void __launch_bounds__(WgCfg<NT, PREC>::THREADS, 1) wg_conv_kernel(const ConvArgs a, int n_xtiles, int n_ytiles, int n_tiles) {
     static_assert(!BST || (PREC == PREC_BF16 && !FUSE), "bf16 storage is built for the non-fused bf16-operand kernels");
+    static_assert(!PAIR || (NT == 32 && FUSE && PREC == PREC_F16 && !BST && !VL), "the paired kernel is built for the fused fp16-split RU(32)");
     using Cfg = WgCfg<NT, PREC>;
     using XT = typename std::conditional<BST, __nv_bfloat16, float>::type;
-    constexpr int S = Cfg::stages(FUSE), CP = TC_CP, TT = TC_TT, KBB = Cfg::KBB, EB = Cfg::EB, TPG = Cfg::TPG, PW = Cfg::PW;
+    constexpr int S = Cfg::stages(FUSE, PAIR), CP = TC_CP, TT = TC_TT, KBB = Cfg::KBB, EB = Cfg::EB, TPG = Cfg::tpg(FUSE), PW = Cfg::PW;
     constexpr int NPROD = Cfg::NPROD, WWARP = (256 + NPROD) / 32;
-    constexpr int STAGE_BYTES = Cfg::STAGE_BYTES, TAP_BYTES = Cfg::TAP_BYTES;
+    constexpr int STAGE_BYTES = Cfg::stage_alloc(FUSE, PAIR), TAP_BYTES = Cfg::TAP_BYTES;
     constexpr int NH = NT / PW;
-    constexpr int NACC = NT / 2;
+    constexpr int NACC = PAIR ? NT : NT / 2;
     constexpr int MBLK = NT * EB / 16;
+    constexpr int MIDP = PAIR ? 2 * TC_MIDP : TC_MIDP;
 
     extern __shared__ __align__(128) unsigned char smem_raw[];
     uint64_t* b_full = reinterpret_cast<uint64_t*>(smem_raw);
@@ -223,11 +230,21 @@
     uint64_t* w_full = b_empty + S;
     uint64_t* w_empty = w_full + 4;
     unsigned char* bst = smem_raw + 512;
-    const int wrows = TT + (a.Ktaps - 1) * a.dil;
-    const int wrp = Cfg::win_pitch(wrows);
-    const int win_b = Cfg::win_bytes(wrows);
+    const int ttile = PAIR ? pair_tt(a.dil) : TT;
+    const int wrows = ttile + (a.Ktaps - 1) * a.dil;
+    const int prows = PAIR ? pair_rows(a.Ktaps, a.dil) : 0;
+    const int wrp = Cfg::win_pitch(PAIR ? 2 * prows : wrows);
+    const int win_b = Cfg::win_bytes(PAIR ? 2 * prows : wrows);
     unsigned char* wbuf0 = bst + S * STAGE_BYTES;
     unsigned char* mbuf = wbuf0 + (size_t)a.n_wbuf * win_b;
+    auto srow = [&](int m) -> int {
+        if constexpr (PAIR) {
+            const int blk = m / a.dil;
+            return (blk & 1) * prows + (blk >> 1) * a.dil + (m - blk * a.dil);
+        } else {
+            return m;
+        }
+    };
 
     const int tid = threadIdx.x, lane = tid & 31;
     const int warp = __shfl_sync(0xffffffffu, tid >> 5, 0);
@@ -246,21 +263,21 @@
     if (warp == WWARP) {
         if (lane == 0) {
             int c = 0;
-            auto stream = [&](const unsigned char* base, int pieces, int taps) {
+            auto stream = [&](const unsigned char* base, int pieces, int taps, int tap_bytes) {
                 for (int p = 0; p < pieces; ++p)
                     for (int t0 = 0; t0 < taps; t0 += TPG, ++c) {
                         const int s = c % S, it = c / S;
-                        const uint32_t bytes = (uint32_t)(taps - t0 >= TPG ? TPG : taps - t0) * TAP_BYTES;
+                        const uint32_t bytes = (uint32_t)(taps - t0 >= TPG ? TPG : taps - t0) * tap_bytes;
                         if (it > 0) mbar_wait(&b_empty[s], (it - 1) & 1, 100);
                         mbar_arrive_expect_tx(&b_full[s], bytes);
-                        bulk_g2s(bst + s * STAGE_BYTES, base + ((long long)p * taps + t0) * TAP_BYTES, bytes, &b_full[s]);
+                        bulk_g2s(bst + s * STAGE_BYTES, base + ((long long)p * taps + t0) * tap_bytes, bytes, &b_full[s]);
                     }
             };
             const unsigned char* w1 = reinterpret_cast<const unsigned char*>(a.w);
             const unsigned char* w2 = reinterpret_cast<const unsigned char*>(a.w2);
             for (TileIter it(blockIdx.x, gridDim.x, n_xtiles, n_ytiles); it.tile < n_tiles; it.next(gridDim.x)) {
-                stream(w1 + (long long)it.y * a.w_tile_floats * 4, a.n_pieces, a.Ktaps);
-                if (FUSE) stream(w2, NT / CP, 1);
+                stream(w1 + (long long)it.y * a.w_tile_floats * 4, a.n_pieces, PAIR ? a.Ktaps + 1 : a.Ktaps, PAIR ? 2 * TAP_BYTES : TAP_BYTES);
+                if (FUSE) stream(w2, NT / CP, 1, TAP_BYTES);
             }
         }
     } else if (warp >= 8) {
@@ -276,7 +293,7 @@
             const int xt = it.xt, y = it.y, b = it.b;
             int g = 0, co_tile = y;
             if (a.n_co_tiles != n_ytiles) { g = y / a.n_co_tiles; co_tile = y - g * a.n_co_tiles; }
-            const int j0 = xt * TT;
+            const int j0 = xt * ttile;
             const XT* xg = reinterpret_cast<const XT*>(a.x) + (long long)b * a.x_bs + g * a.x_goff;
             const XT* sg = reinterpret_cast<const XT*>(a.st_in) + (long long)b * a.P * a.st_ld + g * a.st_goff;
             const int halo = (a.Ktaps - 1) * a.dil;
@@ -324,7 +341,7 @@
 #pragma unroll
                         for (int k = 0; k < UNR; ++k) {
                             const int m = mb + k * RPP;
-                            if (m < wrows) split_store<PREC>(hi + m * 16, lo + m * 16, bstride, apply_act_t<PRE>(u[k], a.slope), apply_act_t<PRE>(v[k], a.slope));
+                            if (m < wrows) split_store<PREC>(hi + srow(m) * 16, lo + srow(m) * 16, bstride, apply_act_t<PRE>(u[k], a.slope), apply_act_t<PRE>(v[k], a.slope));
                         }
                     }
                 } else {
@@ -401,7 +418,7 @@
                                 float4 x0 = u[k], x1 = v[k];
                                 if ((act >> (2 * k)) & 1u) x0 = PRE == ACT_NORM ? norm4(x0, a.mean + ci, a.scale + ci) : apply_act_t<PRE>(x0, a.slope);
                                 if ((act >> (2 * k)) & 2u) x1 = PRE == ACT_NORM ? norm4(x1, a.mean + ci2, a.scale + ci2) : apply_act_t<PRE>(x1, a.slope);
-                                split_store<PREC>(hi + m * 16, lo + m * 16, bstride, x0, x1);
+                                split_store<PREC>(hi + srow(m) * 16, lo + srow(m) * 16, bstride, x0, x1);
                             }
                         }
                     }
@@ -414,10 +431,10 @@
                 if (a.stack_L) {
                     s_lo = (j0 - (a.Tout - 1) + a.stack_L - 1) / a.stack_L;
                     if (j0 < a.Tout - 1) s_lo = 0;
-                    s_hi = (j0 + TT - 1 - (a.Tout - 1)) / a.stack_L;
-                    if (j0 + TT - 1 < a.Tout - 1) s_hi = -1;
+                    s_hi = (j0 + ttile - 1 - (a.Tout - 1)) / a.stack_L;
+                    if (j0 + ttile - 1 < a.Tout - 1) s_hi = -1;
                     if (s_hi > a.n_streams - 1) s_hi = a.n_streams - 1;
-                } else if (xt == (a.Tout - 1) / TT) {
+                } else if (xt == (a.Tout - 1) / ttile) {
                     s_hi = b;
                 }
                 for (int sm = s_lo; sm <= s_hi; ++sm) {
@@ -474,12 +491,14 @@
         const int wrow = 64 * wg + 16 * (warp & 3) + (lane >> 2), col2 = 2 * (lane & 3);
         const uint32_t row0_off = (uint32_t)(64 * wg) * 16u;
         const uint32_t wbuf0_u = smem_u32(wbuf0), mbuf_u = smem_u32(mbuf), bst_u = smem_u32(bst);
-        const uint32_t lbo1 = (uint32_t)wrp * 16u, lbo2 = (uint32_t)TC_MIDP * 16u;
+        const uint32_t lbo1 = (uint32_t)wrp * 16u, lbo2 = (uint32_t)MIDP * 16u;
         const uint32_t tap_step = (uint32_t)a.dil * 16u;
+        constexpr int NPART = PAIR ? PW : PW / 2;
         float racc[NACC];
-        float part[PW / 2];
-#pragma unroll
-        for (int i = 0; i < PW / 2; ++i) part[i] = 0.f;
+        float part[NPART];
+        float (&part_h)[PW / 2] = *reinterpret_cast<float (*)[PW / 2]>(part);
+#pragma unroll
+        for (int i = 0; i < NPART; ++i) part[i] = 0.f;
         int c = 0, wb = 0, wround = 0;
         float vmax = 0.f;
         auto group = [&](uint32_t a_hi, uint32_t a_lo, uint32_t lbo, uint32_t row_off, int ntaps) {
@@ -488,18 +507,29 @@
             const uint32_t bw = bst_u + (uint32_t)s * STAGE_BYTES;
 #pragma unroll
             for (int h = 0; h < NH; ++h) {
-                wg_group<NT, PREC>(part, a_hi + row_off, a_lo + row_off, lbo, tap_step, ntaps, bw + (uint32_t)h * PW * 16u);
-#pragma unroll
-                for (int i = 0; i < PW / 2; ++i) racc[h * (PW / 2) + i] = __fadd_rn(racc[h * (PW / 2) + i], part[i]);
+                wg_group<NT, PREC, TPG>(part_h, a_hi + row_off, a_lo + row_off, lbo, tap_step, ntaps, bw + (uint32_t)h * PW * 16u);
+#pragma unroll
+                for (int i = 0; i < PW / 2; ++i) racc[h * (PW / 2) + i] = __fadd_rn(racc[h * (PW / 2) + i], part_h[i]);
             }
             if (threadIdx.x % 128 == 0) mbar_arrive(&b_empty[s]);
             ++c;
+        };
+        auto pgroup = [&](uint32_t a_hi, uint32_t a_lo, uint32_t row_off) {
+            if constexpr (PAIR) {
+                const int s = c % S;
+                mbar_wait(&b_full[s], (c / S) & 1, 300);
+                wg_group<2 * NT, PREC, 1>(part, a_hi + row_off, a_lo + row_off, lbo1, tap_step, 1, bst_u + (uint32_t)s * STAGE_BYTES);
+#pragma unroll
+                for (int i = 0; i < NACC; ++i) racc[i] = __fadd_rn(racc[i], part[i]);
+                if (threadIdx.x % 128 == 0) mbar_arrive(&b_empty[s]);
+                ++c;
+            }
         };
         for (TileIter it(blockIdx.x, gridDim.x, n_xtiles, n_ytiles); it.tile < n_tiles; it.next(gridDim.x)) {
             const int xt = it.xt, y = it.y, b = it.b;
             int g = 0, co_tile = y;
             if (a.n_co_tiles != n_ytiles) { g = y / a.n_co_tiles; co_tile = y - g * a.n_co_tiles; }
-            const int j0 = xt * TT;
+            const int j0 = xt * ttile;
 #pragma unroll
             for (int i = 0; i < NACC; ++i) racc[i] = 0.f;
             for (int p = 0; p < a.n_pieces; ++p) {
@@ -507,40 +537,66 @@
                 mbar_wait(&w_full[buf], wround & 1, 200);
                 if (++wb == a.n_wbuf) { wb = 0; ++wround; }
                 const uint32_t a_hi = wbuf0_u + (uint32_t)buf * (uint32_t)win_b;
-                for (int t0 = 0; t0 < a.Ktaps; t0 += TPG)
-                    group(a_hi, a_hi + (uint32_t)KBB * lbo1, lbo1, row0_off + (uint32_t)t0 * tap_step, a.Ktaps - t0 >= TPG ? TPG : a.Ktaps - t0);
+                if constexpr (PAIR) {
+                    for (int j = 0; j <= a.Ktaps; ++j)
+                        pgroup(a_hi, a_hi + (uint32_t)KBB * lbo1, row0_off + (uint32_t)((j & 1) * prows + (j >> 1) * a.dil) * 16u);
+                } else {
+                    for (int t0 = 0; t0 < a.Ktaps; t0 += TPG)
+                        group(a_hi, a_hi + (uint32_t)KBB * lbo1, lbo1, row0_off + (uint32_t)t0 * tap_step, a.Ktaps - t0 >= TPG ? TPG : a.Ktaps - t0);
+                }
                 if (threadIdx.x % 128 == 0) mbar_arrive(&w_empty[buf]);
             }
             if (FUSE) {
+                const bool ok0 = !PAIR || wrow < ttile / 2, ok8 = !PAIR || wrow + 8 < ttile / 2;
 #pragma unroll
                 for (int i = 0; i < NACC; i += 4) {
                     const float4 m4 = apply_act_t<PRE>(make_float4(racc[i] * a.w_scale, racc[i + 1] * a.w_scale, racc[i + 2] * a.w_scale, racc[i + 3] * a.w_scale), a.slope);
                     racc[i] = m4.x; racc[i + 1] = m4.y; racc[i + 2] = m4.z; racc[i + 3] = m4.w;
-                    vmax = fmaxf(vmax, fmaxf(fmaxf(fabsf(m4.x), fabsf(m4.y)), fmaxf(fabsf(m4.z), fabsf(m4.w))));
+                    if (PAIR) {
+                        if (ok0) vmax = fmaxf(vmax, fmaxf(fabsf(m4.x), fabsf(m4.y)));
+                        if (ok8) vmax = fmaxf(vmax, fmaxf(fabsf(m4.z), fabsf(m4.w)));
+                    } else {
+                        vmax = fmaxf(vmax, fmaxf(fmaxf(fabsf(m4.x), fabsf(m4.y)), fmaxf(fabsf(m4.z), fabsf(m4.w))));
+                    }
                 }
 #pragma unroll
                 for (int i = 0; i < NACC; i += 2) {
-                    const int h = i / (PW / 2), fi = i % (PW / 2);
-                    const int co = h * PW + 8 * (fi >> 2) + col2, row = wrow + 8 * ((fi >> 1) & 1);
+                    const int h = PAIR ? 0 : i / (PW / 2), fi = PAIR ? i : i % (PW / 2);
+                    int co = h * PW + 8 * (fi >> 2) + col2, row = wrow + 8 * ((fi >> 1) & 1);
+                    if (PAIR) { row += (co / NT) * TC_MIDP; co %= NT; }
                     const int blk = co * EB / 16, off = (co * EB) & 15;
-                    unsigned char* hp = mbuf + ((size_t)blk * TC_MIDP + row) * 16 + off;
+                    unsigned char* hp = mbuf + ((size_t)blk * MIDP + row) * 16 + off;
                     uint2 hi, lo;
                     split2<PREC>(racc[i], racc[i + 1], hi, lo);
                     if (PREC == PREC_TF32) {
                         *reinterpret_cast<uint2*>(hp) = hi;
-                        *reinterpret_cast<uint2*>(hp + (size_t)MBLK * TC_MIDP * 16) = lo;
+                        *reinterpret_cast<uint2*>(hp + (size_t)MBLK * MIDP * 16) = lo;
                     } else {
                         *reinterpret_cast<uint32_t*>(hp) = hi.x;
-                        if (PREC == PREC_F16) *reinterpret_cast<uint32_t*>(hp + (size_t)MBLK * TC_MIDP * 16) = lo.x;
+                        if (PREC == PREC_F16) *reinterpret_cast<uint32_t*>(hp + (size_t)MBLK * MIDP * 16) = lo.x;
                     }
                 }
                 fence_async_smem();
                 named_bar_sync(1 + wg, 128);
 #pragma unroll
                 for (int i = 0; i < NACC; ++i) racc[i] = 0.f;
-                for (int p = 0; p < NT / CP; ++p) {
-                    const uint32_t m_hi = mbuf_u + (uint32_t)(p * KBB) * lbo2;
-                    group(m_hi, m_hi + (uint32_t)MBLK * lbo2, lbo2, row0_off, 1);
+                if constexpr (PAIR) {
+                    const int s = c % S;
+                    mbar_wait(&b_full[s], (c / S) & 1, 300);
+#pragma unroll
+                    for (int hh = 0; hh < 2; ++hh) {
+                        const uint32_t m_hi = mbuf_u + row0_off + (uint32_t)(hh * TC_MIDP * 16);
+                        wg_group<NT, PREC, 1>(part_h, m_hi, m_hi + (uint32_t)MBLK * lbo2, lbo2, tap_step, 1, bst_u + (uint32_t)s * STAGE_BYTES);
+#pragma unroll
+                        for (int i = 0; i < PW / 2; ++i) racc[hh * (PW / 2) + i] = __fadd_rn(racc[hh * (PW / 2) + i], part_h[i]);
+                    }
+                    if (threadIdx.x % 128 == 0) mbar_arrive(&b_empty[s]);
+                    ++c;
+                } else {
+                    for (int p = 0; p < NT / CP; ++p) {
+                        const uint32_t m_hi = mbuf_u + (uint32_t)(p * KBB) * lbo2;
+                        group(m_hi, m_hi + (uint32_t)MBLK * lbo2, lbo2, row0_off, 1);
+                    }
                 }
             }
             const float oscale = FUSE ? a.w2_scale : a.w_scale;
@@ -551,6 +607,36 @@
                 vu_start = vl_row(a.vl_out, halo, vu);
                 vu_next = vl_row(a.vl_out, halo, vu + 1);
             }
+            if constexpr (PAIR) {
+                const float* rb = reinterpret_cast<const float*>(a.res) + (long long)b * a.res_bs;
+                float* yb = reinterpret_cast<float*>(a.y) + (long long)b * a.y_bs;
+                int trow[4];
+#pragma unroll
+                for (int rr = 0; rr < 4; ++rr) {
+                    const int mr = wrow + 8 * (rr & 1), blk = mr / a.dil;
+                    const int t = j0 + blk * 2 * a.dil + (mr - blk * a.dil) + (rr >> 1) * a.dil;
+                    trow[rr] = mr < ttile / 2 && t < a.Tout ? t : -1;
+                }
+                float2 r2[NACC / 2];
+#pragma unroll
+                for (int k = 0; k < NACC / 2; ++k) {
+                    const int rr = k >> 2;
+                    r2[k] = trow[rr] >= 0 ? ldg2(rb + (long long)trow[rr] * a.ldr + 8 * (k & 3) + col2) : make_float2(0.f, 0.f);
+                }
+#pragma unroll
+                for (int k = 0; k < NACC / 2; ++k) {
+                    const int rr = k >> 2, i = (rr >> 1) * (PW / 2) + 2 * (rr & 1) + 4 * (k & 3), co = 8 * (k & 3) + col2;
+                    if (trow[rr] < 0) continue;
+                    float v0 = racc[i] * oscale, v1 = racc[i + 1] * oscale;
+                    if (a.bias) {
+                        const float2 b2 = __ldg(reinterpret_cast<const float2*>(a.bias + co));
+                        v0 += b2.x; v1 += b2.y;
+                    }
+                    v0 = r2[k].x + v0; v1 = r2[k].y + v1;
+                    vmax = fmaxf(vmax, fmaxf(fabsf(v0), fabsf(v1)));
+                    st2(yb + (long long)trow[rr] * a.ldy + co, v0, v1);
+                }
+            } else {
 #pragma unroll
             for (int hr = 0; hr < 2; ++hr) {
                 int bo = b, t = j0 + wrow + 8 * hr;
@@ -586,6 +672,7 @@
                         st2(reinterpret_cast<XT*>(a.y) + (long long)bo * a.y_bs + (long long)t * a.ldy + g * a.y_goff + co_l, v0, v1);
                     }
                 }
+            }
             }
         }
         if (PREC == PREC_F16 && a.err && !(vmax < 60000.f)) atomicOr(a.err, 2);
@@ -633,4 +720,30 @@
     if (sink != 0.f) g_probe_sink = sink;
 }
 
-}
+__global__ void __launch_bounds__(128) wgmma_cols_kernel(const uint4* a, const uint4* b, float* d64, float* d32) {
+    __shared__ __align__(128) uint4 sa[2 * 4 * 64];
+    __shared__ __align__(128) uint4 sb[3 * 4 * 64];
+    __shared__ __align__(128) uint4 sh[2][3 * 4 * 32];
+    const int tid = threadIdx.x, warp = tid >> 5, lane = tid & 31;
+    for (int i = tid; i < 2 * 4 * 64; i += 128) sa[i] = a[i];
+    for (int i = tid; i < 3 * 4 * 64; i += 128) {
+        sb[i] = b[i];
+        sh[(i % 64) / 32][(i / 64) * 32 + i % 32] = b[i];
+    }
+    fence_async_smem();
+    __syncthreads();
+    const uint32_t au = smem_u32(sa), lbo = 64u * 16u;
+    float d[32], h[16];
+    wg_group<64, PREC_F16, 1>(d, au, au + 4u * lbo, lbo, 0u, 1, smem_u32(sb));
+    const int r0 = 16 * warp + (lane >> 2), c0 = 2 * (lane & 3);
+#pragma unroll
+    for (int i = 0; i < 32; ++i) d64[(r0 + 8 * ((i >> 1) & 1)) * 64 + 8 * (i >> 2) + c0 + (i & 1)] = d[i];
+#pragma unroll
+    for (int hh = 0; hh < 2; ++hh) {
+        wg_group<32, PREC_F16, 1>(h, au, au + 4u * lbo, lbo, 0u, 1, smem_u32(sh[hh]));
+#pragma unroll
+        for (int i = 0; i < 16; ++i) d32[(r0 + 8 * ((i >> 1) & 1)) * 64 + 32 * hh + 8 * (i >> 2) + c0 + (i & 1)] = h[i];
+    }
+}
+
+}
diff --git a/include/audiodec_b200.h b/include/audiodec_b200.h
--- a/include/audiodec_b200.h
+++ b/include/audiodec_b200.h
@@ -99,6 +99,8 @@
 int adec_test_residual_unit(int device, const float *x, int B, int C, int T, const float *w1, const float *w2,
                             int K, int dil, float *state, float *y);
 
+int adec_test_wgmma_columns(int device, const void *a, const void *b, float *d64, float *d32);
+
 int adec_test_vocoder_layer(int device, int compute_dtype, int kind, const void *x, int B, int Cin, int T,
                             const float *w, const float *bias, int Cout, int K, int dil, int up, int groups, int shared_in,
                             int pre_act, float slope, const float *mean, const float *scale, const void *res, int offline,
```

Result: faster. 161.3 million (median of 6 runs) (+9.2%).
